# CameronDiao/MolCLR

Hardware: AMD Instinct MI355X
Metric: contrastive pre-train molecules/sec at batch 512, 1/2/4/8 MI355X; HBM GB/s on scatter_add (higher is better)
Workload: dtype f32; 1 GPU; c2: GIN 5x300 feat 512, batch 512/GPU, 10-50 atom graphs; model=gin 5x300 feat 512, global_batch=512, per_gpu_batch=512, mean_nodes_per_view=15278, mean_edges_per_view=25094, parallelism=dp1, views=one paired encoder pass, per-view BatchNorm statistics, augment=host: pre-built resident batch pairs

## Files before the change

### include/molclr.h

```cpp
#ifndef MOLCLR_H_
#define MOLCLR_H_

#include <stddef.h>
#include <stdint.h>

#ifdef __cplusplus
extern "C" {
#endif

typedef void* molclr_stream_t;

enum {
  MOLCLR_OK = 0,
  MOLCLR_ERR_ARG = -1,
  MOLCLR_ERR_WORKSPACE = -2,
  MOLCLR_ERR_UNSUPPORTED = -3
};

#define MOLCLR_NUM_ATOM_TYPE 119
#define MOLCLR_NUM_CHIRALITY 3
#define MOLCLR_NUM_BOND_TYPE 5
#define MOLCLR_NUM_BOND_DIR 3
#define MOLCLR_SELF_LOOP_BOND_TYPE 4
#define MOLCLR_ECOUNT_STRIDE 8
// ... 148 lines not shown
                         int64_t K, int64_t lda, int64_t ldb, int64_t ldc, int a_kmajor,
                         int b_kmajor, int epilogue_flags, const float* bias, const float* aux,
                         int64_t ldaux, void* workspace, size_t workspace_bytes,
                         molclr_stream_t stream, int impl);

size_t molclr_bplanes_bytes(int64_t N, int64_t K);
int molclr_bplanes_make(const float* B, int64_t N, int64_t K, int64_t ldb, int b_kmajor,
                        uint16_t* planes, molclr_stream_t stream);
int molclr_bplanes_make_batch(int count, const float* const* B, const int64_t* N,
                              const int64_t* K, const int64_t* ldb, const int* b_kmajor,
                              uint16_t* const* planes, molclr_stream_t stream);
int molclr_gemm_f32_bplanes(const float* A, const uint16_t* planes, float* C, int64_t M,
                            int64_t N, int64_t K, int64_t lda, int64_t ldc, int a_kmajor,
                            int epilogue_flags, const float* bias, const float* aux,
                            int64_t ldaux, void* workspace, size_t workspace_bytes,
                            molclr_stream_t stream);
int molclr_gemm_f32_bplanes_tile(const float* A, const uint16_t* planes, float* C, int64_t M,
                                 int64_t N, int64_t K, int64_t lda, int64_t ldc, int a_kmajor,
                                 int epilogue_flags, const float* bias, const float* aux,
                                 int64_t ldaux, void* workspace, size_t workspace_bytes,
                                 molclr_stream_t stream, int tile);

size_t molclr_linear_wgrad_workspace_bytes(int64_t rows, int64_t n_out, int64_t n_in);
int molclr_linear_wgrad(const float* dy, const float* x, float* dW, float* db, int64_t rows,
                        int64_t n_out, int64_t n_in, int64_t ld_dy, int64_t ld_x, int accumulate,
                        void* workspace, size_t workspace_bytes, molclr_stream_t stream);
int molclr_linear_wgrad_groups(const float* dy, const float* x, float* dW, float* db,
                               int64_t rows, int64_t n_out, int64_t n_in, int64_t ld_dy,
                               int64_t ld_x, int accumulate, void* workspace,
                               size_t workspace_bytes, molclr_stream_t stream, int groups);

int molclr_absmax_f32(const float* x, int64_t rows, int64_t cols, int64_t ld, float* slot,
                      int accumulate, molclr_stream_t stream);
size_t molclr_hplanes_bytes(int64_t N, int64_t K);
int molclr_hplanes_make_batch(int count, const float* const* B, const int64_t* N,
                              const int64_t* K, const int64_t* ldb, const int* b_kmajor,
                              uint16_t* const* planes, molclr_stream_t stream);
int64_t molclr_gemm_row_parts(int64_t N);
int molclr_gemm_f32_bplanes_max(const float* A, const uint16_t* planes, float* C, int64_t M,
                                int64_t N, int64_t K, int64_t lda, int64_t ldc,
                                int epilogue_flags, const float* bias, const float* aux,
                                int64_t ldaux, float* amax_out, float* cmax, float* crow,
                                uint32_t* relu_bits, void* workspace, size_t workspace_bytes,
                                molclr_stream_t stream);
int molclr_absmax_rows_f32(const float* x, int64_t rows, int64_t cols, int64_t ld,
                           float* rowmax, float* slot, int accumulate, molclr_stream_t stream);
int molclr_gemm_f32_h3(const float* A, const float* amax, int a_row_parts, const uint16_t* hplanes,
                       float* C, int64_t M, int64_t N, int64_t K, int64_t lda, int64_t ldc,
                       int epilogue_flags, const float* bias, const float* aux, int64_t ldaux,
                       const uint32_t* mask_bits, float* cmax, float* crow, float* amax_out,
                       molclr_stream_t stream);
int molclr_gemm_f32_h3_impl(const float* A, const float* amax, int a_row_parts,
                            const uint16_t* hplanes, float* C, int64_t M, int64_t N, int64_t K,
                            int64_t lda, int64_t ldc, int epilogue_flags, const float* bias,
                            const float* aux, int64_t ldaux, const uint32_t* mask_bits, float* cmax,
                            float* crow, float* amax_out, uint32_t* relu_bits,
                            molclr_stream_t stream, int impl);
int molclr_gemm_f32_h3_bits(const float* A, const float* amax, int a_row_parts,
                            const uint16_t* hplanes, float* C, int64_t M, int64_t N, int64_t K,
                            int64_t lda, int64_t ldc, int epilogue_flags, const float* bias,
                            const float* aux, int64_t ldaux, const uint32_t* mask_bits,
                            float* cmax, float* crow, float* amax_out, uint32_t* relu_bits,
                            molclr_stream_t stream);
int molclr_linear_wgrad_h3_groups(const float* dy, const float* dymax, const float* x,
                                  const float* xmax, float* dW, float* db, int64_t rows,
                                  int64_t n_out, int64_t n_in, int64_t ld_dy, int64_t ld_x,
                                  int accumulate, void* workspace, size_t workspace_bytes,
                                  molclr_stream_t stream, int groups);
int molclr_linear_wgrad_h3(const float* dy, const float* dymax, const float* x,
                           const float* xmax, float* dW, float* db, int64_t rows, int64_t n_out,
                           int64_t n_in, int64_t ld_dy, int64_t ld_x, int accumulate,
                           void* workspace, size_t workspace_bytes, molclr_stream_t stream);
size_t molclr_linear_wgrad_h3_pair_workspace_bytes(int64_t rows, int64_t n_out_a, int64_t n_in_a,
                                                   int64_t n_out_b, int64_t n_in_b);
int molclr_linear_wgrad_h3_pair(const float* dy_a, const float* dymax_a, const float* x_a,
                                const float* xmax_a, float* dW_a, float* db_a, int64_t n_out_a,
                                int64_t n_in_a, int64_t ld_dy_a, int64_t ld_x_a,
                                const float* dy_b, const float* dymax_b, const float* x_b,
                                const float* xmax_b, float* dW_b, float* db_b, int64_t n_out_b,
                                int64_t n_in_b, int64_t ld_dy_b, int64_t ld_x_b, int64_t rows,
                                int accumulate, void* workspace, size_t workspace_bytes,
                                molclr_stream_t stream);

size_t molclr_colsum_f32_workspace_bytes(int64_t rows, int64_t cols);
int molclr_colsum_f32(const float* X, float* out, int64_t rows, int64_t cols, int64_t ld,
                      int accumulate, void* workspace, size_t workspace_bytes,
                      molclr_stream_t stream);

size_t molclr_batchnorm_workspace_bytes(int64_t rows, int64_t dim);
int molclr_batchnorm_fwd(const float* z, const float* gamma, const float* beta,
                         float* running_mean, float* running_var,
                         int64_t* num_batches_tracked, float* y,
                         float* save_mean, float* save_invstd, int64_t rows, int64_t dim,
                         double momentum, double eps, int training, int relu,
                         void* workspace, size_t workspace_bytes, molclr_stream_t stream);
int molclr_batchnorm_bwd(const float* dy, const float* z, const float* gamma,
                         const float* beta, const float* save_mean,
                         const float* save_invstd, float* dz, float* dgamma, float* dbeta,
                         int64_t rows, int64_t dim, int relu, int accumulate, void* workspace,
                         size_t workspace_bytes, molclr_stream_t stream);

enum { MOLCLR_DTYPE_F32 = 0, MOLCLR_DTYPE_BF16 = 1 };
size_t molclr_batchnorm_seg_workspace_bytes(int nseg, const int64_t* seg_rows, int64_t dim);
int molclr_batchnorm_seg_fwd(const void* z, const float* gamma, const float* beta,
                             float* running_mean, float* running_var,
                             int64_t* num_batches_tracked, void* y, float* save_mean,
                             float* save_invstd, int nseg, const int64_t* seg_rows, int64_t dim,
                             int dtype, double momentum, double eps, int training, int relu,
                             void* workspace, size_t workspace_bytes, molclr_stream_t stream);
int molclr_batchnorm_seg_bwd(const void* dy, const void* z, const float* gamma,
                             const float* beta, const float* save_mean, const float* save_invstd,
                             void* dz, float* dgamma, float* dbeta, int nseg,
                             const int64_t* seg_rows, int64_t dim, int dtype, int relu,
                             int accumulate, void* workspace, size_t workspace_bytes,
                             molclr_stream_t stream);

int molclr_bn_row_parts(int64_t dim);
size_t molclr_batchnorm_seg_dev_workspace_bytes(int nseg, int64_t rows_cap, int64_t dim);
int molclr_batchnorm_seg_fwd_dev(const void* z, const float* gamma, const float* beta,
                                 float* running_mean, float* running_var,
                                 int64_t* num_batches_tracked, void* y, float* save_mean,
                                 float* save_invstd, int nseg, const int64_t* seg_rows_dev,
                                 int64_t rows_cap, int64_t dim, int dtype, double momentum,
                                 double eps, int training, int relu, void* workspace,
                                 size_t workspace_bytes, molclr_stream_t stream);
int molclr_batchnorm_seg_coeffs(const void* z, const float* gamma, const float* beta,
                                float* running_mean, float* running_var,
                                int64_t* num_batches_tracked, float* save_mean,
                                float* save_invstd, float* coeffs, int nseg,
                                const int64_t* seg_rows, int64_t dim, int dtype, double momentum,
                                double eps, int training, void* workspace, size_t workspace_bytes,
                                molclr_stream_t stream);
int molclr_batchnorm_seg_coeffs_dev(const void* z, const float* gamma, const float* beta,
                                    float* running_mean, float* running_var,
                                    int64_t* num_batches_tracked, float* save_mean,
                                    float* save_invstd, float* coeffs, int nseg,
                                    const int64_t* seg_rows_dev, int64_t rows_cap, int64_t dim,
                                    int dtype, double momentum, double eps, int training,
                                    void* workspace, size_t workspace_bytes,
                                    molclr_stream_t stream);
int molclr_batchnorm_seg_bwd_dev(const void* dy, const void* z, const float* gamma,
                                 const float* beta, const float* save_mean,
                                 const float* save_invstd, void* dz, float* dgamma, float* dbeta,
                                 int nseg, const int64_t* seg_rows_dev, int64_t rows_cap,
                                 int64_t dim, int dtype, int relu, int accumulate, float* rowmax,
                                 float* slot, void* workspace, size_t workspace_bytes,
                                 molclr_stream_t stream);
int molclr_batchnorm_seg_bwd_max(const float* dy, const float* z, const float* gamma,
                                 const float* beta, const float* save_mean,
                                 const float* save_invstd, float* dz, float* dgamma, float* dbeta,
                                 int nseg, const int64_t* seg_rows, int64_t dim, int relu,
                                 int accumulate, float* rowmax, float* slot, void* workspace,
                                 size_t workspace_bytes, molclr_stream_t stream);

int molclr_segment_pool_fwd(const float* h, const int32_t* graph_ptr, float* out,
                            int64_t num_graphs, int64_t dim, int mode,
                            molclr_stream_t stream);
int molclr_segment_pool_bwd(const float* dout, const int32_t* graph_ptr, float* dh,
                            int64_t num_nodes, int64_t num_graphs, int64_t dim, int mode,
                            molclr_stream_t stream);
int molclr_segment_max_fwd(const void* h, const int32_t* graph_ptr, float* out, int32_t* argmax,
                           int64_t num_graphs, int64_t dim, int dtype, molclr_stream_t stream);
int molclr_segment_max_bwd(const float* dout, const int32_t* argmax, void* dh, int64_t num_nodes,
                           int64_t num_graphs, int64_t dim, int dtype, molclr_stream_t stream);

int molclr_l2norm_fwd(const float* z, float* y, float* norm, int64_t rows, int64_t dim,
                      double eps, molclr_stream_t stream);
int molclr_l2norm_bwd(const float* dy, const float* y, const float* norm, float* dz,
                      int64_t rows, int64_t dim, double eps, molclr_stream_t stream);

int molclr_ntxent_prep(const float* r, float* rhat, float* norm, int64_t n, int64_t C,
                       int cosine, molclr_stream_t stream);
int molclr_ntxent_prep_bwd(const float* drhat, const float* rhat, const float* norm,
                           float* dr, int64_t n, int64_t C, int cosine,
                           molclr_stream_t stream);
int molclr_ntxent_prep_pair(const float* z, float* y, float* rhat, float* n1, float* n2,
                            int64_t batch_local, int64_t C, double eps, int cosine,
                            molclr_stream_t stream);
int molclr_ntxent_prep_pair_bwd(const float* drhat, const float* rhat, const float* n2,
                                const float* y, const float* n1, float* dz, int64_t batch_local,
                                int64_t C, double eps, int cosine, molclr_stream_t stream);
size_t molclr_ntxent_workspace_bytes(int64_t nrows, int64_t ncols, int64_t C);
int molclr_ntxent_fwd(const float* rhat_rows, const int32_t* row_gidx, const float* rhat_cols,
                      int64_t nrows, int64_t ncols, int64_t C, int64_t batch_size,
                      double temperature, float* lse_rows, float* loss_rows,
                      void* workspace, size_t workspace_bytes, molclr_stream_t stream);
int molclr_ntxent_bwd(const float* rhat_rows, const int32_t* row_gidx, const float* rhat_cols,
                      const float* lse_cols, const float* grad_loss, int64_t nrows,
                      int64_t ncols, int64_t C, int64_t batch_size, double temperature,
                      float* drhat_rows, void* workspace, size_t workspace_bytes,
                      molclr_stream_t stream);
size_t molclr_ntxent_sim_bytes(int64_t nrows, int64_t ncols, int64_t C, int impl);
int molclr_ntxent_fwd_impl(const float* rhat_rows, const int32_t* row_gidx,
                           const float* rhat_cols, int64_t nrows, int64_t ncols, int64_t C,
                           int64_t batch_size, double temperature, float* lse_rows,
                           float* loss_rows, float* sim, void* workspace, size_t workspace_bytes,
                           molclr_stream_t stream, int impl);
int molclr_ntxent_bwd_impl(const float* rhat_rows, const int32_t* row_gidx,
                           const float* rhat_cols, const float* lse_cols, const float* grad_loss,
                           int64_t nrows, int64_t ncols, int64_t C, int64_t batch_size,
                           double temperature, const float* sim, float* drhat_rows,
                           void* workspace, size_t workspace_bytes, molclr_stream_t stream,
                           int impl);
int molclr_sum_f32(const float* x, float* out, int64_t n, molclr_stream_t stream);

int molclr_adam_step(float* param, const float* grad, float* exp_avg, float* exp_avg_sq,
                     int64_t n, const float* lr, int32_t* step, double beta1, double beta2,
                     double eps, double weight_decay, molclr_stream_t stream);
int molclr_adam_step_ex(float* param, const float* grad, float* exp_avg, float* exp_avg_sq,
                        int64_t n, const float* lr, int32_t* step, double beta1, double beta2,
                        double eps, double weight_decay, int tick, molclr_stream_t stream);
int molclr_step_tail(int32_t* step, const float* loss_src, float* loss_dst,
                     const int32_t* status_src, int32_t* status_acc, molclr_stream_t stream);

typedef struct molclr_gin_encoder {
  int32_t num_layer;
  int32_t training;
  int64_t dim;
  int64_t n_atom;
  int64_t n_chiral;
  double momentum, eps;
  const float* x_embedding1;
  const float* x_embedding2;
  const float* mlp0_weight[MOLCLR_MAX_LAYERS];
  const float* mlp0_bias[MOLCLR_MAX_LAYERS];
  const float* mlp2_weight[MOLCLR_MAX_LAYERS];
  const float* mlp2_bias[MOLCLR_MAX_LAYERS];
  const float* edge_embedding1[MOLCLR_MAX_LAYERS];
  const float* edge_embedding2[MOLCLR_MAX_LAYERS];
  const float* bn_weight[MOLCLR_MAX_LAYERS];
  const float* bn_bias[MOLCLR_MAX_LAYERS];
  float* bn_running_mean[MOLCLR_MAX_LAYERS];
  float* bn_running_var[MOLCLR_MAX_LAYERS];
  int64_t* bn_num_batches_tracked[MOLCLR_MAX_LAYERS];
  const uint16_t* mlp0_planes[MOLCLR_MAX_LAYERS];
  const uint16_t* mlp0_planes_t[MOLCLR_MAX_LAYERS];
  const uint16_t* mlp2_planes[MOLCLR_MAX_LAYERS];
  const uint16_t* mlp2_planes_t[MOLCLR_MAX_LAYERS];
  int32_t dtype;
  int32_t fp32_gemm;
  int32_t* status;
} molclr_gin_encoder;

typedef struct molclr_gin_encoder_grads {
  float* x_embedding1;
  float* x_embedding2;
  float* mlp0_weight[MOLCLR_MAX_LAYERS];
  float* mlp0_bias[MOLCLR_MAX_LAYERS];
  float* mlp2_weight[MOLCLR_MAX_LAYERS];
  float* mlp2_bias[MOLCLR_MAX_LAYERS];
  float* edge_embedding1[MOLCLR_MAX_LAYERS];
  float* edge_embedding2[MOLCLR_MAX_LAYERS];
  float* bn_weight[MOLCLR_MAX_LAYERS];
  float* bn_bias[MOLCLR_MAX_LAYERS];
  void* layer_done[MOLCLR_MAX_LAYERS];
  void* embed_done;
} molclr_gin_encoder_grads;

typedef struct molclr_device_graph {
  int64_t num_nodes, num_edges, num_graphs;
  const int32_t *rowptr, *col, *rowptr_t, *col_t, *ecount, *graph_ptr;
  const uint8_t* ecode;
  const uint32_t *nbr, *nbr_t;
  int32_t num_segments;
  int64_t segment_nodes[MOLCLR_MAX_SEGMENTS];
  const int64_t* segment_nodes_dev;
} molclr_device_graph;

size_t molclr_gin_encoder_arena_bytes(int num_layer, int64_t num_nodes, int64_t dim, int dtype);
size_t molclr_gin_encoder_workspace_bytes(int num_layer, int64_t num_nodes, int64_t dim,
                                          int dtype);
int molclr_gin_encoder_fwd(const molclr_gin_encoder* enc, const int64_t* x,
                           const molclr_device_graph* graph, void* h_out, void* arena,
                           size_t arena_bytes, void* workspace, size_t workspace_bytes,
                           molclr_stream_t stream);
int molclr_gin_encoder_bwd(const molclr_gin_encoder* enc, const molclr_gin_encoder_grads* grads,
                           const int64_t* x, const molclr_device_graph* graph,
                           const void* dh_out, const void* arena, size_t arena_bytes,
                           void* workspace, size_t workspace_bytes, molclr_stream_t stream);

typedef struct molclr_gcn_encoder {
  int32_t num_layer;
  int32_t training;
  int64_t dim;
  int64_t n_atom;
  int64_t n_chiral;
  double momentum, eps;
  const float* x_embedding1;
  const float* x_embedding2;
  const float* weight[MOLCLR_MAX_LAYERS];
  const float* bias[MOLCLR_MAX_LAYERS];
  const float* edge_embedding1[MOLCLR_MAX_LAYERS];
  const float* edge_embedding2[MOLCLR_MAX_LAYERS];
  const float* bn_weight[MOLCLR_MAX_LAYERS];
  const float* bn_bias[MOLCLR_MAX_LAYERS];
  float* bn_running_mean[MOLCLR_MAX_LAYERS];
  float* bn_running_var[MOLCLR_MAX_LAYERS];
  int64_t* bn_num_batches_tracked[MOLCLR_MAX_LAYERS];
  const uint16_t* weight_planes[MOLCLR_MAX_LAYERS];
  const uint16_t* weight_planes_t[MOLCLR_MAX_LAYERS];
  int32_t fp32_gemm;
  int32_t* status;
} molclr_gcn_encoder;

typedef struct molclr_gcn_encoder_grads {
  float* x_embedding1;
// ... 130 lines not shown
```

### molclr_amd/_lib.py

```python
from __future__ import annotations

import ctypes
import os
from ctypes import POINTER, c_char_p, c_double, c_int, c_int64, c_size_t, c_uint64, c_void_p
from pathlib import Path

import torch

LIB_PATH = Path(os.environ.get("MOLCLR_LIB", Path(__file__).resolve().parent / "libmolclr_hip.so"))

_P = c_void_p
_I64 = c_int64

SIGNATURES = {
    "molclr_version": (c_char_p, []),
    "molclr_last_error": (c_char_p, []),
    "molclr_graph_build_workspace_bytes": (c_size_t, [_I64, _I64]),
    "molclr_graph_build": (c_int, [_P, _P, _P, _I64, _I64, _I64, _P, _P, _P, _P, _P, _P, _P, _P,
                                   _P, _P, _P, c_size_t, _P]),
    "molclr_graph_build_multi": (c_int, [c_int, _P, _P, _P, _P, _P, _P, _P, _P, _P, _P, _P, _P,
                                         c_size_t, _P]),
    "molclr_stage_segments": (c_int, [c_int, _P, _P, _P, _I64, _I64, _P, _P]),
    "molclr_graph_build_dev": (c_int, [c_int, _P, _P, _I64, _I64, _P, _P, _P, _P, _P, _P, _P, _P,
                                       _P, _P, _P, c_size_t, _P]),
    "molclr_mask_views_workspace_bytes": (c_size_t, [_I64]),
    "molclr_mask_views": (c_int, [_P, _P, _P, _P, _P, _I64, _I64, _P, _I64, c_uint64, c_int, _P, _P,
                                  _P, _P, _P, _I64, _I64, _P, _P, c_size_t, _P]),
    "molclr_atom_embed_fwd": (c_int, [_P, _P, _P, _P, _I64, _I64, _I64, _I64, _P, _P]),
    "molclr_atom_embed_bwd_workspace_bytes": (c_size_t, [_I64, _I64, _I64, _I64]),
    "molclr_atom_embed_bwd": (c_int, [_P, _P, _P, _P, _I64, _I64, _I64, _I64, c_int, _P, c_size_t,
                                      _P]),
    "molclr_edge_tables_combine": (c_int, [c_int, _P, _P, _P, _I64, _P]),
    "molclr_gine_aggregate_fwd": (c_int, [_P, _P, _P, _P, _P, _P, _P, _I64, _I64, _P]),
    "molclr_rowmax_layout": (_I64, [_I64]),
    "molclr_rowmax_bytes": (c_size_t, [_I64, _I64]),
    "molclr_gine_aggregate_fwd_rowmax": (c_int, [_P, _P, _P, _P, _P, _P, _P, _I64, _I64, _P, _P,
                                                 _P]),
    "molclr_gine_aggregate_bn_fwd": (c_int, [_P, _P, c_int, c_int, _P, _P, _P, _P, _P, _P, _P, _P,
                                             _I64, _I64, _P, _P, _P]),
    "molclr_gine_aggregate_bn_fwd_bf16": (c_int, [_P, _P, c_int, c_int, _P, _P, _P, _P, _P, _P, _P,
                                                  _P, _I64, _I64, _P]),
    "molclr_batchnorm_seg_coeffs": (c_int, [_P, _P, _P, _P, _P, _P, _P, _P, _P, c_int, _P, _I64,
                                            c_int, c_double, c_double, c_int, _P, c_size_t, _P]),
    "molclr_batchnorm_seg_coeffs_dev": (c_int, [_P, _P, _P, _P, _P, _P, _P, _P, _P, c_int, _P, _I64,
                                                _I64, c_int, c_double, c_double, c_int, _P,
                                                c_size_t, _P]),
    "molclr_gine_aggregate_bwd_workspace_bytes": (c_size_t, [_I64, _I64]),
    "molclr_gine_aggregate_bwd": (c_int, [_P, _P, _P, _P, _P, _P, _P, _P, _I64, _I64, c_int, _P,
                                          c_size_t, _P]),
    "molclr_gcn_aggregate_fwd": (c_int, [_P, _P, _P, _P, _P, _P, _P, _P, _P, _I64, _I64, _P]),
    "molclr_gcn_aggregate_bwd_workspace_bytes": (c_size_t, [_I64, _I64]),
    "molclr_gcn_aggregate_bwd": (c_int, [_P, _P, _P, _P, _P, _P, _P, _P, _P, _I64, _I64, c_int,
                                         _P, c_size_t, _P]),
    "molclr_gemm_f32_workspace_bytes": (c_size_t, [_I64, _I64, _I64]),
    "molclr_gemm_f32": (c_int, [_P, _P, _P, _I64, _I64, _I64, _I64, _I64, _I64, c_int, c_int, c_int,
                                _P, _P, _I64, _P, c_size_t, _P]),
    "molclr_gemm_f32_impl": (c_int, [_P, _P, _P, _I64, _I64, _I64, _I64, _I64, _I64, c_int, c_int,
                                     c_int, _P, _P, _I64, _P, c_size_t, _P, c_int]),
    "molclr_bplanes_bytes": (c_size_t, [_I64, _I64]),
    "molclr_bplanes_make": (c_int, [_P, _I64, _I64, _I64, c_int, _P, _P]),
    "molclr_bplanes_make_batch": (c_int, [c_int, _P, _P, _P, _P, _P, _P, _P]),
    "molclr_gemm_f32_bplanes": (c_int, [_P, _P, _P, _I64, _I64, _I64, _I64, _I64, c_int, c_int, _P,
                                        _P, _I64, _P, c_size_t, _P]),
    "molclr_gemm_f32_bplanes_tile": (c_int, [_P, _P, _P, _I64, _I64, _I64, _I64, _I64, c_int,
                                             c_int, _P, _P, _I64, _P, c_size_t, _P, c_int]),
    "molclr_linear_wgrad_workspace_bytes": (c_size_t, [_I64, _I64, _I64]),
    "molclr_linear_wgrad": (c_int, [_P, _P, _P, _P, _I64, _I64, _I64, _I64, _I64, c_int, _P, c_size_t,
                                    _P]),
    "molclr_linear_wgrad_groups": (c_int, [_P, _P, _P, _P, _I64, _I64, _I64, _I64, _I64, c_int, _P,
                                           c_size_t, _P, c_int]),
    "molclr_absmax_f32": (c_int, [_P, _I64, _I64, _I64, _P, c_int, _P]),
    "molclr_hplanes_bytes": (c_size_t, [_I64, _I64]),
    "molclr_hplanes_make_batch": (c_int, [c_int, _P, _P, _P, _P, _P, _P, _P]),
    "molclr_absmax_rows_f32": (c_int, [_P, _I64, _I64, _I64, _P, _P, c_int, _P]),
    "molclr_bn_row_parts": (c_int, [_I64]),
    "molclr_batchnorm_seg_bwd_max": (c_int, [_P, _P, _P, _P, _P, _P, _P, _P, _P, c_int, _P, _I64,
                                             c_int, c_int, _P, _P, _P, c_size_t, _P]),
    "molclr_gemm_row_parts": (_I64, [_I64]),
    "molclr_gemm_f32_bplanes_max": (c_int, [_P, _P, _P, _I64, _I64, _I64, _I64, _I64, c_int, _P,
                                            _P, _I64, _P, _P, _P, _P, _P, c_size_t, _P]),
    "molclr_gemm_f32_h3": (c_int, [_P, _P, c_int, _P, _P, _I64, _I64, _I64, _I64, _I64, c_int, _P,
                                   _P, _I64, _P, _P, _P, _P, _P]),
    "molclr_gemm_f32_h3_bits": (c_int, [_P, _P, c_int, _P, _P, _I64, _I64, _I64, _I64, _I64, c_int,
                                        _P, _P, _I64, _P, _P, _P, _P, _P, _P]),
    "molclr_gemm_f32_h3_impl": (c_int, [_P, _P, c_int, _P, _P, _I64, _I64, _I64, _I64, _I64, c_int,
                                        _P, _P, _I64, _P, _P, _P, _P, _P, _P, c_int]),
    "molclr_linear_wgrad_h3_groups": (c_int, [_P, _P, _P, _P, _P, _P, _I64, _I64, _I64, _I64, _I64,
                                              c_int, _P, c_size_t, _P, c_int]),
    "molclr_linear_wgrad_h3": (c_int, [_P, _P, _P, _P, _P, _P, _I64, _I64, _I64, _I64, _I64, c_int,
                                       _P, c_size_t, _P]),
    "molclr_colsum_f32_workspace_bytes": (c_size_t, [_I64, _I64]),
    "molclr_colsum_f32": (c_int, [_P, _P, _I64, _I64, _I64, c_int, _P, c_size_t, _P]),
    "molclr_batchnorm_workspace_bytes": (c_size_t, [_I64, _I64]),
    "molclr_batchnorm_fwd": (c_int, [_P, _P, _P, _P, _P, _P, _P, _P, _P, _I64, _I64, c_double,
                                     c_double, c_int, c_int, _P, c_size_t, _P]),
    "molclr_batchnorm_bwd": (c_int, [_P, _P, _P, _P, _P, _P, _P, _P, _P, _I64, _I64, c_int, c_int,
                                     _P, c_size_t, _P]),
    "molclr_batchnorm_seg_workspace_bytes": (c_size_t, [c_int, _P, _I64]),
    "molclr_batchnorm_seg_fwd": (c_int, [_P, _P, _P, _P, _P, _P, _P, _P, _P, c_int, _P, _I64, c_int,
                                         c_double, c_double, c_int, c_int, _P, c_size_t, _P]),
    "molclr_batchnorm_seg_bwd": (c_int, [_P, _P, _P, _P, _P, _P, _P, _P, _P, c_int, _P, _I64, c_int,
                                         c_int, c_int, _P, c_size_t, _P]),
    "molclr_batchnorm_seg_dev_workspace_bytes": (c_size_t, [c_int, _I64, _I64]),
    "molclr_batchnorm_seg_fwd_dev": (c_int, [_P, _P, _P, _P, _P, _P, _P, _P, _P, c_int, _P, _I64,
                                             _I64, c_int, c_double, c_double, c_int, c_int, _P,
                                             c_size_t, _P]),
    "molclr_batchnorm_seg_bwd_dev": (c_int, [_P, _P, _P, _P, _P, _P, _P, _P, _P, c_int, _P, _I64,
                                             _I64, c_int, c_int, c_int, _P, _P, _P, c_size_t, _P]),
    "molclr_segment_pool_fwd": (c_int, [_P, _P, _P, _I64, _I64, c_int, _P]),
    "molclr_segment_pool_bwd": (c_int, [_P, _P, _P, _I64, _I64, _I64, c_int, _P]),
    "molclr_l2norm_fwd": (c_int, [_P, _P, _P, _I64, _I64, c_double, _P]),
    "molclr_l2norm_bwd": (c_int, [_P, _P, _P, _P, _I64, _I64, c_double, _P]),
    "molclr_ntxent_prep": (c_int, [_P, _P, _P, _I64, _I64, c_int, _P]),
    "molclr_ntxent_prep_bwd": (c_int, [_P, _P, _P, _P, _I64, _I64, c_int, _P]),
    "molclr_ntxent_prep_pair": (c_int, [_P, _P, _P, _P, _P, _I64, _I64, c_double, c_int, _P]),
    "molclr_ntxent_prep_pair_bwd": (c_int, [_P, _P, _P, _P, _P, _P, _I64, _I64, c_double, c_int,
                                            _P]),
    "molclr_ntxent_workspace_bytes": (c_size_t, [_I64, _I64, _I64]),
    "molclr_ntxent_fwd": (c_int, [_P, _P, _P, _I64, _I64, _I64, _I64, c_double, _P, _P, _P,
                                  c_size_t, _P]),
    "molclr_ntxent_bwd": (c_int, [_P, _P, _P, _P, _P, _I64, _I64, _I64, _I64, c_double, _P, _P,
                                  c_size_t, _P]),
    "molclr_ntxent_sim_bytes": (c_size_t, [_I64, _I64, _I64, c_int]),
    "molclr_ntxent_fwd_impl": (c_int, [_P, _P, _P, _I64, _I64, _I64, _I64, c_double, _P, _P,
                                       _P, _P, c_size_t, _P, c_int]),
    "molclr_ntxent_bwd_impl": (c_int, [_P, _P, _P, _P, _P, _I64, _I64, _I64, _I64, c_double, _P,
                                       _P, _P, c_size_t, _P, c_int]),
    "molclr_sum_f32": (c_int, [_P, _P, _I64, _P]),
    "molclr_linear_wgrad_h3_pair_workspace_bytes": (c_size_t, [_I64, _I64, _I64, _I64, _I64]),
    "molclr_linear_wgrad_h3_pair": (c_int, [_P, _P, _P, _P, _P, _P, _I64, _I64, _I64, _I64,
                                            _P, _P, _P, _P, _P, _P, _I64, _I64, _I64, _I64,
                                            _I64, c_int, _P, c_size_t, _P]),
    "molclr_adam_step": (c_int, [_P, _P, _P, _P, _I64, _P, _P, c_double, c_double, c_double,
                                 c_double, _P]),
    "molclr_adam_step_ex": (c_int, [_P, _P, _P, _P, _I64, _P, _P, c_double, c_double, c_double,
                                    c_double, c_int, _P]),
    "molclr_step_tail": (c_int, [_P, _P, _P, _P, _P, _P]),
    "molclr_gin_encoder_arena_bytes": (c_size_t, [c_int, _I64, _I64, c_int]),
    "molclr_gin_encoder_workspace_bytes": (c_size_t, [c_int, _I64, _I64, c_int]),
    "molclr_gin_encoder_fwd": (c_int, [_P, _P, _P, _P, _P, c_size_t, _P, c_size_t, _P]),
    "molclr_gin_encoder_bwd": (c_int, [_P, _P, _P, _P, _P, _P, c_size_t, _P, c_size_t, _P]),
    "molclr_gcn_encoder_arena_bytes": (c_size_t, [c_int, _I64, _I64]),
    "molclr_gcn_encoder_workspace_bytes": (c_size_t, [c_int, _I64, _I64]),
    "molclr_gcn_encoder_fwd": (c_int, [_P, _P, _P, _P, _P, c_size_t, _P, c_size_t, _P]),
    "molclr_gcn_encoder_bwd": (c_int, [_P, _P, _P, _P, _P, _P, c_size_t, _P, c_size_t, _P]),
    "molclr_aug_views_workspace_bytes": (c_size_t, [_I64, _I64, _I64]),
    "molclr_aug_views_plan": (c_int, [_P, _P, _P, _I64, _I64, _P, _I64, ctypes.c_uint64, c_int,
                                      c_int, _I64, _I64, _P, _P, _P, _P, c_size_t, _P]),
    "molclr_aug_views_big_workspace_bytes": (c_size_t, [_I64, _I64, _I64]),
    "molclr_aug_views_plan_big": (c_int, [_P, _P, _P, _I64, _I64, _P, _I64, ctypes.c_uint64,
                                          c_int, c_int, _I64, _I64, _P, _P, _P, _P, c_size_t,
                                          _I64, _I64, _I64, _P, c_size_t, _P]),
    "molclr_aug_views_write": (c_int, [_P, _P, _P, _P, _P, _I64, _I64, _P, _I64, _P, _I64, _I64,
                                       _I64, _P, _P, _P, _P, _P, c_size_t, _P]),
    "molclr_atom_embed_fwd_bf16": (c_int, [_P, _P, _P, _P, _I64, _I64, _I64, _I64, _P, _P]),
    "molclr_atom_embed_bwd_bf16": (c_int, [_P, _P, _P, _P, _I64, _I64, _I64, _I64, c_int, _P,
                                           c_size_t, _P]),
    "molclr_gine_aggregate_fwd_bf16": (c_int, [_P, _P, _P, _P, _P, _P, _P, _I64, _I64, _P]),
    "molclr_gine_aggregate_bwd_bf16": (c_int, [_P, _P, _P, _P, _P, _P, _P, _P, _I64, _I64, c_int,
                                               _P, c_size_t, _P]),
    "molclr_segment_max_fwd": (c_int, [_P, _P, _P, _P, _I64, _I64, c_int, _P]),
    "molclr_segment_max_bwd": (c_int, [_P, _P, _P, _I64, _I64, _I64, c_int, _P]),
    "molclr_segment_pool_fwd_bf16": (c_int, [_P, _P, _P, _I64, _I64, c_int, _P]),
    "molclr_segment_pool_bwd_bf16": (c_int, [_P, _P, _P, _I64, _I64, _I64, c_int, _P]),
    "molclr_gemm_bf16": (c_int, [_P, _P, _P, _I64, _I64, _I64, _I64, _I64, c_int, _P, _P, _I64,
                                 _P]),
    "molclr_gemm_bf16_bits": (c_int, [_P, _P, _P, _I64, _I64, _I64, _I64, _I64, c_int, _P, _P, _P,
                                      _P]),
    "molclr_gemm_bf16_impl": (c_int, [_P, _P, _P, _I64, _I64, _I64, _I64, _I64, c_int, _P, _P,
                                      _I64, _P, c_int]),
    "molclr_linear_wgrad_bf16_workspace_bytes": (c_size_t, [_I64, _I64, _I64]),
    "molclr_linear_wgrad_bf16_impl": (c_int, [_P, _P, _P, _P, _I64, _I64, _I64, _I64, _I64, c_int,
                                              _P, c_size_t, _P, c_int]),
    "molclr_linear_wgrad_bf16": (c_int, [_P, _P, _P, _P, _I64, _I64, _I64, _I64, _I64, c_int, _P,
                                         c_size_t, _P]),
    "molclr_task_head_workspace_bytes": (c_size_t, [_P]),
    "molclr_task_head_fwd": (c_int, [_P, _P, c_size_t, _P]),
    "molclr_task_head_bwd": (c_int, [_P, _P, _P, c_size_t, _P]),
    "molclr_ktimer_start": (c_int, [c_int]),
    "molclr_ktimer_read": (c_int, [c_int, _P, _P]),
    "molclr_ktimer_stop": (c_int, []),
}

EPI_NONE, EPI_BIAS, EPI_BIAS_RELU, EPI_RELU_MASK = 0, 1, 2, 3
EPI_ACCUMULATE = 16
NUM_ECOMB = 15
MAX_LAYERS = 16
MAX_SEGMENTS = 8
DTYPE_F32, DTYPE_BF16 = 0, 1
STATUS_ATOM_RANGE = 8
STATUS_LABEL_RANGE = 16
TASK_HEAD_MAX_LAYERS = 10
TASK_HEAD_MAX_CLASSES = 16
TASK_HEAD_MAX_DIM = 2044
ACT_NONE, ACT_RELU, ACT_SOFTPLUS = 0, 1, 2
LOSS_NONE, LOSS_CROSS_ENTROPY, LOSS_MSE, LOSS_L1 = 0, 1, 2, 3
KTIMER_GINE_AGG = 1
KTIMER_GEMM = 2
KTIMER_NTXENT = 4
KTIMER_GCN_AGG = 8
AUG_SUBGRAPH, AUG_MIX = 0, 1


_L16 = c_void_p * 16


class GinEncoder(ctypes.Structure):
    _fields_ = [("num_layer", ctypes.c_int32), ("training", ctypes.c_int32), ("dim", c_int64),
                ("n_atom", c_int64), ("n_chiral", c_int64), ("momentum", c_double),
                ("eps", c_double), ("x_embedding1", c_void_p), ("x_embedding2", c_void_p)] + [
        (f, _L16) for f in ("mlp0_weight", "mlp0_bias", "mlp2_weight", "mlp2_bias",
                            "edge_embedding1", "edge_embedding2", "bn_weight", "bn_bias",
                            "bn_running_mean", "bn_running_var", "bn_num_batches_tracked",
                            "mlp0_planes", "mlp0_planes_t", "mlp2_planes", "mlp2_planes_t")] + [
        ("dtype", ctypes.c_int32), ("fp32_gemm", ctypes.c_int32), ("status", c_void_p)]


class GinEncoderGrads(ctypes.Structure):
    _fields_ = [("x_embedding1", c_void_p), ("x_embedding2", c_void_p)] + [
        (f, _L16) for f in ("mlp0_weight", "mlp0_bias", "mlp2_weight", "mlp2_bias",
                            "edge_embedding1", "edge_embedding2", "bn_weight", "bn_bias")] + [
        ("layer_done", _L16), ("embed_done", c_void_p)]


class GcnEncoder(ctypes.Structure):
    _fields_ = [("num_layer", ctypes.c_int32), ("training", ctypes.c_int32), ("dim", c_int64),
                ("n_atom", c_int64), ("n_chiral", c_int64), ("momentum", c_double),
                ("eps", c_double), ("x_embedding1", c_void_p), ("x_embedding2", c_void_p)] + [
        (f, _L16) for f in ("weight", "bias", "edge_embedding1", "edge_embedding2", "bn_weight",
                            "bn_bias", "bn_running_mean", "bn_running_var",
                            "bn_num_batches_tracked", "weight_planes", "weight_planes_t")] + [
        ("fp32_gemm", ctypes.c_int32), ("status", c_void_p)]


class GcnEncoderGrads(ctypes.Structure):
    _fields_ = [("x_embedding1", c_void_p), ("x_embedding2", c_void_p)] + [
        (f, _L16) for f in ("weight", "bias", "edge_embedding1", "edge_embedding2", "bn_weight",
                            "bn_bias")] + [("layer_done", _L16), ("embed_done", c_void_p)]


_L10 = c_void_p * 10


class TaskHeadC(ctypes.Structure):
    _fields_ = [("num_layers", ctypes.c_int32), ("loss", ctypes.c_int32), ("rows", c_int64),
                ("dims", c_int64 * 11), ("act", ctypes.c_int32 * 10), ("x", c_void_p),
                ("ldx", c_int64), ("weight", _L10), ("bias", _L10), ("a", _L10),
                ("target", c_void_p), ("loss_out", c_void_p), ("status", c_void_p),
                ("sync", c_void_p)]


class TaskHeadGradsC(ctypes.Structure):
    _fields_ = [("gloss", c_void_p), ("dh", c_void_p), ("dpred", c_void_p), ("dx", c_void_p),
                ("lddx", c_int64), ("dweight", _L10), ("dbias", _L10),
                ("accumulate", ctypes.c_int32 * 10)]


class DeviceGraphC(ctypes.Structure):
    _fields_ = [("num_nodes", c_int64), ("num_edges", c_int64), ("num_graphs", c_int64)] + [
        (f, c_void_p) for f in ("rowptr", "col", "rowptr_t", "col_t", "ecount", "graph_ptr",
                                "ecode", "nbr", "nbr_t")] + [
# ... 79 lines not shown
```

### molclr_amd/csrc/aggregate.hip

```cpp
#include "common.h"

#include <stdlib.h>

namespace {

constexpr int kT = 256;

template <typename St, int U = 1>
__global__ void k_atom_embed_fwd(const int64_t* __restrict__ x, const float4* __restrict__ X1,
                                 const float4* __restrict__ X2, typename St::T* __restrict__ h,
                                 int64_t N, int d4, int64_t n1, int64_t n2,
                                 int32_t* __restrict__ status) {
  int64_t t = (int64_t)blockIdx.x * blockDim.x + threadIdx.x;
  if (t >= N * d4 / U) return;
  const int64_t u0 = t * U;
  int64_t i = N * d4 < (1ll << 32) ? (int64_t)((uint32_t)u0 / (uint32_t)d4) : u0 / d4;
  int c = (int)(u0 - i * d4);
  const int64_t a = x[2 * i], b = x[2 * i + 1];
  float4 v[U];
  if (a < 0 || a >= n1 || b < 0 || b >= n2) {
    const float q = __builtin_nanf("");
#pragma unroll
    for (int j = 0; j < U; ++j) v[j] = make_float4(q, q, q, q);
    if (c == 0 && status != nullptr) atomicOr(status, MOLCLR_STATUS_ATOM_RANGE);
// ... 80 lines not shown
    kchunk0[k] = kc[k];
  }
  const int nch = kc[nk];
  for (int c = t; c < max_chunks; c += 1024) {
    if (c >= nch) break;
    int lo = 0, hi = nk - 1;
    while (lo < hi) {
      const int mid = (lo + hi + 1) >> 1;
      if (kc[mid] <= c) lo = mid;
      else hi = mid - 1;
    }
    const int32_t q = (c - kc[lo]) * kEmbChunk;
    cbeg[c] = ks[lo] + q;
    cend[c] = ks[lo] + (q + kEmbChunk < tot[lo] ? q + kEmbChunk : tot[lo]);
  }
}

__global__ __launch_bounds__(kEmbBlock) void k_emb_scatter(const int64_t* __restrict__ x,
                                                           int64_t N, int64_t n1, int64_t n2,
                                                           const int32_t* __restrict__ off,
                                                           const int32_t* __restrict__ kstart,
                                                           int32_t* __restrict__ perm) {
  __shared__ int32_t keys[kEmbBlock];
  const int nk = (int)(n1 + n2);
  const int64_t item = (int64_t)blockIdx.x * kEmbBlock + threadIdx.x;
  const bool live = item < 2 * N;
  const int k = live ? emb_key(x, item, N, n1, n2) : -1;
  keys[threadIdx.x] = k;
  __syncthreads();
  if (!live) return;
  int rank = 0;
  for (int j = 0; j < (int)threadIdx.x; ++j) rank += keys[j] == k;
  (void)nk;
  perm[kstart[k] + off[(int64_t)k * gridDim.x + blockIdx.x] + rank] =
      (int32_t)(item < N ? item : item - N);
}

template <typename St>
__global__ __launch_bounds__(64) void k_emb_chunk_sum(const typename St::T* __restrict__ dh,
                                                      const int32_t* __restrict__ perm,
                                                      const int32_t* __restrict__ cbeg,
                                                      const int32_t* __restrict__ cend,
                                                      const int32_t* __restrict__ nchunks,
                                                      int64_t d4, double* __restrict__ csum) {
  const int64_t ch = blockIdx.x;
  if (ch >= *nchunks) return;
  const int64_t c = (int64_t)blockIdx.y * 64 + threadIdx.x;
  if (c >= d4) return;
  const int32_t beg = cbeg[ch], end = cend[ch];
  float4 acc = f4zero();
  int32_t i = beg;
  for (; i + 16 <= end; i += 16) {
    float4 v[16];
#pragma unroll
    for (int u = 0; u < 16; ++u) v[u] = St::ld(dh, (int64_t)perm[i + u] * d4 + c);
#pragma unroll
    for (int u = 0; u < 16; ++u) acc = f4add(acc, v[u]);
  }
  for (; i + 4 <= end; i += 4) {
    float4 v[4];
#pragma unroll
    for (int u = 0; u < 4; ++u) v[u] = St::ld(dh, (int64_t)perm[i + u] * d4 + c);
#pragma unroll
    for (int u = 0; u < 4; ++u) acc = f4add(acc, v[u]);
  }
  for (; i < end; ++i) acc = f4add(acc, St::ld(dh, (int64_t)perm[i] * d4 + c));
  double* o = csum + ch * 4 * d4 + 4 * c;
  o[0] = acc.x;
  o[1] = acc.y;
  o[2] = acc.z;
  o[3] = acc.w;
}

constexpr int kEmbFinW = 8;
__global__ __launch_bounds__(64 * kEmbFinW) void k_emb_finish(
    const double* __restrict__ csum, const int32_t* __restrict__ kchunk0, int64_t n1, int64_t n2,
    int64_t D, float* __restrict__ dX1, float* __restrict__ dX2, int accumulate) {
  __shared__ double red[kEmbFinW][64];
  const int lane = threadIdx.x & 63, w = threadIdx.x >> 6;
  const int64_t k = blockIdx.x;
  const int64_t col = (int64_t)blockIdx.y * 64 + lane;
  double acc = 0.0;
  if (col < D) {
    int32_t ch = kchunk0[k] + w;
    const int32_t ce = kchunk0[k + 1];
    for (; ch + 7 * kEmbFinW < ce; ch += 8 * kEmbFinW) {
      double v[8];
#pragma unroll
      for (int u = 0; u < 8; ++u) v[u] = csum[(int64_t)(ch + u * kEmbFinW) * D + col];
#pragma unroll
      for (int u = 0; u < 8; ++u) acc += v[u];
    }
    for (; ch < ce; ch += kEmbFinW) acc += csum[(int64_t)ch * D + col];
  }
  red[w][lane] = acc;
  __syncthreads();
  if (w != 0 || col >= D) return;
  double t = red[0][lane];
#pragma unroll
  for (int q = 1; q < kEmbFinW; ++q) t += red[q][lane];
  float* o = k < n1 ? dX1 + k * D + col : dX2 + (k - n1) * D + col;
  *o = accumulate ? *o + (float)t : (float)t;
}

__global__ __launch_bounds__(1024) void k_reduce_partials_split(
    const double* __restrict__ partial, int64_t P, int64_t rows, int64_t D, int64_t split,
    float* __restrict__ outA, float* __restrict__ outB, int accumulate) {
  constexpr int EL = 16, LANES = 64;
  __shared__ double red[LANES][EL];
  const int cl = threadIdx.x % EL, rl = threadIdx.x / EL;
  const int64_t t = (int64_t)blockIdx.x * EL + cl;
  const int64_t n = rows * D;
  double a0 = 0.0, a1 = 0.0, a2 = 0.0, a3 = 0.0;
  if (t < n) {
    int64_t p = rl;
    for (; p + 3 * LANES < P; p += 4 * LANES) {
      a0 += partial[p * n + t];
      a1 += partial[(p + LANES) * n + t];
      a2 += partial[(p + 2 * LANES) * n + t];
      a3 += partial[(p + 3 * LANES) * n + t];
    }
    for (; p < P; p += LANES) a0 += partial[p * n + t];
  }
  double acc = (a0 + a1) + (a2 + a3);
  red[rl][cl] = acc;
  __syncthreads();
#pragma unroll
  for (int stride = LANES / 2; stride > 0; stride >>= 1) {
    if (rl < stride) red[rl][cl] = acc = acc + red[rl + stride][cl];
    __syncthreads();
  }
  if (rl != 0 || t >= n) return;
  int64_t r = t / D;
  float* o = r < split ? (outA ? outA + t : nullptr) : (outB ? outB + (t - split * D) : nullptr);
  if (o) *o = accumulate ? *o + (float)acc : (float)acc;
}

struct TablePtrs {
  const float* e1[MOLCLR_MAX_LAYERS];
  const float* e2[MOLCLR_MAX_LAYERS];
};
__global__ void k_edge_tables_combine(TablePtrs p, float* __restrict__ Ec, int layers, int64_t D,
                                      float* __restrict__ zero, int64_t n_zero) {
  const int64_t per = (int64_t)MOLCLR_NUM_ECOMB * D;
  int64_t t = (int64_t)blockIdx.x * blockDim.x + threadIdx.x;
  if (t < n_zero) zero[t] = 0.f;
  if (t >= layers * per) return;
  const int l = (int)(t / per);
  const int64_t rc = t - l * per;
  const int r = (int)(rc / D);
  const int64_t c = rc - (int64_t)r * D;
  Ec[t] = p.e1[l][(r / 3) * D + c] + p.e2[l][(r % 3) * D + c];
}

__device__ __forceinline__ uint32_t nbr_degree(uint32_t w0) { return w0 >> 29; }
__device__ __forceinline__ int32_t nbr_node(uint32_t w) { return (int32_t)(w & 0xFFFFFFu); }
__device__ __forceinline__ int nbr_ecomb(uint32_t w) { return (int)((w >> 24) & 15u); }

__device__ __forceinline__ float4 gine_msg(const float4* __restrict__ x, const float4* __restrict__ Ec,
                                           uint32_t w, int d4, int c) {
  return f4add(x[(int64_t)nbr_node(w) * d4 + c], Ec[nbr_ecomb(w) * d4 + c]);
}

struct NoSrcArgs {};
struct BnSrcArgs {
  const float4* scale;
  const float4* shift;
  int relu;
  Segs sg;
};

template <typename St>
__device__ __forceinline__ float4 bn_src_unit(float4 v, float4 sc, float4 sh, bool relu) {
  float4 o = make_float4(bn_apply1(v.x, sc.x, sh.x), bn_apply1(v.y, sc.y, sh.y),
                         bn_apply1(v.z, sc.z, sh.z), bn_apply1(v.w, sc.w, sh.w));
  if (relu) o = make_float4(fmaxf(o.x, 0.f), fmaxf(o.y, 0.f), fmaxf(o.z, 0.f), fmaxf(o.w, 0.f));
  if constexpr (St::kBytes == 2) {
    const uint32_t lo = f32x2_to_bf16x2(o.x, o.y), hi = f32x2_to_bf16x2(o.z, o.w);
    o = make_float4(bf16_to_f32(lo & 0xFFFFu), bf16_to_f32(lo >> 16), bf16_to_f32(hi & 0xFFFFu),
                    bf16_to_f32(hi >> 16));
  }
  return o;
}

template <typename St, typename SA>
struct AggSrc {
  __device__ __forceinline__ AggSrc(const SA&, int64_t, int, int) {}
  __device__ __forceinline__ float4 operator()(const typename St::T* __restrict__ x,
                                               int64_t unit) const {
    return St::ld(x, unit);
  }
};
template <typename St>
struct AggSrc<St, BnSrcArgs> {
  float4 sc, sh;
  bool relu, pad;
  __device__ __forceinline__ AggSrc(const BnSrcArgs& a, int64_t i, int c, int d4) {
    const int s = seg_of_row(a.sg, i);
    pad = s < 0;
    relu = a.relu != 0;
    sc = pad ? f4zero() : a.scale[s * d4 + c];
    sh = pad ? f4zero() : a.shift[s * d4 + c];
  }
  __device__ __forceinline__ float4 operator()(const typename St::T* __restrict__ x,
                                               int64_t unit) const {
    if (pad) return f4zero();
    return bn_src_unit<St>(St::ld(x, unit), sc, sh, relu);
  }
};

template <typename St, bool NT = false, typename SA = NoSrcArgs>
__device__ __forceinline__ float4 gine_agg_elem(
    const typename St::T* __restrict__ x, const int32_t* __restrict__ rowptr,
    const int32_t* __restrict__ col, const uint8_t* __restrict__ ecode,
    const uint4* __restrict__ nbr, const float4* __restrict__ Ec, typename St::T* __restrict__ out,
    int64_t t, int64_t i, int c, int d4, const SA& sa) {
  const AggSrc<St, SA> src(sa, i, c, d4);
  auto X = [&](int64_t idx) { return src(x, idx); };
  auto msg = [&](uint32_t w) {
    return f4add(X((int64_t)nbr_node(w) * d4 + c), Ec[nbr_ecomb(w) * d4 + c]);
  };
  const uint4 s = nbr[i];
  const float4 self = X(t);
  const float4 es = Ec[MOLCLR_SELF_LOOP_ECOMB * d4 + c];
  const uint32_t deg = nbr_degree(s.x);
  float4 acc = f4zero();
  if (deg <= MOLCLR_NBR_SLOTS) {
    const float4 m0 = deg > 0 ? msg(s.x) : acc;
    const float4 m1 = deg > 1 ? msg(s.y) : acc;
    const float4 m2 = deg > 2 ? msg(s.z) : acc;
    const float4 m3 = deg > 3 ? msg(s.w) : acc;
    if (deg > 0) acc = f4add(acc, m0);
    if (deg > 1) acc = f4add(acc, m1);
    if (deg > 2) acc = f4add(acc, m2);
    if (deg > 3) acc = f4add(acc, m3);
  } else {
    for (int32_t k = rowptr[i], e = rowptr[i + 1]; k < e; ++k)
      acc = f4add(acc, f4add(X((int64_t)col[k] * d4 + c), Ec[MOLCLR_ECOMB(ecode[k]) * d4 + c]));
  }
  acc = f4add(acc, f4add(self, es));
  if constexpr (NT) {
    typedef float f4v __attribute__((ext_vector_type(4)));
    __builtin_nontemporal_store(f4v{acc.x, acc.y, acc.z, acc.w}, reinterpret_cast<f4v*>(out) + t);
  } else {
    St::st(out, t, acc);
  }
  return acc;
}

template <typename St, bool ROWMAX, bool NT = false, typename SA = NoSrcArgs>
__global__ __launch_bounds__(kT) void k_gine_agg_fwd(
    const typename St::T* __restrict__ x, const int32_t* __restrict__ rowptr,
    const int32_t* __restrict__ col, const uint8_t* __restrict__ ecode,
    const uint4* __restrict__ nbr, const float4* __restrict__ Ec, typename St::T* __restrict__ out,
    int64_t N, int d4, float* __restrict__ rowparts, int nparts, float* __restrict__ slot, SA sa) {
  int64_t t = (int64_t)xcd_remap(blockIdx.x, gridDim.x) * blockDim.x + threadIdx.x;
  int64_t i;
  int c;
  if (N * d4 < (1ll << 32)) {
    const uint32_t q = (uint32_t)t / (uint32_t)d4;
    i = q;
    c = (int)((uint32_t)t - q * (uint32_t)d4);
  } else {
    i = t / d4;
    c = (int)(t - i * d4);
  }
  if constexpr (ROWMAX) {
    float m = 0.f;
    int row = -1;
    if (t < N * d4) {
      const float4 v = gine_agg_elem<St, NT>(x, rowptr, col, ecode, nbr, Ec, out, t, i, c, d4, sa);
      m = fmaxf(fmaxf(fabsf(v.x), fabsf(v.y)), fmaxf(fabsf(v.z), fabsf(v.w)));
      row = (int)i;
    }
    if (nparts < 0)
      row_max_waves(m, row, t, N, d4, reinterpret_cast<float2*>(rowparts));
    else
      row_max_parts(m, row, t, N, d4, rowparts, nparts);
    if (slot != nullptr) absmax_publish(m, slot);
    return;
  }
  if (t >= N * d4) return;
  gine_agg_elem<St, NT>(x, rowptr, col, ecode, nbr, Ec, out, t, i, c, d4, sa);
}

template <typename St = StF32>
__global__ __launch_bounds__(kT) void k_transpose_gather(const typename St::T* __restrict__ g,
                                                         const int32_t* __restrict__ rowptr_t,
                                                         const int32_t* __restrict__ col_t,
                                                         const uint4* __restrict__ nbr_t,
                                                         typename St::T* __restrict__ dx, int64_t N,
                                                         int d4) {
  int64_t t = (int64_t)xcd_remap(blockIdx.x, gridDim.x) * blockDim.x + threadIdx.x;
  if (t >= N * d4) return;
  int64_t j = N * d4 < (1ll << 32) ? (int64_t)((uint32_t)t / (uint32_t)d4) : t / d4;
  int c = (int)(t - j * d4);
  const uint4 s = nbr_t[j];
  const uint32_t deg = nbr_degree(s.x);
  float4 acc = f4zero();
  if (deg <= MOLCLR_NBR_SLOTS) {
    if (deg > 0) acc = f4add(acc, St::ld(g, (int64_t)nbr_node(s.x) * d4 + c));
    if (deg > 1) acc = f4add(acc, St::ld(g, (int64_t)nbr_node(s.y) * d4 + c));
    if (deg > 2) acc = f4add(acc, St::ld(g, (int64_t)nbr_node(s.z) * d4 + c));
    if (deg > 3) acc = f4add(acc, St::ld(g, (int64_t)nbr_node(s.w) * d4 + c));
  } else {
    for (int32_t k = rowptr_t[j], e = rowptr_t[j + 1]; k < e; ++k)
      acc = f4add(acc, St::ld(g, (int64_t)col_t[k] * d4 + c));
  }
  St::st(dx, t, f4add(acc, St::ld(g, t)));
}
// ... 751 lines not shown
```

### molclr_amd/csrc/common.h

```cpp
#pragma once

#include <hip/hip_ext.h>
#include <hip/hip_runtime.h>

#include <type_traits>
#include <stdint.h>
#include <stddef.h>

#include "../../include/molclr.h"

#define MOLCLR_API extern "C" __attribute__((visibility("default")))

namespace molclr {

void set_error(const char* fmt, ...) __attribute__((format(printf, 1, 2)));

inline hipStream_t as_stream(molclr_stream_t s) { return reinterpret_cast<hipStream_t>(s); }

int edge_tables_combine_zero(int layers, const float* const* E1s, const float* const* E2s,
                             float* Ec, int64_t D, float* zero, int64_t n_zero,
                             molclr_stream_t stream);

int hplanes_make_and_max(const float* B, int64_t N, int64_t K, uint16_t* planes, const float* x,
                         int64_t x_rows, int64_t x_cols, float* x_slot, hipStream_t stream);
// ... 104 lines not shown
}
}

inline hipError_t fill_async(void* p, int v, size_t bytes, hipStream_t s) {
  if (bytes == 0) return hipSuccess;
  hipLaunchKernelGGL(detail::k_fill_bytes, dim3(detail::fill_blocks(bytes)), dim3(256), 0, s,
                     static_cast<uint8_t*>(p), bytes, (uint8_t)v);
  return hipGetLastError();
}
inline hipError_t zero_async(void* p, size_t bytes, hipStream_t s) {
  return fill_async(p, 0, bytes, s);
}
inline hipError_t copy_async(void* dst, const void* src, size_t bytes, hipStream_t s) {
  if (bytes == 0) return hipSuccess;
  hipLaunchKernelGGL(detail::k_copy_bytes, dim3(detail::fill_blocks(bytes)), dim3(256), 0, s,
                     static_cast<uint8_t*>(dst), static_cast<const uint8_t*>(src), bytes);
  return hipGetLastError();
}

}

size_t molclr_batchnorm_ws_bound(int64_t rows, int64_t D);

#define MOLCLR_REQUIRE(cond, ...)        \
  do {                                   \
    if (!(cond)) {                       \
      molclr::set_error(__VA_ARGS__);    \
      return MOLCLR_ERR_ARG;             \
    }                                    \
  } while (0)

#define MOLCLR_REQUIRE_WS(ws, need)                                                   \
  do {                                                                                \
    if ((ws) < (need)) {                                                              \
      molclr::set_error("%s: workspace %zu bytes < required %zu", __func__,           \
                        (size_t)(ws), (size_t)(need));                                \
      return MOLCLR_ERR_WORKSPACE;                                                    \
    }                                                                                 \
  } while (0)

#define MOLCLR_TRY_RC(expr)   \
  do {                        \
    int rc_ = (expr);         \
    if (rc_) return rc_;      \
  } while (0)

#define MOLCLR_LAUNCHED()                                                             \
  do {                                                                                \
    hipError_t e_ = hipGetLastError();                                                \
    if (e_ != hipSuccess) {                                                           \
      molclr::set_error("%s: launch failed: %s", __func__, hipGetErrorString(e_));    \
      return (int)e_;                                                                 \
    }                                                                                 \
  } while (0)

__device__ __forceinline__ float4 f4add(float4 a, float4 b) {
  return make_float4(a.x + b.x, a.y + b.y, a.z + b.z, a.w + b.w);
}
__device__ __forceinline__ int xcd_remap(int bid, int nwg) {
  int q = nwg / 8, r = nwg % 8;
  int x = bid % 8, pos = bid / 8;
  int base = x < r ? x * (q + 1) : r * (q + 1) + (x - r) * q;
  return base + pos;
}

__device__ __forceinline__ float4 f4zero() { return make_float4(0.f, 0.f, 0.f, 0.f); }

__device__ __forceinline__ void wave_lds_sync() {
  __builtin_amdgcn_fence(__ATOMIC_RELEASE, "wavefront");
  __builtin_amdgcn_wave_barrier();
  __builtin_amdgcn_fence(__ATOMIC_ACQUIRE, "wavefront");
}

struct StF32 {
  typedef float T;
  static constexpr int kBytes = 4;
  __device__ __forceinline__ static float4 ld(const T* __restrict__ p, int64_t unit) {
    return reinterpret_cast<const float4*>(p)[unit];
  }
  __device__ __forceinline__ static void st(T* __restrict__ p, int64_t unit, float4 v) {
    reinterpret_cast<float4*>(p)[unit] = v;
  }
  __device__ __forceinline__ static void ld2(const T* __restrict__ p, int64_t u2, float4& a,
                                             float4& b) {
    a = reinterpret_cast<const float4*>(p)[2 * u2];
    b = reinterpret_cast<const float4*>(p)[2 * u2 + 1];
  }
  __device__ __forceinline__ static void st2(T* __restrict__ p, int64_t u2, float4 a, float4 b) {
    reinterpret_cast<float4*>(p)[2 * u2] = a;
    reinterpret_cast<float4*>(p)[2 * u2 + 1] = b;
  }
  __device__ __forceinline__ static float ld1(const T* __restrict__ p, int64_t i) { return p[i]; }
  __device__ __forceinline__ static void st1(T* __restrict__ p, int64_t i, float v) { p[i] = v; }
};

__device__ __forceinline__ float bf16_to_f32(uint32_t bits16) {
  return __uint_as_float(bits16 << 16);
}
__device__ __forceinline__ uint32_t f32x2_to_bf16x2(float a, float b) {
  typedef __bf16 bf2 __attribute__((ext_vector_type(2)));
  const bf2 v = {(__bf16)a, (__bf16)b};
  return __builtin_bit_cast(uint32_t, v);
}

struct StBF16 {
  typedef uint16_t T;
  static constexpr int kBytes = 2;
  __device__ __forceinline__ static float4 ld(const T* __restrict__ p, int64_t unit) {
    const uint2 u = reinterpret_cast<const uint2*>(p)[unit];
    return make_float4(bf16_to_f32(u.x & 0xFFFFu), bf16_to_f32(u.x >> 16),
                       bf16_to_f32(u.y & 0xFFFFu), bf16_to_f32(u.y >> 16));
  }
  __device__ __forceinline__ static void st(T* __restrict__ p, int64_t unit, float4 v) {
    reinterpret_cast<uint2*>(p)[unit] = make_uint2(f32x2_to_bf16x2(v.x, v.y), f32x2_to_bf16x2(v.z, v.w));
  }
  __device__ __forceinline__ static void ld2(const T* __restrict__ p, int64_t u2, float4& a,
                                             float4& b) {
    const uint4 q = reinterpret_cast<const uint4*>(p)[u2];
    a = make_float4(bf16_to_f32(q.x & 0xFFFFu), bf16_to_f32(q.x >> 16), bf16_to_f32(q.y & 0xFFFFu),
                    bf16_to_f32(q.y >> 16));
    b = make_float4(bf16_to_f32(q.z & 0xFFFFu), bf16_to_f32(q.z >> 16), bf16_to_f32(q.w & 0xFFFFu),
                    bf16_to_f32(q.w >> 16));
  }
  __device__ __forceinline__ static void st2(T* __restrict__ p, int64_t u2, float4 a, float4 b) {
    reinterpret_cast<uint4*>(p)[u2] = make_uint4(f32x2_to_bf16x2(a.x, a.y), f32x2_to_bf16x2(a.z, a.w),
                                                 f32x2_to_bf16x2(b.x, b.y), f32x2_to_bf16x2(b.z, b.w));
  }
  __device__ __forceinline__ static float ld1(const T* __restrict__ p, int64_t i) {
    return bf16_to_f32(p[i]);
  }
  __device__ __forceinline__ static void st1(T* __restrict__ p, int64_t i, float v) {
    p[i] = (uint16_t)(f32x2_to_bf16x2(v, 0.f) & 0xFFFFu);
  }
};

struct Segs {
  int n;
  int band;
  int64_t rows[MOLCLR_MAX_SEGMENTS];
  const int64_t* drows;
};

__device__ __forceinline__ int64_t seg_n(const Segs& sg, int s) {
  return sg.drows ? sg.drows[s] : sg.rows[s];
}
__device__ __forceinline__ int seg_of_row(const Segs& sg, int64_t i) {
  int64_t r = 0;
  for (int s = 0; s < sg.n; ++s) {
    r += seg_n(sg, s);
    if (i < r) return s;
  }
  return -1;
}

__device__ __forceinline__ float bn_apply1(float z, float sc, float sh) { return __fmaf_rn(z, sc, sh); }

__device__ __forceinline__ float wave_sum(float v) {
#pragma unroll
  for (int o = 32; o > 0; o >>= 1) v += __shfl_xor(v, o, 64);
  return v;
}
__device__ __forceinline__ float wave_max_dpp(float v) {
  auto dpp = [](float x, auto ctrl) {
    return __int_as_float(__builtin_amdgcn_update_dpp(0, __float_as_int(x), decltype(ctrl)::value,
                                                      0xF, 0xF, false));
  };
  v = fmaxf(v, dpp(v, std::integral_constant<int, 0xB1>{}));
  v = fmaxf(v, dpp(v, std::integral_constant<int, 0x4E>{}));
  v = fmaxf(v, dpp(v, std::integral_constant<int, 0x141>{}));
  v = fmaxf(v, dpp(v, std::integral_constant<int, 0x140>{}));
  const float a = __int_as_float(__builtin_amdgcn_readlane(__float_as_int(v), 0));
  const float b = __int_as_float(__builtin_amdgcn_readlane(__float_as_int(v), 16));
  const float c = __int_as_float(__builtin_amdgcn_readlane(__float_as_int(v), 32));
  const float d = __int_as_float(__builtin_amdgcn_readlane(__float_as_int(v), 48));
  return fmaxf(fmaxf(a, b), fmaxf(c, d));
}
__device__ __forceinline__ float wave_max(float v) {
#pragma unroll
  for (int o = 32; o > 0; o >>= 1) v = fmaxf(v, __shfl_xor(v, o, 64));
  return v;
}

__device__ __forceinline__ void row_max_parts(float m, int row, int64_t t, int64_t rows, int d4,
                                              float* __restrict__ rowparts, int nparts) {
  const int lane = threadIdx.x & 63;
  if (d4 >= 64) {
    const int64_t t0 = t - lane;
    const int64_t r0 = rows * d4 < (1ll << 32) ? (int64_t)((uint32_t)t0 / (uint32_t)d4) : t0 / d4;
    const bool second = row >= 0 && row != r0;
    const float m0 = wave_max_dpp(second ? 0.f : m), m1 = wave_max_dpp(second ? m : 0.f);
    if (lane == 0 && r0 < rows) {
      const int64_t rs = r0 * d4;
      const int part = (int)((t0 >> 6) - (rs >> 6));
      rowparts[part * rows + r0] = m0;
      if (part == 0)
        for (int q = (int)(((rs + d4 - 1) >> 6) - (rs >> 6)) + 1; q < nparts; ++q)
          rowparts[q * rows + r0] = 0.f;
    }
    const int64_t r1 = r0 + 1, rs1 = r1 * d4;
    if (lane == 1 && r1 < rows && rs1 < t0 + 64) {
      rowparts[r1] = m1;
      for (int q = (int)(((rs1 + d4 - 1) >> 6) - (rs1 >> 6)) + 1; q < nparts; ++q)
        rowparts[q * rows + r1] = 0.f;
    }
    return;
  }
#pragma unroll
  for (int off = 1; off < 64; off <<= 1) {
    const float mv = __shfl_down(m, off, 64);
    const int rv = __shfl_down(row, off, 64);
    if (lane + off < 64 && rv == row) m = fmaxf(m, mv);
  }
  const int rp = __shfl_up(row, 1, 64);
  if (row >= 0 && (lane == 0 || rp != row)) {
    const int64_t rs = (int64_t)row * d4;
    const int part = (int)((t >> 6) - (rs >> 6));
    rowparts[part * rows + row] = m;
    if (part == 0)
      for (int q = (int)(((rs + d4 - 1) >> 6) - (rs >> 6)) + 1; q < nparts; ++q)
        rowparts[q * rows + row] = 0.f;
  }
}

__device__ __forceinline__ void row_max_waves(float m, int row, int64_t t, int64_t rows, int d4,
                                              float2* __restrict__ wm) {
  const int lane = threadIdx.x & 63;
  const int64_t t0 = t - lane;
  const int64_t r0 = rows * d4 < (1ll << 32) ? (int64_t)((uint32_t)t0 / (uint32_t)d4) : t0 / d4;
  const bool second = row >= 0 && row != r0;
  const float m0 = wave_max_dpp(second ? 0.f : m), m1 = wave_max_dpp(second ? m : 0.f);
  if (lane == 0 && t0 < rows * d4) wm[t0 >> 6] = make_float2(m0, m1);
}
__device__ __forceinline__ float row_max_of_waves(const float2* __restrict__ wm, int64_t row,
                                                  int d4) {
  const int64_t s = row * d4, e = s + d4 - 1;
  float m = 0.f;
  for (int64_t w = s >> 6; w <= (e >> 6); ++w) {
    const float2 v = wm[w];
    m = fmaxf(m, (w << 6) >= s ? v.x : v.y);
  }
  return m;
}

constexpr int kMaxSlotParts = 64;
constexpr int kMaxSlotStride = 32;
constexpr int kMaxSlotFloats = kMaxSlotParts * kMaxSlotStride;

__device__ __forceinline__ float absmax4_range(const float4* __restrict__ x, int64_t t, int64_t n4,
                                               int64_t stride) {
  auto amax4 = [](float4 v) {
    return fmaxf(fmaxf(fabsf(v.x), fabsf(v.y)), fmaxf(fabsf(v.z), fabsf(v.w)));
  };
  float m = 0.f;
  for (; t + 7 * stride < n4; t += 8 * stride) {
    float4 v[8];
#pragma unroll
    for (int j = 0; j < 8; ++j) v[j] = x[t + j * stride];
#pragma unroll
    for (int j = 0; j < 8; ++j) m = fmaxf(m, amax4(v[j]));
  }
  for (; t < n4; t += stride) m = fmaxf(m, amax4(x[t]));
  return m;
}

__device__ __forceinline__ float block_max(float v) {
  __shared__ float red_b[16];
  v = wave_max(v);
  if ((threadIdx.x & 63) == 0) red_b[threadIdx.x >> 6] = v;
  __syncthreads();
  if (threadIdx.x == 0)
    for (int w = 1; w < (int)(blockDim.x >> 6); ++w) v = fmaxf(v, red_b[w]);
  return v;
}

__device__ __forceinline__ void absmax_publish(float v, float* slot) {
  __shared__ float red_[16];
  v = wave_max(v);
  if ((threadIdx.x & 63) == 0) red_[threadIdx.x >> 6] = v;
  __syncthreads();
  if (threadIdx.x == 0) {
    for (int w = 1; w < (int)((blockDim.x + 63) >> 6); ++w) v = fmaxf(v, red_[w]);
    atomicMax(reinterpret_cast<unsigned int*>(slot + (blockIdx.x % kMaxSlotParts) * kMaxSlotStride),
              __float_as_uint(v));
  }
  __syncthreads();
}
```

### molclr_amd/csrc/encoder.hip

```cpp
#include "common.h"

#include <stdlib.h>

namespace {

bool agg_bn() {
  static const bool on = [] {
    const char* e = getenv("MOLCLR_AGG_BN");
    return !(e != nullptr && e[0] == '0');
  }();
  return on;
}

struct ArenaLayout {
  size_t agg[MOLCLR_MAX_LAYERS], a1[MOLCLR_MAX_LAYERS], z[MOLCLR_MAX_LAYERS],
      h[MOLCLR_MAX_LAYERS], mean[MOLCLR_MAX_LAYERS], invstd[MOLCLR_MAX_LAYERS],
      coef[MOLCLR_MAX_LAYERS];
  size_t bits[MOLCLR_MAX_LAYERS];
  size_t h0, ec, smax, bmax, total;
  ArenaLayout(int L, int64_t N, int64_t D, size_t es) {
    size_t used = 0;
    auto off = [&](size_t bytes) {
      const size_t o = used;
      used += (bytes + 255) / 256 * 256;
      return o;
    };
    for (int l = 0; l < L; ++l) {
      agg[l] = off(N * D * es);
      a1[l] = off(N * 2 * D * es);
      z[l] = off(N * D * es);
      h[l] = agg_bn() ? 0 : off(N * D * es);
      mean[l] = off(MOLCLR_MAX_SEGMENTS * D * sizeof(float));
      invstd[l] = off(MOLCLR_MAX_SEGMENTS * D * sizeof(float));
      coef[l] = off(2 * MOLCLR_MAX_SEGMENTS * D * sizeof(float));
      bits[l] = off((size_t)N * ((2 * D + 31) / 32) * sizeof(uint32_t));
    }
    h0 = off(N * D * es);
    ec = off((size_t)L * MOLCLR_NUM_ECOMB * D * sizeof(float));
    smax = off((size_t)MOLCLR_MAX_LAYERS * 2 * kMaxSlotFloats * sizeof(float));
    bmax = off((size_t)MOLCLR_MAX_LAYERS * 2 * kMaxSlotFloats * sizeof(float));
    total = used;
  }
};

size_t elem_bytes(int dtype) { return dtype == MOLCLR_DTYPE_BF16 ? 2 : 4; }

size_t kernels_ws(int64_t N, int64_t D) {
  size_t m = 0;
  auto mx = [&](size_t v) { m = v > m ? v : m; };
  mx(molclr_gemm_f32_workspace_bytes(2 * D, D, N));
  mx(molclr_gemm_f32_workspace_bytes(D, 2 * D, N));
  mx(molclr_gemm_f32_workspace_bytes(N, 2 * D, D));
  mx(molclr_gemm_f32_workspace_bytes(N, D, 2 * D));
  mx(molclr_colsum_f32_workspace_bytes(N, 2 * D));
  mx(molclr_linear_wgrad_workspace_bytes(N, D, 2 * D));
  mx(molclr_linear_wgrad_workspace_bytes(N, 2 * D, D));
  if (N >= 1024 && D % 4 == 0) mx(molclr_linear_wgrad_h3_pair_workspace_bytes(N, D, 2 * D, 2 * D, D));
  mx(molclr_linear_wgrad_bf16_workspace_bytes(N, D, 2 * D));
  mx(molclr_linear_wgrad_bf16_workspace_bytes(N, 2 * D, D));
  mx(molclr_batchnorm_ws_bound(N, D));
  mx(molclr_gine_aggregate_bwd_workspace_bytes(N, D));
  mx(molclr_atom_embed_bwd_workspace_bytes(N, D, MOLCLR_NUM_ATOM_TYPE, MOLCLR_NUM_CHIRALITY));
  return m;
}

size_t scratch_bytes(int64_t N, int64_t D, size_t es) { return ((size_t)N * D * 3 + (size_t)N * 2 * D) * es; }

int check_encoder(const molclr_gin_encoder* e, const molclr_device_graph* g) {
  MOLCLR_REQUIRE(e && g, "gin_encoder: null encoder / graph");
  MOLCLR_REQUIRE(e->num_layer >= 1 && e->num_layer <= MOLCLR_MAX_LAYERS,
                 "gin_encoder: num_layer %d", e->num_layer);
  MOLCLR_REQUIRE(e->dim > 0 && e->dim % 4 == 0, "gin_encoder: dim %lld", (long long)e->dim);
  MOLCLR_REQUIRE(e->dtype == MOLCLR_DTYPE_F32 || (e->dtype == MOLCLR_DTYPE_BF16 && e->dim % 8 == 0),
                 "gin_encoder: dtype %d (bf16 needs dim %% 8 == 0)", e->dtype);
  MOLCLR_REQUIRE(e->n_atom == MOLCLR_NUM_ATOM_TYPE && e->n_chiral == MOLCLR_NUM_CHIRALITY,
                 "gin_encoder: embedding tables must be [%d,D] and [%d,D]",
                 MOLCLR_NUM_ATOM_TYPE, MOLCLR_NUM_CHIRALITY);
  for (int l = 0; l < e->num_layer; ++l)
    MOLCLR_REQUIRE(e->mlp0_planes[l] && e->mlp0_planes_t[l] && e->mlp2_planes[l] &&
                       e->mlp2_planes_t[l] && e->bn_weight[l] && e->bn_bias[l],
                   "gin_encoder: layer %d: missing planes or BatchNorm affine", l);
  return MOLCLR_OK;
}

struct SegRows {
  int n;
  const int64_t* rows;
  const int64_t* dev;
  int64_t cap;
};
int graph_segments(const molclr_device_graph* g, const int64_t* N, SegRows& out) {
  if (g->segment_nodes_dev) {
    MOLCLR_REQUIRE(g->num_segments >= 1 && g->num_segments <= MOLCLR_MAX_SEGMENTS,
                   "encoder: %d graph segments", g->num_segments);
    out = {g->num_segments, nullptr, g->segment_nodes_dev, *N};
    return MOLCLR_OK;
  }
  if (g->num_segments <= 1) {
    out = {1, N, nullptr, *N};
    return MOLCLR_OK;
  }
  MOLCLR_REQUIRE(g->num_segments <= MOLCLR_MAX_SEGMENTS, "encoder: %d graph segments",
                 g->num_segments);
  int64_t tot = 0;
  for (int s = 0; s < g->num_segments; ++s) tot += g->segment_nodes[s];
  MOLCLR_REQUIRE(tot == *N, "encoder: segment nodes sum to %lld, graph has %lld", (long long)tot,
                 (long long)*N);
  out = {g->num_segments, g->segment_nodes, nullptr, *N};
  return MOLCLR_OK;
}

int seg_bn_fwd(const SegRows& sg, const void* z, const float* gamma, const float* beta,
               float* rmean, float* rvar, int64_t* nbt, void* y, float* mean, float* invstd,
               int64_t D, int dtype, double momentum, double eps, int training, int relu,
               void* ws, size_t ws_bytes, molclr_stream_t stream) {
  if (sg.dev)
    return molclr_batchnorm_seg_fwd_dev(z, gamma, beta, rmean, rvar, nbt, y, mean, invstd, sg.n,
                                        sg.dev, sg.cap, D, dtype, momentum, eps, training, relu,
                                        ws, ws_bytes, stream);
  return molclr_batchnorm_seg_fwd(z, gamma, beta, rmean, rvar, nbt, y, mean, invstd, sg.n,
                                  sg.rows, D, dtype, momentum, eps, training, relu, ws, ws_bytes,
                                  stream);
}
int seg_bn_coeffs(const SegRows& sg, const void* z, const float* gamma, const float* beta,
                  float* rmean, float* rvar, int64_t* nbt, float* mean, float* invstd, float* coef,
                  int64_t D, int dtype, double momentum, double eps, int training, void* ws,
                  size_t ws_bytes, molclr_stream_t stream) {
  if (sg.dev)
    return molclr_batchnorm_seg_coeffs_dev(z, gamma, beta, rmean, rvar, nbt, mean, invstd, coef,
                                           sg.n, sg.dev, sg.cap, D, dtype, momentum, eps, training,
                                           ws, ws_bytes, stream);
  return molclr_batchnorm_seg_coeffs(z, gamma, beta, rmean, rvar, nbt, mean, invstd, coef, sg.n,
                                     sg.rows, D, dtype, momentum, eps, training, ws, ws_bytes,
                                     stream);
}
int seg_bn_bwd(const SegRows& sg, const void* dy, const void* z, const float* gamma,
               const float* beta, const float* mean, const float* invstd, void* dz, float* dgamma,
               float* dbeta, int64_t D, int dtype, int relu, int accumulate, float* rowmax,
               float* slot, void* ws, size_t ws_bytes, molclr_stream_t stream) {
  if (sg.dev)
    return molclr_batchnorm_seg_bwd_dev(dy, z, gamma, beta, mean, invstd, dz, dgamma, dbeta, sg.n,
                                        sg.dev, sg.cap, D, dtype, relu, accumulate, rowmax, slot,
                                        ws, ws_bytes, stream);
  if (rowmax)
    return molclr_batchnorm_seg_bwd_max((const float*)dy, (const float*)z, gamma, beta, mean,
                                        invstd, (float*)dz, dgamma, dbeta, sg.n, sg.rows, D, relu,
                                        accumulate, rowmax, slot, ws, ws_bytes, stream);
  return molclr_batchnorm_seg_bwd(dy, z, gamma, beta, mean, invstd, dz, dgamma, dbeta, sg.n,
                                  sg.rows, D, dtype, relu, accumulate, ws, ws_bytes, stream);
}

#define MOLCLR_TRY(expr)      \
  do {                        \
    int rc_ = (expr);         \
    if (rc_) return rc_;      \
  } while (0)

int record_done(void* ev, molclr_stream_t stream) {
  if (ev && hipEventRecord(static_cast<hipEvent_t>(ev), molclr::as_stream(stream)) != hipSuccess) {
    molclr::set_error("encoder_bwd: hipEventRecord failed");
    return MOLCLR_ERR_ARG;
  }
  return MOLCLR_OK;
}

}

MOLCLR_API size_t molclr_gin_encoder_arena_bytes(int L, int64_t N, int64_t D, int dtype) {
  if (L < 1 || L > MOLCLR_MAX_LAYERS) return 0;
  return ArenaLayout(L, N, D, elem_bytes(dtype)).total;
}

constexpr size_t kSlotBytes = MOLCLR_MAX_LAYERS * 2 * kMaxSlotFloats * sizeof(float);
size_t rowmax_first_bytes(int64_t N, int64_t D) {
  const size_t dz = (size_t)molclr_bn_row_parts(D) * N * sizeof(float);
  const size_t agg = molclr_rowmax_bytes(N, D);
  return molclr::align_up(dz > agg ? dz : agg, 256);
}
size_t rowmax_bytes(int64_t N, int64_t D) {
  return molclr::align_up(
      rowmax_first_bytes(N, D) + (size_t)molclr_gemm_row_parts(2 * D) * N * sizeof(float), 256);
}

MOLCLR_API size_t molclr_gin_encoder_workspace_bytes(int L, int64_t N, int64_t D, int dtype) {
  (void)L;
  return molclr::align_up(scratch_bytes(N, D, elem_bytes(dtype)), 256) + kSlotBytes +
         rowmax_bytes(N, D) + kernels_ws(N, D) + 256;
}

MOLCLR_API int molclr_gin_encoder_fwd(const molclr_gin_encoder* e, const int64_t* x,
                                      const molclr_device_graph* g, void* h_out, void* arena,
                                      size_t arena_bytes, void* workspace, size_t workspace_bytes,
                                      molclr_stream_t stream) {
  MOLCLR_TRY(check_encoder(e, g));
  const int L = e->num_layer;
  const int64_t N = g->num_nodes, D = e->dim;
  if (N == 0) return MOLCLR_OK;
  SegRows seg;
  MOLCLR_TRY(graph_segments(g, &g->num_nodes, seg));
  MOLCLR_REQUIRE(x && h_out && arena, "gin_encoder_fwd: null pointer");
  const bool bf = e->dtype == MOLCLR_DTYPE_BF16;
  const size_t es = elem_bytes(e->dtype);
  const ArenaLayout lay(L, N, D, es);
  MOLCLR_REQUIRE_WS(arena_bytes, lay.total);
  MOLCLR_REQUIRE_WS(workspace_bytes, molclr_gin_encoder_workspace_bytes(L, N, D, e->dtype));
  char* A = (char*)arena;
  auto F = [&](size_t off) { return (float*)(A + off); };
  auto H = [&](size_t off) { return (uint16_t*)(A + off); };
  float* ragg = (float*)((char*)workspace + molclr::align_up(scratch_bytes(N, D, es), 256) +
                         kSlotBytes);
  float* ra1 = (float*)((char*)ragg + rowmax_first_bytes(N, D));
  void* kws = (char*)ragg + rowmax_bytes(N, D);
  const size_t kws_bytes = kernels_ws(N, D);
  const bool h3 = !bf && e->fp32_gemm != 0;
  const bool h3f = h3 && (e->fp32_gemm & 2);
  float* fmax = F(lay.smax);

  const bool fused = agg_bn();
  void* h = A + lay.h0;
  if (bf)
    MOLCLR_TRY(molclr_atom_embed_fwd_bf16(x, e->x_embedding1, e->x_embedding2, (uint16_t*)h, N, D,
                                          e->n_atom, e->n_chiral, e->status, stream));
  else
    MOLCLR_TRY(molclr_atom_embed_fwd(x, e->x_embedding1, e->x_embedding2, (float*)h, N, D,
                                     e->n_atom, e->n_chiral, e->status, stream));
  float* Ec = F(lay.ec);
  const int64_t nz = h3 ? (int64_t)(lay.bmax - lay.smax) / 4 + (int64_t)L * 2 * kMaxSlotFloats : 0;
  MOLCLR_TRY(molclr::edge_tables_combine_zero(L, e->edge_embedding1, e->edge_embedding2, Ec, D,
                                              h3 ? fmax : nullptr, nz, stream));
  for (int l = 0; l < L; ++l) {
    const bool last = l == L - 1;
    const bool bn_src = fused && l > 0;
    const bool bn_next = fused && !last;
    void* y = last ? h_out : bn_next ? nullptr : A + lay.h[l];
    const float* Ecl = Ec + (size_t)l * MOLCLR_NUM_ECOMB * D;
    const void* zp = bn_src ? A + lay.z[l - 1] : nullptr;
    const float* cp = bn_src ? F(lay.coef[l - 1]) : nullptr;
    if (bf) {
      uint16_t *agg = H(lay.agg[l]), *a1 = H(lay.a1[l]), *z = H(lay.z[l]);
      if (bn_src)
        MOLCLR_TRY(molclr_gine_aggregate_bn_fwd_bf16((const uint16_t*)zp, cp, 1, seg.n, seg.rows,
                                                     seg.dev, g->rowptr, g->col, g->ecode, g->nbr,
                                                     Ecl, agg, N, D, stream));
      else
        MOLCLR_TRY(molclr_gine_aggregate_fwd_bf16((const uint16_t*)h, g->rowptr, g->col, g->ecode,
                                                  g->nbr, Ecl, agg, N, D, stream));
      if (D % 64 == 0)
        MOLCLR_TRY(molclr_gemm_bf16_bits(agg, e->mlp0_planes[l], a1, N, 2 * D, D, D, 2 * D,
                                         MOLCLR_EPI_BIAS_RELU, e->mlp0_bias[l],
                                         (uint32_t*)(A + lay.bits[l]), nullptr, stream));
      else
        MOLCLR_TRY(molclr_gemm_bf16(agg, e->mlp0_planes[l], a1, N, 2 * D, D, D, 2 * D,
                                    MOLCLR_EPI_BIAS_RELU, e->mlp0_bias[l], nullptr, 0, stream));
      MOLCLR_TRY(molclr_gemm_bf16(a1, e->mlp2_planes[l], z, N, D, 2 * D, 2 * D, D,
                                  MOLCLR_EPI_BIAS, e->mlp2_bias[l], nullptr, 0, stream));
      if (bn_next)
        MOLCLR_TRY(seg_bn_coeffs(seg, z, e->bn_weight[l], e->bn_bias[l], e->bn_running_mean[l],
                                 e->bn_running_var[l], e->bn_num_batches_tracked[l],
                                 F(lay.mean[l]), F(lay.invstd[l]), F(lay.coef[l]), D,
                                 MOLCLR_DTYPE_BF16, e->momentum, e->eps, e->training, kws,
                                 kws_bytes, stream));
      else
        MOLCLR_TRY(seg_bn_fwd(seg, z, e->bn_weight[l], e->bn_bias[l], e->bn_running_mean[l],
                              e->bn_running_var[l], e->bn_num_batches_tracked[l], y,
                              F(lay.mean[l]), F(lay.invstd[l]), D, MOLCLR_DTYPE_BF16, e->momentum,
                              e->eps, e->training, last ? 0 : 1, kws, kws_bytes, stream));
    } else {
      float *agg = F(lay.agg[l]), *a1 = F(lay.a1[l]), *z = F(lay.z[l]);
      float* sl = fmax + 2 * l * kMaxSlotFloats;
      if (bn_src)
        MOLCLR_TRY(molclr_gine_aggregate_bn_fwd((const float*)zp, cp, 1, seg.n, seg.rows, seg.dev,
                                                g->rowptr, g->col, g->ecode, g->nbr, Ecl, agg, N,
                                                D, h3f ? ragg : nullptr, nullptr, stream));
      else if (h3f)
        MOLCLR_TRY(molclr_gine_aggregate_fwd_rowmax((const float*)h, g->rowptr, g->col, g->ecode,
                                                    g->nbr, Ecl, agg, N, D, ragg, nullptr,
                                                    stream));
      else
        MOLCLR_TRY(molclr_gine_aggregate_fwd((const float*)h, g->rowptr, g->col, g->ecode, g->nbr,
                                             Ecl, agg, N, D, stream));
      if (h3f) {
        const uint16_t* p0 = e->mlp0_planes[l];
        const uint16_t* p2 = e->mlp2_planes[l];
        MOLCLR_TRY(molclr_gemm_f32_h3_bits(agg, ragg, (int)molclr_rowmax_layout(D), p0, a1, N,
                                           2 * D, D, D, 2 * D, MOLCLR_EPI_BIAS_RELU,
                                           e->mlp0_bias[l], nullptr, 0, nullptr,
                                           sl + kMaxSlotFloats, ra1, sl,
                                           (uint32_t*)(A + lay.bits[l]), stream));
        MOLCLR_TRY(molclr_gemm_f32_h3(a1, ra1, (int)molclr_gemm_row_parts(2 * D), p2, z, N, D,
                                      2 * D, 2 * D, D, MOLCLR_EPI_BIAS, e->mlp2_bias[l], nullptr, 0,
                                      nullptr,
                                      nullptr, nullptr, nullptr, stream));
      } else {
        if (h3)
          MOLCLR_TRY(molclr_gemm_f32_bplanes_max(agg, e->mlp0_planes[l], a1, N, 2 * D, D, D, 2 * D,
                                                 MOLCLR_EPI_BIAS_RELU, e->mlp0_bias[l], nullptr, 0,
                                                 fmax + 2 * l * kMaxSlotFloats,
                                                 fmax + (2 * l + 1) * kMaxSlotFloats, nullptr,
                                                 (uint32_t*)(A + lay.bits[l]), kws, kws_bytes,
                                                 stream));
        else
          MOLCLR_TRY(molclr_gemm_f32_bplanes(agg, e->mlp0_planes[l], a1, N, 2 * D, D, D, 2 * D, 0,
                                             MOLCLR_EPI_BIAS_RELU, e->mlp0_bias[l], nullptr, 0, kws,
                                             kws_bytes, stream));
        MOLCLR_TRY(molclr_gemm_f32_bplanes(a1, e->mlp2_planes[l], z, N, D, 2 * D, 2 * D, D, 0,
                                           MOLCLR_EPI_BIAS, e->mlp2_bias[l], nullptr, 0, kws,
                                           kws_bytes, stream));
      }
      if (bn_next)
        MOLCLR_TRY(seg_bn_coeffs(seg, z, e->bn_weight[l], e->bn_bias[l], e->bn_running_mean[l],
                                 e->bn_running_var[l], e->bn_num_batches_tracked[l],
                                 F(lay.mean[l]), F(lay.invstd[l]), F(lay.coef[l]), D,
                                 MOLCLR_DTYPE_F32, e->momentum, e->eps, e->training, kws, kws_bytes,
                                 stream));
      else
        MOLCLR_TRY(seg_bn_fwd(seg, z, e->bn_weight[l], e->bn_bias[l], e->bn_running_mean[l],
                              e->bn_running_var[l], e->bn_num_batches_tracked[l], y,
                              F(lay.mean[l]), F(lay.invstd[l]), D, MOLCLR_DTYPE_F32, e->momentum,
                              e->eps, e->training, last ? 0 : 1, kws, kws_bytes, stream));
    }
    h = y;
  }
  return MOLCLR_OK;
}

MOLCLR_API int molclr_gin_encoder_bwd(const molclr_gin_encoder* e,
                                      const molclr_gin_encoder_grads* gr, const int64_t* x,
                                      const molclr_device_graph* g, const void* dh_out,
                                      const void* arena, size_t arena_bytes, void* workspace,
                                      size_t workspace_bytes, molclr_stream_t stream) {
  MOLCLR_TRY(check_encoder(e, g));
  MOLCLR_REQUIRE(gr, "gin_encoder_bwd: null grads");
  MOLCLR_REQUIRE(e->training, "gin_encoder_bwd: backward through eval-mode BatchNorm");
  const int L = e->num_layer;
  const int64_t N = g->num_nodes, D = e->dim;
  if (N == 0) return MOLCLR_OK;
  SegRows seg;
  MOLCLR_TRY(graph_segments(g, &g->num_nodes, seg));
  MOLCLR_REQUIRE(x && dh_out && arena, "gin_encoder_bwd: null pointer");
  const bool bf = e->dtype == MOLCLR_DTYPE_BF16;
  const size_t es = elem_bytes(e->dtype);
  const ArenaLayout lay(L, N, D, es);
  MOLCLR_REQUIRE_WS(arena_bytes, lay.total);
  MOLCLR_REQUIRE_WS(workspace_bytes, molclr_gin_encoder_workspace_bytes(L, N, D, e->dtype));
  const char* A = (const char*)arena;
  auto F = [&](size_t off) { return (const float*)(A + off); };
  char* S = (char*)workspace;
  void* dh = S;
  void* dz = S + (size_t)N * D * es;
  void* dagg = S + 2 * (size_t)N * D * es;
  void* dz1 = S + 3 * (size_t)N * D * es;
  float* bmax = const_cast<float*>(F(lay.bmax));
  float* rdz = (float*)(S + molclr::align_up(scratch_bytes(N, D, es), 256)) +
               kSlotBytes / sizeof(float);
  float* rdz1 = (float*)((char*)rdz + rowmax_first_bytes(N, D));
  void* kws = (char*)rdz + rowmax_bytes(N, D);
  const size_t kws_bytes = kernels_ws(N, D);
  const int dt = bf ? MOLCLR_DTYPE_BF16 : MOLCLR_DTYPE_F32;
  const bool h3 = !bf && e->fp32_gemm != 0;
  const float* fmax = F(lay.smax);

  const void* dy = dh_out;
  for (int l = L - 1; l >= 0; --l) {
    const void* agg = A + lay.agg[l];
    const void* a1 = A + lay.a1[l];
    const void* z = A + lay.z[l];
    const bool last = l == L - 1;
    MOLCLR_REQUIRE(gr->bn_weight[l] && gr->bn_bias[l], "gin_encoder_bwd: BatchNorm grads needed");
    if (h3) {
      MOLCLR_TRY(seg_bn_bwd(seg, dy, z, e->bn_weight[l], e->bn_bias[l], F(lay.mean[l]),
                            F(lay.invstd[l]), dz, gr->bn_weight[l], gr->bn_bias[l], D,
                            MOLCLR_DTYPE_F32, last ? 0 : 1, 1, rdz, nullptr, kws, kws_bytes,
                            stream));
    } else {
      MOLCLR_TRY(seg_bn_bwd(seg, dy, z, e->bn_weight[l], e->bn_bias[l], F(lay.mean[l]),
                            F(lay.invstd[l]), dz, gr->bn_weight[l], gr->bn_bias[l], D, dt,
                            last ? 0 : 1, 1, nullptr, nullptr, kws, kws_bytes, stream));
    }
    if (bf) {
      const uint16_t *hz = (const uint16_t*)dz, *ha1 = (const uint16_t*)a1;
      if (gr->mlp2_weight[l] || gr->mlp2_bias[l]) {
        MOLCLR_REQUIRE(gr->mlp2_weight[l], "gin_encoder_bwd: bf16 needs the weight gradient");
        MOLCLR_TRY(molclr_linear_wgrad_bf16(hz, ha1, gr->mlp2_weight[l], gr->mlp2_bias[l], N, D,
                                            2 * D, D, 2 * D, 1, kws, kws_bytes, stream));
      }
      if (D % 64 == 0)
        MOLCLR_TRY(molclr_gemm_bf16_bits(hz, e->mlp2_planes_t[l], (uint16_t*)dz1, N, 2 * D, D, D,
                                         2 * D, MOLCLR_EPI_RELU_MASK, nullptr, nullptr,
                                         (const uint32_t*)(A + lay.bits[l]), stream));
      else
        MOLCLR_TRY(molclr_gemm_bf16(hz, e->mlp2_planes_t[l], (uint16_t*)dz1, N, 2 * D, D, D, 2 * D,
                                    MOLCLR_EPI_RELU_MASK, nullptr, ha1, 2 * D, stream));
      if (gr->mlp0_weight[l] || gr->mlp0_bias[l]) {
        MOLCLR_REQUIRE(gr->mlp0_weight[l], "gin_encoder_bwd: bf16 needs the weight gradient");
        MOLCLR_TRY(molclr_linear_wgrad_bf16((const uint16_t*)dz1, (const uint16_t*)agg,
                                            gr->mlp0_weight[l], gr->mlp0_bias[l], N, 2 * D, D,
                                            2 * D, D, 1, kws, kws_bytes, stream));
      }
      MOLCLR_TRY(molclr_gemm_bf16((const uint16_t*)dz1, e->mlp0_planes_t[l], (uint16_t*)dagg, N,
                                  D, 2 * D, 2 * D, D, MOLCLR_EPI_NONE, nullptr, nullptr, 0, stream));
      MOLCLR_TRY(molclr_gine_aggregate_bwd_bf16((const uint16_t*)dagg, g->rowptr_t, g->col_t,
                                                g->nbr_t, g->ecount, (uint16_t*)dh,
                                                gr->edge_embedding1[l], gr->edge_embedding2[l], N,
                                                D, 1, kws, kws_bytes, stream));
    } else if (h3) {
      const float *fz = (const float*)dz, *fa1 = (const float*)a1, *fagg = (const float*)agg;
      float* sl = bmax + 2 * l * kMaxSlotFloats;
      const float* fl = fmax + 2 * l * kMaxSlotFloats;
      MOLCLR_REQUIRE(gr->mlp2_weight[l] && gr->mlp2_bias[l] && gr->mlp0_weight[l] &&
                         gr->mlp0_bias[l],
                     "gin_encoder_bwd: h3 needs every MLP gradient");
      MOLCLR_TRY(molclr_gemm_f32_h3(fz, rdz, molclr_bn_row_parts(D), e->mlp2_planes_t[l],
                                    (float*)dz1, N, 2 * D, D, D, 2 * D, MOLCLR_EPI_RELU_MASK,
                                    nullptr, fa1, 2 * D, (const uint32_t*)(A + lay.bits[l]),
                                    sl + kMaxSlotFloats, rdz1, sl, stream));
      if (N >= 1024) {
        MOLCLR_TRY(molclr_linear_wgrad_h3_pair(
            fz, sl, fa1, fl + kMaxSlotFloats, gr->mlp2_weight[l], gr->mlp2_bias[l], D, 2 * D, D,
            2 * D, (const float*)dz1, sl + kMaxSlotFloats, fagg, fl, gr->mlp0_weight[l],
            gr->mlp0_bias[l], 2 * D, D, 2 * D, D, N, 1, kws, kws_bytes, stream));
      } else {
        MOLCLR_TRY(molclr_linear_wgrad_h3(fz, sl, fa1, fl + kMaxSlotFloats, gr->mlp2_weight[l],
                                          gr->mlp2_bias[l], N, D, 2 * D, D, 2 * D, 1, kws,
                                          kws_bytes, stream));
        MOLCLR_TRY(molclr_linear_wgrad_h3((const float*)dz1, sl + kMaxSlotFloats, fagg, fl,
                                          gr->mlp0_weight[l], gr->mlp0_bias[l], N, 2 * D, D, 2 * D,
                                          D, 1, kws, kws_bytes, stream));
      }
      MOLCLR_TRY(molclr_gemm_f32_h3((const float*)dz1, rdz1, (int)molclr_gemm_row_parts(2 * D),
                                    e->mlp0_planes_t[l], (float*)dagg, N, D, 2 * D, 2 * D, D,
                                    MOLCLR_EPI_NONE, nullptr, nullptr, 0, nullptr, nullptr,
                                    nullptr, nullptr, stream));
      MOLCLR_TRY(molclr_gine_aggregate_bwd((const float*)dagg, g->rowptr_t, g->col_t, g->nbr_t,
                                           g->ecount, (float*)dh, gr->edge_embedding1[l],
                                           gr->edge_embedding2[l], N, D, 1, kws, kws_bytes, stream));
    } else {
      const float *fz = (const float*)dz, *fa1 = (const float*)a1;
      if (gr->mlp2_weight[l])
        MOLCLR_TRY(molclr_linear_wgrad(fz, fa1, gr->mlp2_weight[l], gr->mlp2_bias[l], N, D, 2 * D,
                                       D, 2 * D, 1, kws, kws_bytes, stream));
      else if (gr->mlp2_bias[l])
        MOLCLR_TRY(molclr_colsum_f32(fz, gr->mlp2_bias[l], N, D, D, 1, kws, kws_bytes, stream));
      MOLCLR_TRY(molclr_gemm_f32_bplanes(fz, e->mlp2_planes_t[l], (float*)dz1, N, 2 * D, D, D,
                                         2 * D, 0, MOLCLR_EPI_RELU_MASK, nullptr, fa1, 2 * D, kws,
                                         kws_bytes, stream));
      if (gr->mlp0_weight[l])
        MOLCLR_TRY(molclr_linear_wgrad((const float*)dz1, (const float*)agg, gr->mlp0_weight[l],
                                       gr->mlp0_bias[l], N, 2 * D, D, 2 * D, D, 1, kws, kws_bytes,
                                       stream));
      else if (gr->mlp0_bias[l])
        MOLCLR_TRY(molclr_colsum_f32((const float*)dz1, gr->mlp0_bias[l], N, 2 * D, 2 * D, 1, kws,
                                     kws_bytes, stream));
      MOLCLR_TRY(molclr_gemm_f32_bplanes((const float*)dz1, e->mlp0_planes_t[l], (float*)dagg, N,
                                         D, 2 * D, 2 * D, D, 0, MOLCLR_EPI_NONE, nullptr, nullptr,
                                         0, kws, kws_bytes, stream));
      MOLCLR_TRY(molclr_gine_aggregate_bwd((const float*)dagg, g->rowptr_t, g->col_t, g->nbr_t,
                                           g->ecount, (float*)dh, gr->edge_embedding1[l],
                                           gr->edge_embedding2[l], N, D, 1, kws, kws_bytes, stream));
    }
    MOLCLR_TRY(record_done(gr->layer_done[l], stream));
    dy = dh;
  }
  if (gr->x_embedding1 || gr->x_embedding2) {
    MOLCLR_REQUIRE(gr->x_embedding1 && gr->x_embedding2,
                   "gin_encoder_bwd: both atom-embedding grads or neither");
    if (bf)
      MOLCLR_TRY(molclr_atom_embed_bwd_bf16(x, (const uint16_t*)dh, gr->x_embedding1,
                                            gr->x_embedding2, N, D, e->n_atom, e->n_chiral, 1, kws,
                                            kws_bytes, stream));
    else
      MOLCLR_TRY(molclr_atom_embed_bwd(x, (const float*)dh, gr->x_embedding1, gr->x_embedding2, N,
                                       D, e->n_atom, e->n_chiral, 1, kws, kws_bytes, stream));
  }
  MOLCLR_TRY(record_done(gr->embed_done, stream));
  return MOLCLR_OK;
}

namespace {

struct GcnArena {
  size_t z[MOLCLR_MAX_LAYERS], h[MOLCLR_MAX_LAYERS], mean[MOLCLR_MAX_LAYERS],
      invstd[MOLCLR_MAX_LAYERS];
  size_t hmax[MOLCLR_MAX_LAYERS];
  size_t h0, total;
  GcnArena(int L, int64_t N, int64_t D) {
    size_t used = 0;
    auto off = [&](size_t count) {
      const size_t o = used;
      used += (count + 63) / 64 * 64;
      return o;
    };
    for (int l = 0; l < L; ++l) {
      z[l] = off(N * D);
      h[l] = off(N * D);
      mean[l] = off(MOLCLR_MAX_SEGMENTS * D);
      invstd[l] = off(MOLCLR_MAX_SEGMENTS * D);
    }
    const size_t slots = off((size_t)L * kMaxSlotFloats);
    for (int l = 0; l < L; ++l) hmax[l] = slots + (size_t)l * kMaxSlotFloats;
    h0 = off(N * D);
    total = used * sizeof(float);
  }
};

size_t gcn_kernels_ws(int64_t N, int64_t D) {
  size_t m = 0;
  auto mx = [&](size_t v) { m = v > m ? v : m; };
  mx(molclr_gemm_f32_workspace_bytes(N, D, D));
  mx(molclr_gemm_f32_workspace_bytes(D, D, N));
  mx(molclr_linear_wgrad_workspace_bytes(N, D, D));
  mx(molclr_batchnorm_ws_bound(N, D));
  mx(molclr_gcn_aggregate_bwd_workspace_bytes(N, D));
  mx(molclr_atom_embed_bwd_workspace_bytes(N, D, MOLCLR_NUM_ATOM_TYPE, MOLCLR_NUM_CHIRALITY));
  return m;
}
size_t gcn_scratch_floats(int64_t N, int64_t D) { return (size_t)N * D * 3; }
size_t gcn_h3_bytes(int64_t N) {
  return molclr::align_up((size_t)N * sizeof(float), 256) + kMaxSlotFloats * sizeof(float);
}

int check_gcn(const molclr_gcn_encoder* e, const molclr_device_graph* g) {
  MOLCLR_REQUIRE(e && g, "gcn_encoder: null encoder / graph");
  MOLCLR_REQUIRE(e->num_layer >= 1 && e->num_layer <= MOLCLR_MAX_LAYERS,
                 "gcn_encoder: num_layer %d", e->num_layer);
  MOLCLR_REQUIRE(e->dim > 0 && e->dim % 4 == 0, "gcn_encoder: dim %lld", (long long)e->dim);
  MOLCLR_REQUIRE(e->n_atom == MOLCLR_NUM_ATOM_TYPE && e->n_chiral == MOLCLR_NUM_CHIRALITY,
                 "gcn_encoder: embedding tables must be [%d,D] and [%d,D]",
                 MOLCLR_NUM_ATOM_TYPE, MOLCLR_NUM_CHIRALITY);
  for (int l = 0; l < e->num_layer; ++l)
    MOLCLR_REQUIRE(e->weight_planes[l] && e->weight_planes_t[l] && e->bias[l] &&
                       e->edge_embedding1[l] && e->edge_embedding2[l] && e->bn_weight[l] &&
                       e->bn_bias[l],
                   "gcn_encoder: layer %d: missing planes, bias, edge tables or BatchNorm", l);
  return MOLCLR_OK;
}

}

MOLCLR_API size_t molclr_gcn_encoder_arena_bytes(int L, int64_t N, int64_t D) {
  if (L < 1 || L > MOLCLR_MAX_LAYERS) return 0;
  return GcnArena(L, N, D).total;
}

MOLCLR_API size_t molclr_gcn_encoder_workspace_bytes(int L, int64_t N, int64_t D) {
  (void)L;
  return gcn_scratch_floats(N, D) * sizeof(float) + 256 + gcn_h3_bytes(N) + gcn_kernels_ws(N, D) +
         256;
}

MOLCLR_API int molclr_gcn_encoder_fwd(const molclr_gcn_encoder* e, const int64_t* x,
                                      const molclr_device_graph* g, float* h_out, void* arena,
                                      size_t arena_bytes, void* workspace, size_t workspace_bytes,
                                      molclr_stream_t stream) {
  MOLCLR_TRY(check_gcn(e, g));
  const int L = e->num_layer;
  const int64_t N = g->num_nodes, D = e->dim;
  if (N == 0) return MOLCLR_OK;
  SegRows seg;
  MOLCLR_TRY(graph_segments(g, &g->num_nodes, seg));
  MOLCLR_REQUIRE(x && h_out && arena, "gcn_encoder_fwd: null pointer");
  const GcnArena lay(L, N, D);
  MOLCLR_REQUIRE_WS(arena_bytes, lay.total);
  MOLCLR_REQUIRE_WS(workspace_bytes, molclr_gcn_encoder_workspace_bytes(L, N, D));
  float* A = (float*)arena;
  float* xw = (float*)workspace;
  void* kws = (char*)workspace + molclr::align_up(gcn_scratch_floats(N, D) * sizeof(float), 256);
  const size_t kws_bytes = gcn_kernels_ws(N, D);

  const bool h3 = e->fp32_gemm == 1;
  if (h3 && molclr::zero_async(A + lay.hmax[0], (size_t)L * kMaxSlotFloats * sizeof(float),
                           molclr::as_stream(stream)) != hipSuccess) {
    molclr::set_error("gcn_encoder_fwd: zeroing the max slots failed");
    return MOLCLR_ERR_ARG;
  }
  float* h = A + lay.h0;
  MOLCLR_TRY(molclr_atom_embed_fwd(x, e->x_embedding1, e->x_embedding2, h, N, D, e->n_atom,
                                   e->n_chiral, e->status, stream));
  for (int l = 0; l < L; ++l) {
    float* z = A + lay.z[l];
    const bool last = l == L - 1;
    float* y = last ? h_out : A + lay.h[l];
    if (h3)
      MOLCLR_TRY(molclr_gemm_f32_bplanes_max(h, e->weight_planes[l], xw, N, D, D, D, D,
                                             MOLCLR_EPI_NONE, nullptr, nullptr, 0,
                                             (float*)(A + lay.hmax[l]), nullptr, nullptr, nullptr,
                                             kws, kws_bytes, stream));
    else
      MOLCLR_TRY(molclr_gemm_f32_bplanes(h, e->weight_planes[l], xw, N, D, D, D, D, 0,
                                       MOLCLR_EPI_NONE, nullptr, nullptr, 0, kws, kws_bytes,
                                       stream));
    MOLCLR_TRY(molclr_gcn_aggregate_fwd(xw, g->rowptr, g->col, g->ecode, g->nbr,
                                        e->edge_embedding1[l], e->edge_embedding2[l], e->bias[l],
                                        z, N, D, stream));
    MOLCLR_TRY(seg_bn_fwd(seg, z, e->bn_weight[l], e->bn_bias[l], e->bn_running_mean[l],
                          e->bn_running_var[l], e->bn_num_batches_tracked[l], y, A + lay.mean[l],
                          A + lay.invstd[l], D, MOLCLR_DTYPE_F32, e->momentum, e->eps,
                          e->training, last ? 0 : 1, kws, kws_bytes, stream));
    h = y;
  }
  return MOLCLR_OK;
}

MOLCLR_API int molclr_gcn_encoder_bwd(const molclr_gcn_encoder* e,
                                      const molclr_gcn_encoder_grads* gr, const int64_t* x,
                                      const molclr_device_graph* g, const float* dh_out,
                                      const void* arena, size_t arena_bytes, void* workspace,
                                      size_t workspace_bytes, molclr_stream_t stream) {
  MOLCLR_TRY(check_gcn(e, g));
  MOLCLR_REQUIRE(gr, "gcn_encoder_bwd: null grads");
  MOLCLR_REQUIRE(e->training, "gcn_encoder_bwd: backward through eval-mode BatchNorm");
  const int L = e->num_layer;
  const int64_t N = g->num_nodes, D = e->dim;
  if (N == 0) return MOLCLR_OK;
// ... 61 lines not shown
```

### molclr_amd/csrc/norm.hip

```cpp
#include "common.h"

#include <math.h>

namespace {

constexpr int kT = 256;

__host__ __device__ __forceinline__ int64_t band_parts(int64_t rows, int band) {
  const int64_t unit = (int64_t)band * 16;
  int64_t P = (rows + unit - 1) / unit;
  if (P > 1024) P = 1024;
  if (P < 1) P = 1;
  return P;
}

int64_t band_parts_bound(int64_t rows, int band, int nseg) {
  const int64_t unit = (int64_t)band * 16;
  int64_t P = (rows + unit - 1) / unit + nseg;
  if (P > (int64_t)nseg * 1024) P = (int64_t)nseg * 1024;
  return P;
}

__global__ void k_colsum_partial(const float4* __restrict__ X, int64_t rows, int d4, int64_t ld4,
                                 int band, int64_t rows_per_part, float4* __restrict__ partial) {
// ... 160 lines not shown
}

__device__ __forceinline__ void chan1(float& n, float& mean, float& m2, float nb, float mb, float qb) {
  if (nb == 0.f) return;
  if (n == 0.f) {
    n = nb;
    mean = mb;
    m2 = qb;
    return;
  }
  float nn = n + nb;
  float d = mb - mean;
  mean = mean + d * (nb / nn);
  m2 = m2 + qb + d * d * (n * nb / nn);
  n = nn;
}

constexpr int kSegLanes = kRedLanes / 2;

__global__ __launch_bounds__(kRedCols* kRedLanes) void k_bn_stats_final(
    const float* __restrict__ pmean, const float* __restrict__ pm2, const float* __restrict__ pn,
    Segs sg, int64_t D, const float* __restrict__ gamma, const float* __restrict__ beta,
    float* __restrict__ running_mean, float* __restrict__ running_var,
    float* __restrict__ save_mean, float* __restrict__ save_invstd, float* __restrict__ scale,
    float* __restrict__ shift, float momentum, float eps, int64_t* __restrict__ nbt) {
  __shared__ float rn[kRedLanes][kRedCols], rm[kRedLanes][kRedCols], rq[kRedLanes][kRedCols];
  if (nbt && blockIdx.x == 0 && threadIdx.x == 0) *nbt += sg.n;
  const int cl = threadIdx.x % kRedCols, rl = threadIdx.x / kRedCols;
  const int half = rl / kSegLanes, sl = rl % kSegLanes;
  const int64_t c = (int64_t)blockIdx.x * kRedCols + cl;
  for (int s0 = 0; s0 < sg.n; s0 += 2) {
    const int s = s0 + half;
    float n = 0.f, mean = 0.f, m2 = 0.f;
    if (s < sg.n && c < D) {
      const SegAt at = seg_info(sg, s);
      const int64_t P = at.P;
      const float* sm = pmean + at.part0 * D;
      const float* sq = pm2 + at.part0 * D;
      const float* sn = pn + at.part0;
      for (int64_t p = sl; p < P; p += 4 * kSegLanes) {
        float bn[4], bm[4], bq[4];
#pragma unroll
        for (int u = 0; u < 4; ++u) {
          const int64_t q = p + u * kSegLanes;
          const bool in = q < P;
          bn[u] = in ? sn[q] : 0.f;
          bm[u] = in ? sm[q * D + c] : 0.f;
          bq[u] = in ? sq[q * D + c] : 0.f;
        }
#pragma unroll
        for (int u = 0; u < 4; ++u) chan1(n, mean, m2, bn[u], bm[u], bq[u]);
      }
    }
    __syncthreads();
    rn[rl][cl] = n;
    rm[rl][cl] = mean;
    rq[rl][cl] = m2;
    __syncthreads();
#pragma unroll
    for (int stride = kSegLanes / 2; stride > 0; stride >>= 1) {
      if (sl < stride) {
        chan1(n, mean, m2, rn[rl + stride][cl], rm[rl + stride][cl], rq[rl + stride][cl]);
        rn[rl][cl] = n;
        rm[rl][cl] = mean;
        rq[rl][cl] = m2;
      }
      __syncthreads();
    }
    if (rl == 0 && c < D) {
      for (int h = 0; h < 2 && s0 + h < sg.n; ++h) {
        const int ss = s0 + h;
        const float nn = rn[h * kSegLanes][cl], mu = rm[h * kSegLanes][cl];
        const float q2 = rq[h * kSegLanes][cl];
        const float var = q2 / nn;
        const float invstd = 1.0f / sqrtf(var + eps);
        save_mean[ss * D + c] = mu;
        save_invstd[ss * D + c] = invstd;
        if (running_mean) running_mean[c] = (1.f - momentum) * running_mean[c] + momentum * mu;
        if (running_var) {
          const float unbiased = nn > 1.f ? q2 / (nn - 1.f) : var;
          running_var[c] = (1.f - momentum) * running_var[c] + momentum * unbiased;
        }
        float sc, sh;
        bn_coeffs(gamma ? gamma[c] : 1.f, beta ? beta[c] : 0.f, mu, invstd, sc, sh);
        scale[ss * D + c] = sc;
        shift[ss * D + c] = sh;
      }
    }
  }
}

__global__ void k_bn_eval_coeffs(const float* __restrict__ gamma, const float* __restrict__ beta,
                                 const float* __restrict__ running_mean,
                                 const float* __restrict__ running_var, int64_t D, int nseg,
                                 float eps, float* __restrict__ save_mean,
                                 float* __restrict__ save_invstd, float* __restrict__ scale,
                                 float* __restrict__ shift) {
  int64_t c = (int64_t)blockIdx.x * blockDim.x + threadIdx.x;
  if (c >= D) return;
  float mean = running_mean[c];
  float invstd = 1.0f / sqrtf(running_var[c] + eps);
  float sc, sh;
  bn_coeffs(gamma ? gamma[c] : 1.f, beta ? beta[c] : 0.f, mean, invstd, sc, sh);
  for (int s = 0; s < nseg; ++s) {
    if (save_mean) save_mean[s * D + c] = mean;
    if (save_invstd) save_invstd[s * D + c] = invstd;
    scale[s * D + c] = sc;
    shift[s * D + c] = sh;
  }
}

template <typename St, int U = 1>
__global__ __launch_bounds__(kT) void k_bn_apply(const typename St::T* __restrict__ z,
                                                 const float4* __restrict__ scale,
                                                 const float4* __restrict__ shift,
                                                 typename St::T* __restrict__ y, int64_t total4,
                                                 int d4, int relu, Segs sg) {
  int64_t t = (int64_t)blockIdx.x * blockDim.x + threadIdx.x;
  if (t >= total4 / U) return;
  const int64_t u0 = t * U;
  const int64_t i = row_of(u0, d4, total4);
  const int c = (int)(u0 - i * d4);
  const int s = seg_of_row(sg, i);
  float4 v[U];
  if (s < 0) {
    if constexpr (U == 2) St::st2(y, t, f4zero(), f4zero());
    else St::st(y, t, f4zero());
    return;
  }
  if constexpr (U == 2) St::ld2(z, t, v[0], v[1]);
  else v[0] = St::ld(z, t);
#pragma unroll
  for (int j = 0; j < U; ++j) {
    const float4 sc = scale[s * d4 + c + j], sh = shift[s * d4 + c + j];
    float4 o = make_float4(bn_apply1(v[j].x, sc.x, sh.x), bn_apply1(v[j].y, sc.y, sh.y),
                           bn_apply1(v[j].z, sc.z, sh.z), bn_apply1(v[j].w, sc.w, sh.w));
    if (relu) o = make_float4(fmaxf(o.x, 0.f), fmaxf(o.y, 0.f), fmaxf(o.z, 0.f), fmaxf(o.w, 0.f));
    v[j] = o;
  }
  if constexpr (U == 2) St::st2(y, t, v[0], v[1]);
  else St::st(y, t, v[0]);
}

__device__ __forceinline__ void bn_coeffs4(const float* gamma, const float* beta, float4 mu,
                                           float4 is, int c, float4& sc, float4& sh) {
  float4 g = gamma ? reinterpret_cast<const float4*>(gamma)[c] : make_float4(1.f, 1.f, 1.f, 1.f);
  float4 b = beta ? reinterpret_cast<const float4*>(beta)[c] : f4zero();
  bn_coeffs(g.x, b.x, mu.x, is.x, sc.x, sh.x);
  bn_coeffs(g.y, b.y, mu.y, is.y, sc.y, sh.y);
  bn_coeffs(g.z, b.z, mu.z, is.z, sc.z, sh.z);
  bn_coeffs(g.w, b.w, mu.w, is.w, sc.w, sh.w);
}

template <typename St>
__global__ void k_bn_bwd_partial(const typename St::T* __restrict__ dy,
                                 const typename St::T* __restrict__ z,
                                 const float4* __restrict__ mean, const float4* __restrict__ invstd,
                                 const float* __restrict__ gamma, const float* __restrict__ beta,
                                 int d4, int band, Segs sg, int relu, float4* __restrict__ p1,
                                 float4* __restrict__ p2) {
  extern __shared__ __attribute__((aligned(16))) float4 red[];
  const int tid = threadIdx.x;
  const bool live = tid < band * d4;
  const int r = live ? tid / d4 : 0, c = live ? tid - r * d4 : 0;
  const SegAt at = seg_of_part(sg, blockIdx.x);
  if (at.s < 0) return;
  const int s = at.s;
  const int64_t beg = at.row0 + (blockIdx.x - at.part0) * at.rpp;
  int64_t end = beg + at.rpp;
  if (end > at.row1) end = at.row1;
  float4 s1 = f4zero(), s2 = f4zero();
  if (live) {
    float4 mu = mean[s * d4 + c], is = invstd[s * d4 + c], sc, sh;
    bn_coeffs4(gamma, beta, mu, is, c, sc, sh);
    constexpr int U = 8;
    for (int64_t i0 = beg + r; i0 < end; i0 += U * (int64_t)band) {
      float4 gv[U], xv[U];
#pragma unroll
      for (int u = 0; u < U; ++u) {
        const int64_t i = i0 + (int64_t)u * band;
        const int64_t ii = i < end ? i : i0;
        gv[u] = St::ld(dy, ii * d4 + c);
        xv[u] = St::ld(z, ii * d4 + c);
      }
#pragma unroll
      for (int u = 0; u < U; ++u) {
        if (i0 + (int64_t)u * band >= end) break;
        float4 g = gv[u];
        const float4 x = xv[u];
        if (relu) {
          g.x = bn_apply1(x.x, sc.x, sh.x) > 0.f ? g.x : 0.f;
          g.y = bn_apply1(x.y, sc.y, sh.y) > 0.f ? g.y : 0.f;
          g.z = bn_apply1(x.z, sc.z, sh.z) > 0.f ? g.z : 0.f;
          g.w = bn_apply1(x.w, sc.w, sh.w) > 0.f ? g.w : 0.f;
        }
        s1 = f4add(s1, g);
        s2.x += g.x * ((x.x - mu.x) * is.x);
        s2.y += g.y * ((x.y - mu.y) * is.y);
        s2.z += g.z * ((x.z - mu.z) * is.z);
        s2.w += g.w * ((x.w - mu.w) * is.w);
      }
    }
    red[r * d4 + c] = s1;
    red[(band + r) * d4 + c] = s2;
  }
  __syncthreads();
  if (live && r == 0) {
    float4 a = red[c], b = red[band * d4 + c];
    for (int q = 1; q < band; ++q) {
      a = f4add(a, red[q * d4 + c]);
      b = f4add(b, red[(band + q) * d4 + c]);
    }
    p1[(int64_t)blockIdx.x * d4 + c] = a;
    p2[(int64_t)blockIdx.x * d4 + c] = b;
  }
}

__global__ __launch_bounds__(kRedCols* kRedLanes) void k_bn_bwd_final(
    const float* __restrict__ p1, const float* __restrict__ p2, Segs sg, int64_t D,
    float* __restrict__ dgamma, float* __restrict__ dbeta, float* __restrict__ k1,
    float* __restrict__ k2, int accumulate) {
  __shared__ float ra[kRedLanes][kRedCols], rb[kRedLanes][kRedCols];
  const int cl = threadIdx.x % kRedCols, rl = threadIdx.x / kRedCols;
  const int half = rl / kSegLanes, sl = rl % kSegLanes;
  const int64_t c = (int64_t)blockIdx.x * kRedCols + cl;
  for (int s0 = 0; s0 < sg.n; s0 += 2) {
    const int s = s0 + half;
    float a0 = 0.f, a1 = 0.f, a2 = 0.f, a3 = 0.f, b0 = 0.f, b1 = 0.f, b2 = 0.f, b3 = 0.f;
    if (s < sg.n && c < D) {
      const SegAt at = seg_info(sg, s);
      const int64_t P = at.P;
      const float* q1 = p1 + at.part0 * D;
      const float* q2 = p2 + at.part0 * D;
      for (int64_t p = sl; p < P; p += 4 * kSegLanes) {
        float x1[4], x2[4];
#pragma unroll
        for (int u = 0; u < 4; ++u) {
          const int64_t q = p + u * kSegLanes;
          x1[u] = q < P ? q1[q * D + c] : 0.f;
          x2[u] = q < P ? q2[q * D + c] : 0.f;
        }
        a0 += x1[0];
        a1 += x1[1];
        a2 += x1[2];
        a3 += x1[3];
        b0 += x2[0];
        b1 += x2[1];
        b2 += x2[2];
        b3 += x2[3];
      }
    }
    float a = (a0 + a1) + (a2 + a3), b = (b0 + b1) + (b2 + b3);
    __syncthreads();
    ra[rl][cl] = a;
    rb[rl][cl] = b;
    __syncthreads();
#pragma unroll
    for (int stride = kSegLanes / 2; stride > 0; stride >>= 1) {
      if (sl < stride) {
        ra[rl][cl] = a = a + ra[rl + stride][cl];
        rb[rl][cl] = b = b + rb[rl + stride][cl];
      }
      __syncthreads();
    }
    if (rl == 0 && c < D) {
      for (int h = 0; h < 2 && s0 + h < sg.n; ++h) {
        const int ss = s0 + h;
        const float sa = ra[h * kSegLanes][cl], sb = rb[h * kSegLanes][cl];
        const float inv_rows = 1.0f / (float)seg_n(sg, ss);
        const bool add = accumulate || ss > 0;
        if (dbeta) dbeta[c] = add ? dbeta[c] + sa : sa;
        if (dgamma) dgamma[c] = add ? dgamma[c] + sb : sb;
        k1[ss * D + c] = sa * inv_rows;
        k2[ss * D + c] = sb * inv_rows;
      }
    }
  }
}

__device__ __forceinline__ float4 bn_bwd_math(float4 g, float4 x, const float4* __restrict__ mean,
                                              const float4* __restrict__ invstd,
                                              const float* __restrict__ gamma,
                                              const float* __restrict__ beta,
                                              const float4* __restrict__ k1,
                                              const float4* __restrict__ k2, int s, int c, int d4,
                                              int relu) {
  float4 mu = mean[s * d4 + c], is = invstd[s * d4 + c], sc, sh;
  bn_coeffs4(gamma, beta, mu, is, c, sc, sh);
  float4 a = k1[s * d4 + c], b = k2[s * d4 + c];
  if (relu) {
    g.x = bn_apply1(x.x, sc.x, sh.x) > 0.f ? g.x : 0.f;
    g.y = bn_apply1(x.y, sc.y, sh.y) > 0.f ? g.y : 0.f;
    g.z = bn_apply1(x.z, sc.z, sh.z) > 0.f ? g.z : 0.f;
    g.w = bn_apply1(x.w, sc.w, sh.w) > 0.f ? g.w : 0.f;
  }
  float4 o;
  o.x = (g.x - a.x - ((x.x - mu.x) * is.x) * b.x) * sc.x;
  o.y = (g.y - a.y - ((x.y - mu.y) * is.y) * b.y) * sc.y;
  o.z = (g.z - a.z - ((x.z - mu.z) * is.z) * b.z) * sc.z;
  o.w = (g.w - a.w - ((x.w - mu.w) * is.w) * b.w) * sc.w;
  return o;
}

template <typename St>
__device__ __forceinline__ float4 bn_bwd_elem(
    const typename St::T* __restrict__ dy, const typename St::T* __restrict__ z,
    const float4* __restrict__ mean, const float4* __restrict__ invstd,
    const float* __restrict__ gamma, const float* __restrict__ beta, const float4* __restrict__ k1,
    const float4* __restrict__ k2, typename St::T* __restrict__ dz, int64_t t, int d4, int relu,
    Segs sg, int64_t total4) {
  const int64_t i = row_of(t, d4, total4);
  const int c = (int)(t - i * d4);
  const int s = seg_of_row(sg, i);
  if (s < 0) {
    St::st(dz, t, f4zero());
    return f4zero();
  }
  const float4 o = bn_bwd_math(St::ld(dy, t), St::ld(z, t), mean, invstd, gamma, beta, k1, k2, s,
                               c, d4, relu);
  St::st(dz, t, o);
  return o;
}

template <typename St>
__global__ __launch_bounds__(kT) void k_bn_bwd_apply2(
    const typename St::T* __restrict__ dy, const typename St::T* __restrict__ z,
    const float4* __restrict__ mean, const float4* __restrict__ invstd,
    const float* __restrict__ gamma, const float* __restrict__ beta, const float4* __restrict__ k1,
    const float4* __restrict__ k2, typename St::T* __restrict__ dz, int64_t total4, int d4,
    int relu, Segs sg) {
  const int64_t t = (int64_t)blockIdx.x * blockDim.x + threadIdx.x;
  if (t >= total4 / 2) return;
  const int64_t u0 = 2 * t;
  const int64_t i = row_of(u0, d4, total4);
  const int c = (int)(u0 - i * d4);
  const int s = seg_of_row(sg, i);
  if (s < 0) {
    St::st2(dz, t, f4zero(), f4zero());
    return;
  }
  float4 g0, g1, x0, x1;
  St::ld2(dy, t, g0, g1);
  St::ld2(z, t, x0, x1);
  St::st2(dz, t, bn_bwd_math(g0, x0, mean, invstd, gamma, beta, k1, k2, s, c, d4, relu),
          bn_bwd_math(g1, x1, mean, invstd, gamma, beta, k1, k2, s, c + 1, d4, relu));
}

template <typename St>
__global__ __launch_bounds__(kT) void k_bn_bwd_apply(
    const typename St::T* __restrict__ dy, const typename St::T* __restrict__ z,
    const float4* __restrict__ mean, const float4* __restrict__ invstd,
    const float* __restrict__ gamma, const float* __restrict__ beta, const float4* __restrict__ k1,
    const float4* __restrict__ k2, typename St::T* __restrict__ dz, int64_t total4, int d4,
    int relu, Segs sg, float* __restrict__ rowparts, int nparts, float* __restrict__ slot) {
  int64_t t = (int64_t)blockIdx.x * blockDim.x + threadIdx.x;
  if (rowparts != nullptr) {
    const int64_t rows = total4 / d4;
    float m = 0.f;
    int row = -1;
    if (t < total4) {
      const float4 o = bn_bwd_elem<St>(dy, z, mean, invstd, gamma, beta, k1, k2, dz, t, d4, relu,
                                       sg, total4);
      m = fmaxf(fmaxf(fabsf(o.x), fabsf(o.y)), fmaxf(fabsf(o.z), fabsf(o.w)));
      row = (int)row_of(t, d4, total4);
    }
    row_max_parts(m, row, t, rows, d4, rowparts, nparts);
    if (slot != nullptr) absmax_publish(m, slot);
    return;
  }
  if (t >= total4) return;
  bn_bwd_elem<St>(dy, z, mean, invstd, gamma, beta, k1, k2, dz, t, d4, relu, sg, total4);
}


template <typename St = StF32>
__global__ void k_pool_fwd(const typename St::T* __restrict__ h, const int32_t* __restrict__ ptr,
                           float4* __restrict__ out, int64_t G, int d4, int mode) {
  int64_t t = (int64_t)blockIdx.x * blockDim.x + threadIdx.x;
  if (t >= G * d4) return;
  int64_t g = t / d4;
  int c = (int)(t - g * d4);
  int32_t beg = ptr[g], end = ptr[g + 1];
  float4 acc = f4zero();
  int32_t i = beg;
  for (; i + 8 <= end; i += 8) {
    float4 v[8];
#pragma unroll
    for (int u = 0; u < 8; ++u) v[u] = St::ld(h, (int64_t)(i + u) * d4 + c);
#pragma unroll
    for (int u = 0; u < 8; ++u) acc = f4add(acc, v[u]);
  }
  for (; i < end; ++i) acc = f4add(acc, St::ld(h, (int64_t)i * d4 + c));
  if (mode == 0) {
    float cnt = (float)(end - beg > 1 ? end - beg : 1);
    acc = make_float4(acc.x / cnt, acc.y / cnt, acc.z / cnt, acc.w / cnt);
  }
  out[t] = acc;
}

template <typename St = StF32>
__global__ void k_pool_bwd(const float4* __restrict__ dout, const int32_t* __restrict__ ptr,
                           typename St::T* __restrict__ dh, int64_t G, int d4, int mode, int64_t N) {
  int64_t t = (int64_t)blockIdx.x * blockDim.x + threadIdx.x;
  {
    const int64_t stride = (int64_t)gridDim.x * blockDim.x;
    const int64_t lo = (int64_t)ptr[0] * d4, hi0 = (int64_t)ptr[G] * d4, n4 = N * d4;
    const float4 z = make_float4(0.f, 0.f, 0.f, 0.f);
    for (int64_t q = t; q < lo; q += stride) St::st(dh, q, z);
    for (int64_t q = hi0 + t; q < n4; q += stride) St::st(dh, q, z);
  }
  if (t >= G * d4) return;
  int64_t g = t / d4;
  int c = (int)(t - g * d4);
  int32_t beg = ptr[g], end = ptr[g + 1];
  float4 v = dout[t];
  if (mode == 0) {
    float cnt = (float)(end - beg > 1 ? end - beg : 1);
    v = make_float4(v.x / cnt, v.y / cnt, v.z / cnt, v.w / cnt);
  }
  for (int32_t i = beg; i < end; ++i) St::st(dh, (int64_t)i * d4 + c, v);
}

template <typename St = StF32>
__global__ void k_pool_max_fwd(const typename St::T* __restrict__ h, const int32_t* __restrict__ ptr,
                               float4* __restrict__ out, int4* __restrict__ arg, int64_t G, int d4) {
  int64_t t = (int64_t)blockIdx.x * blockDim.x + threadIdx.x;
  if (t >= G * d4) return;
  int64_t g = t / d4;
  int c = (int)(t - g * d4);
  int32_t beg = ptr[g], end = ptr[g + 1];
  float m[4] = {-INFINITY, -INFINITY, -INFINITY, -INFINITY};
  int a[4] = {-1, -1, -1, -1};
  for (int32_t i = beg; i < end; ++i) {
    const float4 v = St::ld(h, (int64_t)i * d4 + c);
    const float e[4] = {v.x, v.y, v.z, v.w};
#pragma unroll
    for (int j = 0; j < 4; ++j)
      if (a[j] < 0 || e[j] > m[j]) {
        m[j] = e[j];
        a[j] = i;
      }
  }
#pragma unroll
  for (int j = 0; j < 4; ++j)
    if (a[j] < 0) m[j] = 0.f;
  out[t] = make_float4(m[0], m[1], m[2], m[3]);
  arg[t] = make_int4(a[0], a[1], a[2], a[3]);
}

template <typename St = StF32>
__global__ void k_pool_max_bwd(const float4* __restrict__ dout, const int4* __restrict__ arg,
                               typename St::T* __restrict__ dh, int64_t G, int d4) {
  int64_t t = (int64_t)blockIdx.x * blockDim.x + threadIdx.x;
  if (t >= G * d4) return;
  const int c = (int)(t % d4);
  const float4 v = dout[t];
  const int4 a = arg[t];
  const float e[4] = {v.x, v.y, v.z, v.w};
  const int ai[4] = {a.x, a.y, a.z, a.w};
#pragma unroll
  for (int j = 0; j < 4; ++j)
    if (ai[j] >= 0) St::st1(dh, (int64_t)ai[j] * (4 * d4) + 4 * c + j, e[j]);
}

__global__ __launch_bounds__(256) void k_l2norm_fwd(const float* __restrict__ z,
                                                    float* __restrict__ y,
                                                    float* __restrict__ norm, int64_t rows,
                                                    int64_t D, float eps) {
  const int lane = threadIdx.x & 63;
  const int64_t r = ((int64_t)blockIdx.x * blockDim.x + threadIdx.x) >> 6;
  if (r >= rows) return;
  const float* zr = z + r * D;
  float ss = 0.f;
  for (int64_t c = lane; c < D; c += 64) ss += zr[c] * zr[c];
  ss = wave_sum(ss);
  float nrm = sqrtf(ss);
  float den = fmaxf(nrm, eps);
  if (lane == 0) norm[r] = nrm;
  for (int64_t c = lane; c < D; c += 64) y[r * D + c] = zr[c] / den;
}

__global__ __launch_bounds__(256) void k_l2norm_bwd(const float* __restrict__ dy,
                                                    const float* __restrict__ y,
                                                    const float* __restrict__ norm,
                                                    float* __restrict__ dz, int64_t rows,
                                                    int64_t D, float eps) {
  const int lane = threadIdx.x & 63;
  const int64_t r = ((int64_t)blockIdx.x * blockDim.x + threadIdx.x) >> 6;
  if (r >= rows) return;
  float nrm = norm[r];
  if (nrm > eps) {
    float dot = 0.f;
    for (int64_t c = lane; c < D; c += 64) dot += dy[r * D + c] * y[r * D + c];
    dot = wave_sum(dot);
    for (int64_t c = lane; c < D; c += 64)
      dz[r * D + c] = (dy[r * D + c] - dot * y[r * D + c]) / nrm;
  } else {
    for (int64_t c = lane; c < D; c += 64) dz[r * D + c] = dy[r * D + c] / eps;
  }
}

__global__ __launch_bounds__(1024) void k_sum(const float* __restrict__ x, float* __restrict__ out,
                                              int64_t n) {
  __shared__ float ws[16];
  float acc = 0.f;
  for (int64_t i = threadIdx.x; i < n; i += blockDim.x) acc += x[i];
  acc = wave_sum(acc);
  if ((threadIdx.x & 63) == 0) ws[threadIdx.x >> 6] = acc;
  __syncthreads();
  if (threadIdx.x == 0) {
    float s = 0.f;
    for (int w = 0; w < (int)(blockDim.x >> 6); ++w) s += ws[w];
    *out = s;
  }
}

}

size_t molclr_colsum_ws(int64_t rows, int64_t cols) {
  molclr::Band b = molclr::make_band(cols);
  return (size_t)band_parts(rows, b.band) * cols * sizeof(float) + 256;
}

int molclr_colsum_impl(const float* X, float* out, int64_t rows, int64_t cols, int64_t ld,
// ... 3 lines not shown
  int64_t P = band_parts(rows, b.band);
  float* partial = w.take<float>(P * cols);
  if (!w.ok()) {
    molclr::set_error("colsum: workspace too small");
    return MOLCLR_ERR_WORKSPACE;
  }
  int64_t rpp = molclr::ceil_div(rows > 0 ? rows : 1, P);
  size_t lds = (size_t)b.band * b.d4 * sizeof(float4);
  hipLaunchKernelGGL(k_colsum_partial, dim3(P), dim3(b.threads), lds, s, (const float4*)X, rows,
                     b.d4, ld / 4, b.band, rpp, (float4*)partial);
  hipLaunchKernelGGL(k_colsum_final, dim3(molclr::ceil_div(cols, kRedCols)), dim3(kRedCols * kRedLanes), 0, s, partial, P,
                     cols, out, accumulate);
  MOLCLR_LAUNCHED();
  return MOLCLR_OK;
}

MOLCLR_API size_t molclr_colsum_f32_workspace_bytes(int64_t rows, int64_t cols) {
  return molclr_colsum_ws(rows, cols);
}

MOLCLR_API int molclr_colsum_f32(const float* X, float* out, int64_t rows, int64_t cols,
                                 int64_t ld, int accumulate, void* workspace,
                                 size_t workspace_bytes, molclr_stream_t stream) {
  MOLCLR_REQUIRE_WS(workspace_bytes, molclr_colsum_ws(rows, cols));
  molclr::Workspace w(workspace, workspace_bytes);
  return molclr_colsum_impl(X, out, rows, cols, ld, accumulate, w, molclr::as_stream(stream));
}

namespace {

int make_segs(int nseg, const int64_t* seg_rows, const int64_t* drows, int64_t cap, int64_t D,
              Segs& sg, int64_t& P, int64_t& rows) {
  MOLCLR_REQUIRE(nseg >= 1 && nseg <= MOLCLR_MAX_SEGMENTS && (seg_rows || drows),
                 "batchnorm: %d segments (1..%d)", nseg, MOLCLR_MAX_SEGMENTS);
  const molclr::Band b = molclr::make_band(D);
  sg.n = nseg;
  sg.band = b.band;
  sg.drows = drows;
  P = 0;
  rows = 0;
  for (int s = 0; s < MOLCLR_MAX_SEGMENTS; ++s) sg.rows[s] = 0;
  if (drows) {
    MOLCLR_REQUIRE(cap >= 0, "batchnorm: negative row capacity");
    P = band_parts_bound(cap, b.band, nseg);
    rows = cap;
    return MOLCLR_OK;
  }
  for (int s = 0; s < nseg; ++s) {
    MOLCLR_REQUIRE(seg_rows[s] >= 0, "batchnorm: negative segment rows");
    sg.rows[s] = seg_rows[s];
    P += band_parts(seg_rows[s], b.band);
    rows += seg_rows[s];
  }
  return MOLCLR_OK;
}

size_t bn_ws_bytes(int64_t P, int64_t D, int nseg) {
  molclr::Workspace w(nullptr, 0);
  w.take<float>(P * D);
  w.take<float>(P * D);
  w.take<float>(P);
  w.take<float>(nseg * D);
  w.take<float>(nseg * D);
  w.take<float>(nseg * D);
  w.take<float>(nseg * D);
  return w.used + 256;
}

struct BnPlan {
  Segs sg;
  int64_t rows;
  const float *scale, *shift;
};
template <typename St>
int bn_fwd_coeffs(const void* zv, const float* gamma, const float* beta, float* running_mean,
                  float* running_var, int64_t* nbt, float* save_mean, float* save_invstd,
                  float* coeffs, int nseg, const int64_t* seg_rows, int64_t D, double momentum,
                  double eps, int training, void* workspace, size_t workspace_bytes, hipStream_t s,
                  const int64_t* drows, int64_t cap, BnPlan& plan) {
  Segs& sg = plan.sg;
  int64_t P = 0, rows = 0;
  if (int rc = make_segs(nseg, seg_rows, drows, cap, D, sg, P, rows)) return rc;
  MOLCLR_REQUIRE(D > 0 && D % 4 == 0, "batchnorm_fwd: dim must be a multiple of 4");
  for (int q = 0; q < nseg && !drows; ++q)
    MOLCLR_REQUIRE(!training || seg_rows[q] > 1,
                   "batchnorm_fwd: need more than 1 row per segment when training");
  MOLCLR_REQUIRE(training || (running_mean && running_var), "batchnorm_fwd: eval needs running stats");
  MOLCLR_REQUIRE(save_mean && save_invstd && (rows == 0 || zv), "batchnorm_fwd: null pointer");
  MOLCLR_REQUIRE_WS(workspace_bytes, bn_ws_bytes(P, D, nseg));
  const auto* z = static_cast<const typename St::T*>(zv);
  const molclr::Band b = molclr::make_band(D);
  molclr::Workspace w(workspace, workspace_bytes);
  float* pmean = w.take<float>(P * D);
  float* pm2 = w.take<float>(P * D);
  float* pn = w.take<float>(P);
  float* scale = w.take<float>(nseg * D);
  float* shift = w.take<float>(nseg * D);
  if (coeffs) {
    scale = coeffs;
    shift = coeffs + (size_t)nseg * D;
  }
  if (training) {
    const size_t lds = 2 * (size_t)b.band * b.d4 * sizeof(float4);
    hipLaunchKernelGGL(k_bn_stats_partial<St>, dim3((unsigned)P), dim3(b.threads), lds, s, z, b.d4,
                       b.band, sg, (float4*)pmean, (float4*)pm2, pn);
    hipLaunchKernelGGL(k_bn_stats_final, dim3(molclr::ceil_div(D, kRedCols)),
                       dim3(kRedCols * kRedLanes), 0, s, pmean, pm2, pn, sg, D, gamma, beta,
                       running_mean, running_var, save_mean, save_invstd, scale, shift,
                       (float)momentum, (float)eps, nbt);
  } else {
    hipLaunchKernelGGL(k_bn_eval_coeffs, dim3(molclr::ceil_div(D, kT)), dim3(kT), 0, s, gamma,
                       beta, running_mean, running_var, D, nseg, (float)eps, save_mean,
                       save_invstd, scale, shift);
  }
  plan.rows = rows;
  plan.scale = scale;
  plan.shift = shift;
  MOLCLR_LAUNCHED();
  return MOLCLR_OK;
}

template <typename St>
int bn_fwd(const void* zv, const float* gamma, const float* beta, float* running_mean,
           float* running_var, int64_t* nbt, void* yv, float* save_mean, float* save_invstd,
           int nseg, const int64_t* seg_rows, int64_t D, double momentum, double eps, int training,
           int relu, void* workspace, size_t workspace_bytes, hipStream_t s,
           const int64_t* drows = nullptr, int64_t cap = 0) {
  BnPlan plan;
  if (int rc = bn_fwd_coeffs<St>(zv, gamma, beta, running_mean, running_var, nbt, save_mean,
                                 save_invstd, nullptr, nseg, seg_rows, D, momentum, eps, training,
                                 workspace, workspace_bytes, s, drows, cap, plan))
    return rc;
  const auto* z = static_cast<const typename St::T*>(zv);
  auto* y = static_cast<typename St::T*>(yv);
  const Segs& sg = plan.sg;
  const float *scale = plan.scale, *shift = plan.shift;
  const int64_t total4 = plan.rows * (D / 4);
  if (total4 > 0 && y) {
    if (St::kBytes == 2 && D % 8 == 0)
      hipLaunchKernelGGL((k_bn_apply<St, 2>), dim3(molclr::ceil_div(total4 / 2, kT)), dim3(kT), 0,
                         s, z, (const float4*)scale, (const float4*)shift, y, total4, (int)(D / 4),
                         relu, sg);
    else
      hipLaunchKernelGGL((k_bn_apply<St, 1>), dim3(molclr::ceil_div(total4, kT)), dim3(kT), 0, s,
                         z, (const float4*)scale, (const float4*)shift, y, total4, (int)(D / 4),
                         relu, sg);
  }
  MOLCLR_LAUNCHED();
  return MOLCLR_OK;
}

int bn_row_parts(int64_t D) { return (int)((D / 4 + 62) / 64) + 1; }

template <typename St>
int bn_bwd(const void* dyv, const void* zv, const float* gamma, const float* beta,
           const float* save_mean, const float* save_invstd, void* dzv, float* dgamma,
           float* dbeta, int nseg, const int64_t* seg_rows, int64_t D, int relu, int accumulate,
           void* workspace, size_t workspace_bytes, hipStream_t s, float* rowparts = nullptr,
           float* slot = nullptr, const int64_t* drows = nullptr, int64_t cap = 0) {
  Segs sg;
  int64_t P = 0, rows = 0;
  if (int rc = make_segs(nseg, seg_rows, drows, cap, D, sg, P, rows)) return rc;
  MOLCLR_REQUIRE(D > 0 && D % 4 == 0, "batchnorm_bwd: dim must be a multiple of 4");
  MOLCLR_REQUIRE(rows > 0 && dyv && zv && save_mean && save_invstd && dzv, "batchnorm_bwd: bad args");
  for (int q = 0; q < nseg && !drows; ++q)
    MOLCLR_REQUIRE(seg_rows[q] > 0, "batchnorm_bwd: empty segment");
  MOLCLR_REQUIRE_WS(workspace_bytes, bn_ws_bytes(P, D, nseg));
  const auto* dy = static_cast<const typename St::T*>(dyv);
  const auto* z = static_cast<const typename St::T*>(zv);
  auto* dz = static_cast<typename St::T*>(dzv);
  const molclr::Band b = molclr::make_band(D);
  molclr::Workspace w(workspace, workspace_bytes);
  float* p1 = w.take<float>(P * D);
  float* p2 = w.take<float>(P * D);
  w.take<float>(P);
  w.take<float>(nseg * D);
  w.take<float>(nseg * D);
  float* k1 = w.take<float>(nseg * D);
  float* k2 = w.take<float>(nseg * D);
  const size_t lds = 2 * (size_t)b.band * b.d4 * sizeof(float4);
  hipLaunchKernelGGL(k_bn_bwd_partial<St>, dim3((unsigned)P), dim3(b.threads), lds, s, dy, z,
                     (const float4*)save_mean, (const float4*)save_invstd, gamma, beta, b.d4,
                     b.band, sg, relu, (float4*)p1, (float4*)p2);
  hipLaunchKernelGGL(k_bn_bwd_final, dim3(molclr::ceil_div(D, kRedCols)), dim3(kRedCols * kRedLanes),
                     0, s, p1, p2, sg, D, dgamma, dbeta, k1, k2, accumulate);
  const int64_t total4 = rows * (D / 4);
  static_assert(kT % 64 == 0, "row parts follow the waves");
  MOLCLR_REQUIRE(!rowparts || rows < (1ll << 31), "batchnorm_seg_bwd_max: too many rows");
  if (St::kBytes == 2 && D % 8 == 0 && !rowparts && !slot)
    hipLaunchKernelGGL(k_bn_bwd_apply2<St>, dim3(molclr::ceil_div(total4 / 2, kT)), dim3(kT), 0, s,
                       dy, z, (const float4*)save_mean, (const float4*)save_invstd, gamma, beta,
                       (const float4*)k1, (const float4*)k2, dz, total4, (int)(D / 4), relu, sg);
  else
    hipLaunchKernelGGL(k_bn_bwd_apply<St>, dim3(molclr::ceil_div(total4, kT)), dim3(kT), 0, s, dy,
                       z, (const float4*)save_mean, (const float4*)save_invstd, gamma, beta,
                       (const float4*)k1, (const float4*)k2, dz, total4, (int)(D / 4), relu, sg,
                       rowparts, bn_row_parts(D), slot);
  MOLCLR_LAUNCHED();
  return MOLCLR_OK;
}

}

size_t molclr_batchnorm_ws_bound(int64_t rows, int64_t D) {
  const molclr::Band b = molclr::make_band(D > 0 ? D : 4);
  return bn_ws_bytes(band_parts_bound(rows, b.band, MOLCLR_MAX_SEGMENTS), D, MOLCLR_MAX_SEGMENTS);
}

MOLCLR_API size_t molclr_batchnorm_seg_workspace_bytes(int nseg, const int64_t* seg_rows,
                                                       int64_t D) {
  Segs sg;
  int64_t P = 0, rows = 0;
  if (make_segs(nseg, seg_rows, nullptr, 0, D > 0 ? D : 4, sg, P, rows)) return 0;
  return bn_ws_bytes(P, D, nseg);
}

MOLCLR_API size_t molclr_batchnorm_workspace_bytes(int64_t rows, int64_t D) {
  return molclr_batchnorm_seg_workspace_bytes(1, &rows, D);
}

MOLCLR_API int molclr_batchnorm_seg_fwd(const void* z, const float* gamma, const float* beta,
                                        float* running_mean, float* running_var,
                                        int64_t* num_batches_tracked, void* y, float* save_mean,
                                        float* save_invstd, int nseg, const int64_t* seg_rows,
                                        int64_t D, int dtype, double momentum, double eps,
                                        int training, int relu, void* workspace,
                                        size_t workspace_bytes, molclr_stream_t stream) {
  hipStream_t s = molclr::as_stream(stream);
  if (dtype == MOLCLR_DTYPE_F32)
    return bn_fwd<StF32>(z, gamma, beta, running_mean, running_var, num_batches_tracked, y,
                         save_mean, save_invstd, nseg, seg_rows, D, momentum, eps, training, relu,
                         workspace, workspace_bytes, s);
  MOLCLR_REQUIRE(dtype == MOLCLR_DTYPE_BF16, "batchnorm_seg_fwd: dtype %d", dtype);
  return bn_fwd<StBF16>(z, gamma, beta, running_mean, running_var, num_batches_tracked, y,
                        save_mean, save_invstd, nseg, seg_rows, D, momentum, eps, training, relu,
                        workspace, workspace_bytes, s);
}

MOLCLR_API int molclr_batchnorm_seg_bwd(const void* dy, const void* z, const float* gamma,
                                        const float* beta, const float* save_mean,
                                        const float* save_invstd, void* dz, float* dgamma,
                                        float* dbeta, int nseg, const int64_t* seg_rows, int64_t D,
                                        int dtype, int relu, int accumulate, void* workspace,
                                        size_t workspace_bytes, molclr_stream_t stream) {
  hipStream_t s = molclr::as_stream(stream);
  if (dtype == MOLCLR_DTYPE_F32)
    return bn_bwd<StF32>(dy, z, gamma, beta, save_mean, save_invstd, dz, dgamma, dbeta, nseg,
                         seg_rows, D, relu, accumulate, workspace, workspace_bytes, s);
  MOLCLR_REQUIRE(dtype == MOLCLR_DTYPE_BF16, "batchnorm_seg_bwd: dtype %d", dtype);
  return bn_bwd<StBF16>(dy, z, gamma, beta, save_mean, save_invstd, dz, dgamma, dbeta, nseg,
                        seg_rows, D, relu, accumulate, workspace, workspace_bytes, s);
}

MOLCLR_API int molclr_bn_row_parts(int64_t dim) { return bn_row_parts(dim); }

MOLCLR_API int molclr_batchnorm_seg_bwd_max(const float* dy, const float* z, const float* gamma,
                                            const float* beta, const float* save_mean,
                                            const float* save_invstd, float* dz, float* dgamma,
                                            float* dbeta, int nseg, const int64_t* seg_rows,
                                            int64_t D, int relu, int accumulate, float* rowmax,
                                            float* slot, void* workspace, size_t workspace_bytes,
                                            molclr_stream_t stream) {
  MOLCLR_REQUIRE(rowmax, "batchnorm_seg_bwd_max: null rowmax");
  return bn_bwd<StF32>(dy, z, gamma, beta, save_mean, save_invstd, dz, dgamma, dbeta, nseg,
                       seg_rows, D, relu, accumulate, workspace, workspace_bytes,
                       molclr::as_stream(stream), rowmax, slot);
}

MOLCLR_API size_t molclr_batchnorm_seg_dev_workspace_bytes(int nseg, int64_t rows_cap, int64_t D) {
  if (nseg < 1 || nseg > MOLCLR_MAX_SEGMENTS) return 0;
  const molclr::Band b = molclr::make_band(D > 0 ? D : 4);
  return bn_ws_bytes(band_parts_bound(rows_cap, b.band, nseg), D, nseg);
}

MOLCLR_API int molclr_batchnorm_seg_fwd_dev(const void* z, const float* gamma, const float* beta,
                                            float* running_mean, float* running_var,
                                            int64_t* num_batches_tracked, void* y, float* save_mean,
                                            float* save_invstd, int nseg,
                                            const int64_t* seg_rows_dev, int64_t rows_cap,
                                            int64_t D, int dtype, double momentum, double eps,
                                            int training, int relu, void* workspace,
                                            size_t workspace_bytes, molclr_stream_t stream) {
  MOLCLR_REQUIRE(seg_rows_dev, "batchnorm_seg_fwd_dev: null seg_rows_dev");
  hipStream_t s = molclr::as_stream(stream);
  if (dtype == MOLCLR_DTYPE_F32)
    return bn_fwd<StF32>(z, gamma, beta, running_mean, running_var, num_batches_tracked, y,
                         save_mean, save_invstd, nseg, nullptr, D, momentum, eps, training, relu,
                         workspace, workspace_bytes, s, seg_rows_dev, rows_cap);
  MOLCLR_REQUIRE(dtype == MOLCLR_DTYPE_BF16, "batchnorm_seg_fwd_dev: dtype %d", dtype);
  return bn_fwd<StBF16>(z, gamma, beta, running_mean, running_var, num_batches_tracked, y,
                        save_mean, save_invstd, nseg, nullptr, D, momentum, eps, training, relu,
                        workspace, workspace_bytes, s, seg_rows_dev, rows_cap);
}

MOLCLR_API int molclr_batchnorm_seg_coeffs(const void* z, const float* gamma, const float* beta,
                                           float* running_mean, float* running_var,
                                           int64_t* num_batches_tracked, float* save_mean,
                                           float* save_invstd, float* coeffs, int nseg,
                                           const int64_t* seg_rows, int64_t D, int dtype,
                                           double momentum, double eps, int training,
                                           void* workspace, size_t workspace_bytes,
                                           molclr_stream_t stream) {
  MOLCLR_REQUIRE(coeffs, "batchnorm_seg_coeffs: null coeffs");
  hipStream_t s = molclr::as_stream(stream);
  BnPlan plan;
  if (dtype == MOLCLR_DTYPE_F32)
    return bn_fwd_coeffs<StF32>(z, gamma, beta, running_mean, running_var, num_batches_tracked,
                                save_mean, save_invstd, coeffs, nseg, seg_rows, D, momentum, eps,
                                training, workspace, workspace_bytes, s, nullptr, 0, plan);
  MOLCLR_REQUIRE(dtype == MOLCLR_DTYPE_BF16, "batchnorm_seg_coeffs: dtype %d", dtype);
  return bn_fwd_coeffs<StBF16>(z, gamma, beta, running_mean, running_var, num_batches_tracked,
                               save_mean, save_invstd, coeffs, nseg, seg_rows, D, momentum, eps,
                               training, workspace, workspace_bytes, s, nullptr, 0, plan);
}

MOLCLR_API int molclr_batchnorm_seg_coeffs_dev(const void* z, const float* gamma, const float* beta,
                                               float* running_mean, float* running_var,
                                               int64_t* num_batches_tracked, float* save_mean,
                                               float* save_invstd, float* coeffs, int nseg,
                                               const int64_t* seg_rows_dev, int64_t rows_cap,
                                               int64_t D, int dtype, double momentum, double eps,
                                               int training, void* workspace,
                                               size_t workspace_bytes, molclr_stream_t stream) {
  MOLCLR_REQUIRE(coeffs && seg_rows_dev, "batchnorm_seg_coeffs_dev: null coeffs / seg_rows_dev");
  hipStream_t s = molclr::as_stream(stream);
  BnPlan plan;
  if (dtype == MOLCLR_DTYPE_F32)
    return bn_fwd_coeffs<StF32>(z, gamma, beta, running_mean, running_var, num_batches_tracked,
                                save_mean, save_invstd, coeffs, nseg, nullptr, D, momentum, eps,
                                training, workspace, workspace_bytes, s, seg_rows_dev, rows_cap,
                                plan);
  MOLCLR_REQUIRE(dtype == MOLCLR_DTYPE_BF16, "batchnorm_seg_coeffs_dev: dtype %d", dtype);
  return bn_fwd_coeffs<StBF16>(z, gamma, beta, running_mean, running_var, num_batches_tracked,
                               save_mean, save_invstd, coeffs, nseg, nullptr, D, momentum, eps,
                               training, workspace, workspace_bytes, s, seg_rows_dev, rows_cap,
                               plan);
}

MOLCLR_API int molclr_batchnorm_seg_bwd_dev(const void* dy, const void* z, const float* gamma,
                                            const float* beta, const float* save_mean,
                                            const float* save_invstd, void* dz, float* dgamma,
                                            float* dbeta, int nseg, const int64_t* seg_rows_dev,
                                            int64_t rows_cap, int64_t D, int dtype, int relu,
                                            int accumulate, float* rowmax, float* slot,
                                            void* workspace, size_t workspace_bytes,
                                            molclr_stream_t stream) {
  MOLCLR_REQUIRE(seg_rows_dev, "batchnorm_seg_bwd_dev: null seg_rows_dev");
  MOLCLR_REQUIRE(!rowmax || dtype == MOLCLR_DTYPE_F32, "batchnorm_seg_bwd_dev: row maxima are fp32 only");
  hipStream_t s = molclr::as_stream(stream);
  if (dtype == MOLCLR_DTYPE_F32)
    return bn_bwd<StF32>(dy, z, gamma, beta, save_mean, save_invstd, dz, dgamma, dbeta, nseg,
                         nullptr, D, relu, accumulate, workspace, workspace_bytes, s, rowmax, slot,
                         seg_rows_dev, rows_cap);
  MOLCLR_REQUIRE(dtype == MOLCLR_DTYPE_BF16, "batchnorm_seg_bwd_dev: dtype %d", dtype);
  return bn_bwd<StBF16>(dy, z, gamma, beta, save_mean, save_invstd, dz, dgamma, dbeta, nseg,
                        nullptr, D, relu, accumulate, workspace, workspace_bytes, s, nullptr,
                        nullptr, seg_rows_dev, rows_cap);
}

MOLCLR_API int molclr_batchnorm_fwd(const float* z, const float* gamma, const float* beta,
                                    float* running_mean, float* running_var,
                                    int64_t* num_batches_tracked, float* y,
                                    float* save_mean, float* save_invstd, int64_t rows,
                                    int64_t D, double momentum, double eps, int training,
                                    int relu, void* workspace, size_t workspace_bytes,
                                    molclr_stream_t stream) {
  return molclr_batchnorm_seg_fwd(z, gamma, beta, running_mean, running_var, num_batches_tracked,
                                  y, save_mean, save_invstd, 1, &rows, D, MOLCLR_DTYPE_F32,
                                  momentum, eps, training, relu, workspace, workspace_bytes, stream);
}

MOLCLR_API int molclr_batchnorm_bwd(const float* dy, const float* z, const float* gamma,
                                    const float* beta, const float* save_mean,
                                    const float* save_invstd, float* dz, float* dgamma,
                                    float* dbeta, int64_t rows, int64_t D, int relu,
                                    int accumulate, void* workspace, size_t workspace_bytes,
                                    molclr_stream_t stream) {
  return molclr_batchnorm_seg_bwd(dy, z, gamma, beta, save_mean, save_invstd, dz, dgamma, dbeta,
                                  1, &rows, D, MOLCLR_DTYPE_F32, relu, accumulate, workspace,
                                  workspace_bytes, stream);
}

MOLCLR_API int molclr_segment_pool_fwd(const float* h, const int32_t* graph_ptr, float* out,
                                       int64_t G, int64_t D, int mode, molclr_stream_t stream) {
  MOLCLR_REQUIRE(D > 0 && D % 4 == 0, "segment_pool_fwd: dim must be a multiple of 4");
  if (mode != 0 && mode != 1) {
    molclr::set_error("segment_pool_fwd: mode %d unsupported (0 mean, 1 add)", mode);
    return MOLCLR_ERR_UNSUPPORTED;
  }
  if (G == 0) return MOLCLR_OK;
  int d4 = (int)(D / 4);
  hipLaunchKernelGGL(k_pool_fwd<StF32>, dim3(molclr::ceil_div(G * d4, kT)), dim3(kT), 0,
                     molclr::as_stream(stream), h, graph_ptr, (float4*)out, G, d4, mode);
  MOLCLR_LAUNCHED();
  return MOLCLR_OK;
}

MOLCLR_API int molclr_segment_pool_bwd(const float* dout, const int32_t* graph_ptr, float* dh,
                                       int64_t N, int64_t G, int64_t D, int mode,
                                       molclr_stream_t stream) {
  MOLCLR_REQUIRE(D > 0 && D % 4 == 0, "segment_pool_bwd: dim must be a multiple of 4");
  if (mode != 0 && mode != 1) {
    molclr::set_error("segment_pool_bwd: mode %d unsupported (0 mean, 1 add)", mode);
    return MOLCLR_ERR_UNSUPPORTED;
  }
  hipStream_t s = molclr::as_stream(stream);
  if (N == 0) return MOLCLR_OK;
  int d4 = (int)(D / 4);
  const int64_t work = G * d4 > 0 ? G * d4 : 1;
  hipLaunchKernelGGL(k_pool_bwd<StF32>, dim3(molclr::ceil_div(work, kT)), dim3(kT), 0, s,
                     (const float4*)dout, graph_ptr, dh, G, d4, mode, N);
  MOLCLR_LAUNCHED();
  return MOLCLR_OK;
}

MOLCLR_API int molclr_segment_pool_fwd_bf16(const uint16_t* h, const int32_t* graph_ptr,
                                            float* out, int64_t G, int64_t D, int mode,
                                            molclr_stream_t stream) {
  MOLCLR_REQUIRE(D > 0 && D % 4 == 0, "segment_pool_fwd_bf16: dim must be a multiple of 4");
  MOLCLR_REQUIRE(mode == 0 || mode == 1, "segment_pool_fwd_bf16: mode %d (0 mean, 1 add)", mode);
  if (G == 0) return MOLCLR_OK;
  const int d4 = (int)(D / 4);
  hipLaunchKernelGGL(k_pool_fwd<StBF16>, dim3(molclr::ceil_div(G * d4, kT)), dim3(kT), 0,
                     molclr::as_stream(stream), h, graph_ptr, (float4*)out, G, d4, mode);
  MOLCLR_LAUNCHED();
  return MOLCLR_OK;
}

MOLCLR_API int molclr_segment_pool_bwd_bf16(const float* dout, const int32_t* graph_ptr,
                                            uint16_t* dh, int64_t N, int64_t G, int64_t D, int mode,
                                            molclr_stream_t stream) {
  MOLCLR_REQUIRE(D > 0 && D % 4 == 0, "segment_pool_bwd_bf16: dim must be a multiple of 4");
  MOLCLR_REQUIRE(mode == 0 || mode == 1, "segment_pool_bwd_bf16: mode %d (0 mean, 1 add)", mode);
  hipStream_t s = molclr::as_stream(stream);
  if (N == 0) return MOLCLR_OK;
  const int d4 = (int)(D / 4);
  const int64_t work = G * d4 > 0 ? G * d4 : 1;
  hipLaunchKernelGGL(k_pool_bwd<StBF16>, dim3(molclr::ceil_div(work, kT)), dim3(kT), 0, s,
                     (const float4*)dout, graph_ptr, dh, G, d4, mode, N);
  MOLCLR_LAUNCHED();
  return MOLCLR_OK;
}

MOLCLR_API int molclr_segment_max_fwd(const void* h, const int32_t* graph_ptr, float* out,
                                      int32_t* argmax, int64_t G, int64_t D, int dtype,
                                      molclr_stream_t stream) {
  MOLCLR_REQUIRE(D > 0 && D % 4 == 0, "segment_max_fwd: dim must be a multiple of 4");
  MOLCLR_REQUIRE(dtype == MOLCLR_DTYPE_F32 || dtype == MOLCLR_DTYPE_BF16,
                 "segment_max_fwd: bad dtype %d", dtype);
  MOLCLR_REQUIRE(G >= 0, "segment_max_fwd: bad graph count");
  if (G == 0) return MOLCLR_OK;
  MOLCLR_REQUIRE(h && graph_ptr && out && argmax, "segment_max_fwd: null pointer");
  const int d4 = (int)(D / 4);
  const dim3 g(molclr::ceil_div(G * d4, kT)), b(kT);
  hipStream_t s = molclr::as_stream(stream);
  if (dtype == MOLCLR_DTYPE_BF16)
    hipLaunchKernelGGL(k_pool_max_fwd<StBF16>, g, b, 0, s, static_cast<const uint16_t*>(h),
                       graph_ptr, (float4*)out, (int4*)argmax, G, d4);
  else
    hipLaunchKernelGGL(k_pool_max_fwd<StF32>, g, b, 0, s, static_cast<const float*>(h), graph_ptr,
                       (float4*)out, (int4*)argmax, G, d4);
  MOLCLR_LAUNCHED();
  return MOLCLR_OK;
}

MOLCLR_API int molclr_segment_max_bwd(const float* dout, const int32_t* argmax, void* dh,
                                      int64_t N, int64_t G, int64_t D, int dtype,
                                      molclr_stream_t stream) {
  MOLCLR_REQUIRE(D > 0 && D % 4 == 0, "segment_max_bwd: dim must be a multiple of 4");
  MOLCLR_REQUIRE(dtype == MOLCLR_DTYPE_F32 || dtype == MOLCLR_DTYPE_BF16,
                 "segment_max_bwd: bad dtype %d", dtype);
  MOLCLR_REQUIRE(N >= 0 && G >= 0, "segment_max_bwd: bad sizes");
  hipStream_t s = molclr::as_stream(stream);
  const size_t esz = dtype == MOLCLR_DTYPE_BF16 ? sizeof(uint16_t) : sizeof(float);
  if (N > 0 && molclr::zero_async(dh, (size_t)N * D * esz, s) != hipSuccess) {
    molclr::set_error("segment_max_bwd: memset failed");
    return MOLCLR_ERR_ARG;
  }
  if (G == 0) return MOLCLR_OK;
  const int d4 = (int)(D / 4);
  const dim3 g(molclr::ceil_div(G * d4, kT)), b(kT);
  if (dtype == MOLCLR_DTYPE_BF16)
    hipLaunchKernelGGL(k_pool_max_bwd<StBF16>, g, b, 0, s, (const float4*)dout,
                       (const int4*)argmax, static_cast<uint16_t*>(dh), G, d4);
  else
    hipLaunchKernelGGL(k_pool_max_bwd<StF32>, g, b, 0, s, (const float4*)dout, (const int4*)argmax,
                       static_cast<float*>(dh), G, d4);
  MOLCLR_LAUNCHED();
  return MOLCLR_OK;
}

MOLCLR_API int molclr_l2norm_fwd(const float* z, float* y, float* norm, int64_t rows, int64_t D,
                                 double eps, molclr_stream_t stream) {
  MOLCLR_REQUIRE(D > 0, "l2norm_fwd: bad dim");
  if (rows == 0) return MOLCLR_OK;
  hipLaunchKernelGGL(k_l2norm_fwd, dim3(molclr::ceil_div(rows * 64, 256)), dim3(256), 0,
                     molclr::as_stream(stream), z, y, norm, rows, D, (float)eps);
  MOLCLR_LAUNCHED();
  return MOLCLR_OK;
}

MOLCLR_API int molclr_l2norm_bwd(const float* dy, const float* y, const float* norm, float* dz,
                                 int64_t rows, int64_t D, double eps, molclr_stream_t stream) {
  MOLCLR_REQUIRE(D > 0, "l2norm_bwd: bad dim");
  if (rows == 0) return MOLCLR_OK;
  hipLaunchKernelGGL(k_l2norm_bwd, dim3(molclr::ceil_div(rows * 64, 256)), dim3(256), 0,
                     molclr::as_stream(stream), dy, y, norm, dz, rows, D, (float)eps);
  MOLCLR_LAUNCHED();
  return MOLCLR_OK;
}

MOLCLR_API int molclr_sum_f32(const float* x, float* out, int64_t n, molclr_stream_t stream) {
// ... 6 lines not shown
```

Measured before the change: 186,800 molecules/s.

## Fuse GINE aggregate-backward node gather into next BatchNorm backward

For layers below the top, the aggregate backward no longer writes dh. The following BatchNorm backward gathers the upstream gradient on the fly from dagg, summing over in-neighbours plus the self row via the neighbour slot table or CSR, so the full dh write and re-read are avoided. The fold is on by default for fp32, and mode 2 also materialises the gathered dy once so the apply pass reads it instead of gathering again. In the default mode the gather runs twice, in the partial-sum kernel and again in the apply kernel, so random neighbour reads rise while the streaming dh traffic goes away.

```diff
diff --git a/include/molclr.h b/include/molclr.h
--- a/include/molclr.h
+++ b/include/molclr.h
@@ -324,6 +324,15 @@
                                  int nseg, const int64_t* seg_rows, int64_t dim, int relu,
                                  int accumulate, float* rowmax, float* slot, void* workspace,
                                  size_t workspace_bytes, molclr_stream_t stream);
+int molclr_batchnorm_seg_bwd_gather(const void* g, const int32_t* rowptr_t, const int32_t* col_t,
+                                    const uint32_t* nbr_t, const void* z, const float* gamma,
+                                    const float* beta, const float* save_mean,
+                                    const float* save_invstd, void* dz, float* dgamma,
+                                    float* dbeta, int nseg, const int64_t* seg_rows,
+                                    const int64_t* seg_rows_dev, int64_t rows_cap, int64_t dim,
+                                    int dtype, int relu, int accumulate, float* rowmax,
+                                    float* slot, void* dy_out, void* workspace,
+                                    size_t workspace_bytes, molclr_stream_t stream);
 
 int molclr_segment_pool_fwd(const float* h, const int32_t* graph_ptr, float* out,
                             int64_t num_graphs, int64_t dim, int mode,
diff --git a/molclr_amd/_lib.py b/molclr_amd/_lib.py
--- a/molclr_amd/_lib.py
+++ b/molclr_amd/_lib.py
@@ -107,6 +107,9 @@
                                              c_size_t, _P]),
     "molclr_batchnorm_seg_bwd_dev": (c_int, [_P, _P, _P, _P, _P, _P, _P, _P, _P, c_int, _P, _I64,
                                              _I64, c_int, c_int, c_int, _P, _P, _P, c_size_t, _P]),
+    "molclr_batchnorm_seg_bwd_gather": (c_int, [_P, _P, _P, _P, _P, _P, _P, _P, _P, _P, _P, _P, c_int,
+                                                _P, _P, _I64, _I64, c_int, c_int, c_int, _P, _P, _P,
+                                                _P, c_size_t, _P]),
     "molclr_segment_pool_fwd": (c_int, [_P, _P, _P, _I64, _I64, c_int, _P]),
     "molclr_segment_pool_bwd": (c_int, [_P, _P, _P, _I64, _I64, _I64, c_int, _P]),
     "molclr_l2norm_fwd": (c_int, [_P, _P, _P, _I64, _I64, c_double, _P]),
diff --git a/molclr_amd/csrc/aggregate.hip b/molclr_amd/csrc/aggregate.hip
--- a/molclr_amd/csrc/aggregate.hip
+++ b/molclr_amd/csrc/aggregate.hip
@@ -256,10 +256,6 @@
   const int64_t c = rc - (int64_t)r * D;
   Ec[t] = p.e1[l][(r / 3) * D + c] + p.e2[l][(r % 3) * D + c];
 }
-
-__device__ __forceinline__ uint32_t nbr_degree(uint32_t w0) { return w0 >> 29; }
-__device__ __forceinline__ int32_t nbr_node(uint32_t w) { return (int32_t)(w & 0xFFFFFFu); }
-__device__ __forceinline__ int nbr_ecomb(uint32_t w) { return (int)((w >> 24) & 15u); }
 
 __device__ __forceinline__ float4 gine_msg(const float4* __restrict__ x, const float4* __restrict__ Ec,
                                            uint32_t w, int d4, int c) {
diff --git a/molclr_amd/csrc/common.h b/molclr_amd/csrc/common.h
--- a/molclr_amd/csrc/common.h
+++ b/molclr_amd/csrc/common.h
@@ -280,6 +280,10 @@
   }
   return -1;
 }
+
+__device__ __forceinline__ uint32_t nbr_degree(uint32_t w0) { return w0 >> 29; }
+__device__ __forceinline__ int32_t nbr_node(uint32_t w) { return (int32_t)(w & 0xFFFFFFu); }
+__device__ __forceinline__ int nbr_ecomb(uint32_t w) { return (int)((w >> 24) & 15u); }
 
 __device__ __forceinline__ float bn_apply1(float z, float sc, float sh) { return __fmaf_rn(z, sc, sh); }
 
diff --git a/molclr_amd/csrc/encoder.hip b/molclr_amd/csrc/encoder.hip
--- a/molclr_amd/csrc/encoder.hip
+++ b/molclr_amd/csrc/encoder.hip
@@ -10,6 +10,12 @@
     return !(e != nullptr && e[0] == '0');
   }();
   return on;
+}
+
+int bnbwd_gather(bool bf) {
+  const char* e = getenv("MOLCLR_BNBWD_GATHER");
+  if (e == nullptr) return bf ? 0 : 1;
+  return e[0] == '0' ? 0 : e[0] == '2' ? 2 : 1;
 }
 
 struct ArenaLayout {
@@ -148,6 +154,17 @@
                                         accumulate, rowmax, slot, ws, ws_bytes, stream);
   return molclr_batchnorm_seg_bwd(dy, z, gamma, beta, mean, invstd, dz, dgamma, dbeta, sg.n,
                                   sg.rows, D, dtype, relu, accumulate, ws, ws_bytes, stream);
+}
+
+int seg_bn_bwd_gather(const SegRows& sg, const void* g, const molclr_device_graph* gph,
+                      const void* z, const float* gamma, const float* beta, const float* mean,
+                      const float* invstd, void* dz, float* dgamma, float* dbeta, int64_t D,
+                      int dtype, int relu, int accumulate, float* rowmax, float* slot,
+                      void* dy_out, void* ws, size_t ws_bytes, molclr_stream_t stream) {
+  return molclr_batchnorm_seg_bwd_gather(g, gph->rowptr_t, gph->col_t, gph->nbr_t, z, gamma, beta,
+                                         mean, invstd, dz, dgamma, dbeta, sg.n, sg.rows, sg.dev,
+                                         sg.cap, D, dtype, relu, accumulate, rowmax, slot, dy_out,
+                                         ws, ws_bytes, stream);
 }
 
 #define MOLCLR_TRY(expr)      \
@@ -360,6 +377,8 @@
   const bool h3 = !bf && e->fp32_gemm != 0;
   const float* fmax = F(lay.smax);
 
+  const int fold = bnbwd_gather(bf);
+  bool gathered = false;
   const void* dy = dh_out;
   for (int l = L - 1; l >= 0; --l) {
     const void* agg = A + lay.agg[l];
@@ -367,16 +386,17 @@
     const void* z = A + lay.z[l];
     const bool last = l == L - 1;
     MOLCLR_REQUIRE(gr->bn_weight[l] && gr->bn_bias[l], "gin_encoder_bwd: BatchNorm grads needed");
-    if (h3) {
-      MOLCLR_TRY(seg_bn_bwd(seg, dy, z, e->bn_weight[l], e->bn_bias[l], F(lay.mean[l]),
-                            F(lay.invstd[l]), dz, gr->bn_weight[l], gr->bn_bias[l], D,
-                            MOLCLR_DTYPE_F32, last ? 0 : 1, 1, rdz, nullptr, kws, kws_bytes,
-                            stream));
-    } else {
+    float* rmax = h3 ? rdz : nullptr;
+    if (gathered)
+      MOLCLR_TRY(seg_bn_bwd_gather(seg, dagg, g, z, e->bn_weight[l], e->bn_bias[l],
+                                   F(lay.mean[l]), F(lay.invstd[l]), dz, gr->bn_weight[l],
+                                   gr->bn_bias[l], D, dt, last ? 0 : 1, 1, rmax, nullptr,
+                                   fold == 2 ? dh : nullptr, kws, kws_bytes, stream));
+    else
       MOLCLR_TRY(seg_bn_bwd(seg, dy, z, e->bn_weight[l], e->bn_bias[l], F(lay.mean[l]),
                             F(lay.invstd[l]), dz, gr->bn_weight[l], gr->bn_bias[l], D, dt,
-                            last ? 0 : 1, 1, nullptr, nullptr, kws, kws_bytes, stream));
-    }
+                            last ? 0 : 1, 1, rmax, nullptr, kws, kws_bytes, stream));
+    void* dx = fold && l >= 1 ? nullptr : dh;
     if (bf) {
       const uint16_t *hz = (const uint16_t*)dz, *ha1 = (const uint16_t*)a1;
       if (gr->mlp2_weight[l] || gr->mlp2_bias[l]) {
@@ -400,7 +420,7 @@
       MOLCLR_TRY(molclr_gemm_bf16((const uint16_t*)dz1, e->mlp0_planes_t[l], (uint16_t*)dagg, N,
                                   D, 2 * D, 2 * D, D, MOLCLR_EPI_NONE, nullptr, nullptr, 0, stream));
       MOLCLR_TRY(molclr_gine_aggregate_bwd_bf16((const uint16_t*)dagg, g->rowptr_t, g->col_t,
-                                                g->nbr_t, g->ecount, (uint16_t*)dh,
+                                                g->nbr_t, g->ecount, (uint16_t*)dx,
                                                 gr->edge_embedding1[l], gr->edge_embedding2[l], N,
                                                 D, 1, kws, kws_bytes, stream));
     } else if (h3) {
@@ -432,7 +452,7 @@
                                     MOLCLR_EPI_NONE, nullptr, nullptr, 0, nullptr, nullptr,
                                     nullptr, nullptr, stream));
       MOLCLR_TRY(molclr_gine_aggregate_bwd((const float*)dagg, g->rowptr_t, g->col_t, g->nbr_t,
-                                           g->ecount, (float*)dh, gr->edge_embedding1[l],
+                                           g->ecount, (float*)dx, gr->edge_embedding1[l],
                                            gr->edge_embedding2[l], N, D, 1, kws, kws_bytes, stream));
     } else {
       const float *fz = (const float*)dz, *fa1 = (const float*)a1;
@@ -455,10 +475,11 @@
                                          D, 2 * D, 2 * D, D, 0, MOLCLR_EPI_NONE, nullptr, nullptr,
                                          0, kws, kws_bytes, stream));
       MOLCLR_TRY(molclr_gine_aggregate_bwd((const float*)dagg, g->rowptr_t, g->col_t, g->nbr_t,
-                                           g->ecount, (float*)dh, gr->edge_embedding1[l],
+                                           g->ecount, (float*)dx, gr->edge_embedding1[l],
                                            gr->edge_embedding2[l], N, D, 1, kws, kws_bytes, stream));
     }
     MOLCLR_TRY(record_done(gr->layer_done[l], stream));
+    gathered = dx == nullptr;
     dy = dh;
   }
   if (gr->x_embedding1 || gr->x_embedding2) {
diff --git a/molclr_amd/csrc/norm.hip b/molclr_amd/csrc/norm.hip
--- a/molclr_amd/csrc/norm.hip
+++ b/molclr_amd/csrc/norm.hip
@@ -336,53 +336,161 @@
   bn_coeffs(g.w, b.w, mu.w, is.w, sc.w, sh.w);
 }
 
+struct PlainDy {};
+struct GatherDy {
+  const int32_t* rowptr_t;
+  const int32_t* col_t;
+  const uint4* nbr_t;
+};
+
+template <typename St, int W>
+__device__ __forceinline__ void ld_units(const typename St::T* __restrict__ p, int64_t idx,
+                                         float4 (&o)[W]) {
+  if constexpr (W == 2) St::ld2(p, idx, o[0], o[1]);
+  else o[0] = St::ld(p, idx);
+}
 template <typename St>
-__global__ void k_bn_bwd_partial(const typename St::T* __restrict__ dy,
-                                 const typename St::T* __restrict__ z,
-                                 const float4* __restrict__ mean, const float4* __restrict__ invstd,
-                                 const float* __restrict__ gamma, const float* __restrict__ beta,
-                                 int d4, int band, Segs sg, int relu, float4* __restrict__ p1,
-                                 float4* __restrict__ p2) {
+__device__ __forceinline__ float4 st_round(float4 o) {
+  if constexpr (St::kBytes == 2) {
+    const uint32_t lo = f32x2_to_bf16x2(o.x, o.y), hi = f32x2_to_bf16x2(o.z, o.w);
+    o = make_float4(bf16_to_f32(lo & 0xFFFFu), bf16_to_f32(lo >> 16), bf16_to_f32(hi & 0xFFFFu),
+                    bf16_to_f32(hi >> 16));
+  }
+  return o;
+}
+template <typename St, int W>
+__device__ __forceinline__ void dy_gather(const typename St::T* __restrict__ g, const GatherDy& ga,
+                                          int64_t j, int c, int dw, float4 (&o)[W]) {
+  const uint4 s = ga.nbr_t[j];
+  const uint32_t deg = nbr_degree(s.x);
+  float4 acc[W];
+#pragma unroll
+  for (int w = 0; w < W; ++w) acc[w] = f4zero();
+  auto add = [&](int64_t row) {
+    float4 v[W];
+    ld_units<St, W>(g, row * dw + c, v);
+#pragma unroll
+    for (int w = 0; w < W; ++w) acc[w] = f4add(acc[w], v[w]);
+  };
+  if (deg <= MOLCLR_NBR_SLOTS) {
+    if (deg > 0) add(nbr_node(s.x));
+    if (deg > 1) add(nbr_node(s.y));
+    if (deg > 2) add(nbr_node(s.z));
+    if (deg > 3) add(nbr_node(s.w));
+  } else {
+    for (int32_t k = ga.rowptr_t[j], e = ga.rowptr_t[j + 1]; k < e; ++k) add(ga.col_t[k]);
+  }
+  add(j);
+#pragma unroll
+  for (int w = 0; w < W; ++w) o[w] = st_round<St>(acc[w]);
+}
+template <typename St, int W, typename SA>
+__device__ __forceinline__ void dy_units(const typename St::T* __restrict__ dy, const SA& sa,
+                                         int64_t t, int64_t i, int c, int dw, float4 (&o)[W]) {
+  if constexpr (std::is_same<SA, GatherDy>::value) dy_gather<St, W>(dy, sa, i, c, dw, o);
+  else ld_units<St, W>(dy, t, o);
+}
+template <typename SA>
+__device__ __forceinline__ int64_t dy_block() {
+  if constexpr (std::is_same<SA, GatherDy>::value) return xcd_remap(blockIdx.x, gridDim.x);
+  else return blockIdx.x;
+}
+
+__device__ __forceinline__ void bn_bwd_sums(float4 g, float4 x, float4 mu, float4 is, float4 sc,
+                                            float4 sh, int relu, float4& s1, float4& s2) {
+  if (relu) {
+    g.x = bn_apply1(x.x, sc.x, sh.x) > 0.f ? g.x : 0.f;
+    g.y = bn_apply1(x.y, sc.y, sh.y) > 0.f ? g.y : 0.f;
+    g.z = bn_apply1(x.z, sc.z, sh.z) > 0.f ? g.z : 0.f;
+    g.w = bn_apply1(x.w, sc.w, sh.w) > 0.f ? g.w : 0.f;
+  }
+  s1 = f4add(s1, g);
+  s2.x += g.x * ((x.x - mu.x) * is.x);
+  s2.y += g.y * ((x.y - mu.y) * is.y);
+  s2.z += g.z * ((x.z - mu.z) * is.z);
+  s2.w += g.w * ((x.w - mu.w) * is.w);
+}
+
+template <typename St, typename SA, int U, int LB>
+__global__ __launch_bounds__(LB) void k_bn_bwd_partial(
+    const typename St::T* __restrict__ dy, const typename St::T* __restrict__ z,
+    const float4* __restrict__ mean, const float4* __restrict__ invstd,
+    const float* __restrict__ gamma, const float* __restrict__ beta, int d4, int band, Segs sg,
+    int relu, float4* __restrict__ p1, float4* __restrict__ p2, SA sa,
+    typename St::T* __restrict__ dy_out) {
   extern __shared__ __attribute__((aligned(16))) float4 red[];
   const int tid = threadIdx.x;
   const bool live = tid < band * d4;
   const int r = live ? tid / d4 : 0, c = live ? tid - r * d4 : 0;
-  const SegAt at = seg_of_part(sg, blockIdx.x);
+  const int64_t blk = dy_block<SA>();
+  const SegAt at = seg_of_part(sg, blk);
   if (at.s < 0) return;
   const int s = at.s;
-  const int64_t beg = at.row0 + (blockIdx.x - at.part0) * at.rpp;
+  const int64_t beg = at.row0 + (blk - at.part0) * at.rpp;
   int64_t end = beg + at.rpp;
   if (end > at.row1) end = at.row1;
   float4 s1 = f4zero(), s2 = f4zero();
   if (live) {
     float4 mu = mean[s * d4 + c], is = invstd[s * d4 + c], sc, sh;
     bn_coeffs4(gamma, beta, mu, is, c, sc, sh);
-    constexpr int U = 8;
     for (int64_t i0 = beg + r; i0 < end; i0 += U * (int64_t)band) {
       float4 gv[U], xv[U];
-#pragma unroll
-      for (int u = 0; u < U; ++u) {
-        const int64_t i = i0 + (int64_t)u * band;
-        const int64_t ii = i < end ? i : i0;
-        gv[u] = St::ld(dy, ii * d4 + c);
-        xv[u] = St::ld(z, ii * d4 + c);
-      }
-#pragma unroll
-      for (int u = 0; u < U; ++u) {
-        if (i0 + (int64_t)u * band >= end) break;
-        float4 g = gv[u];
-        const float4 x = xv[u];
-        if (relu) {
-          g.x = bn_apply1(x.x, sc.x, sh.x) > 0.f ? g.x : 0.f;
-          g.y = bn_apply1(x.y, sc.y, sh.y) > 0.f ? g.y : 0.f;
-          g.z = bn_apply1(x.z, sc.z, sh.z) > 0.f ? g.z : 0.f;
-          g.w = bn_apply1(x.w, sc.w, sh.w) > 0.f ? g.w : 0.f;
+      if constexpr (std::is_same<SA, GatherDy>::value) {
+        uint4 sl[U];
+        float4 nv[U][MOLCLR_NBR_SLOTS];
+#pragma unroll
+        for (int u = 0; u < U; ++u) {
+          const int64_t i = i0 + (int64_t)u * band;
+          sl[u] = sa.nbr_t[i < end ? i : i0];
         }
-        s1 = f4add(s1, g);
-        s2.x += g.x * ((x.x - mu.x) * is.x);
-        s2.y += g.y * ((x.y - mu.y) * is.y);
-        s2.z += g.z * ((x.z - mu.z) * is.z);
-        s2.w += g.w * ((x.w - mu.w) * is.w);
+#pragma unroll
+        for (int u = 0; u < U; ++u) {
+          const int64_t i = i0 + (int64_t)u * band;
+          const int64_t ii = i < end ? i : i0;
+          const uint32_t deg = nbr_degree(sl[u].x);
+#pragma unroll
+          for (int q = 0; q < MOLCLR_NBR_SLOTS; ++q) nv[u][q] = f4zero();
+          if (deg <= MOLCLR_NBR_SLOTS) {
+            if (deg > 0) nv[u][0] = St::ld(dy, (int64_t)nbr_node(sl[u].x) * d4 + c);
+            if (deg > 1) nv[u][1] = St::ld(dy, (int64_t)nbr_node(sl[u].y) * d4 + c);
+            if (deg > 2) nv[u][2] = St::ld(dy, (int64_t)nbr_node(sl[u].z) * d4 + c);
+            if (deg > 3) nv[u][3] = St::ld(dy, (int64_t)nbr_node(sl[u].w) * d4 + c);
+          }
+          gv[u] = St::ld(dy, ii * d4 + c);
+          xv[u] = St::ld(z, ii * d4 + c);
+        }
+#pragma unroll
+        for (int u = 0; u < U; ++u) {
+          const int64_t i = i0 + (int64_t)u * band;
+          if (i >= end) break;
+          const uint32_t deg = nbr_degree(sl[u].x);
+          float4 acc = f4zero();
+          if (deg <= MOLCLR_NBR_SLOTS) {
+            if (deg > 0) acc = f4add(acc, nv[u][0]);
+            if (deg > 1) acc = f4add(acc, nv[u][1]);
+            if (deg > 2) acc = f4add(acc, nv[u][2]);
+            if (deg > 3) acc = f4add(acc, nv[u][3]);
+          } else {
+            for (int32_t k = sa.rowptr_t[i], e = sa.rowptr_t[i + 1]; k < e; ++k)
+              acc = f4add(acc, St::ld(dy, (int64_t)sa.col_t[k] * d4 + c));
+          }
+          const float4 g = st_round<St>(f4add(acc, gv[u]));
+          if (dy_out != nullptr) St::st(dy_out, i * d4 + c, g);
+          bn_bwd_sums(g, xv[u], mu, is, sc, sh, relu, s1, s2);
+        }
+      } else {
+#pragma unroll
+        for (int u = 0; u < U; ++u) {
+          const int64_t i = i0 + (int64_t)u * band;
+          const int64_t ii = i < end ? i : i0;
+          gv[u] = St::ld(dy, ii * d4 + c);
+          xv[u] = St::ld(z, ii * d4 + c);
+        }
+#pragma unroll
+        for (int u = 0; u < U; ++u) {
+          if (i0 + (int64_t)u * band >= end) break;
+          bn_bwd_sums(gv[u], xv[u], mu, is, sc, sh, relu, s1, s2);
+        }
       }
     }
     red[r * d4 + c] = s1;
@@ -395,8 +503,8 @@
       a = f4add(a, red[q * d4 + c]);
       b = f4add(b, red[(band + q) * d4 + c]);
     }
-    p1[(int64_t)blockIdx.x * d4 + c] = a;
-    p2[(int64_t)blockIdx.x * d4 + c] = b;
+    p1[blk * d4 + c] = a;
+    p2[blk * d4 + c] = b;
   }
 }
 
@@ -486,13 +594,13 @@
   return o;
 }
 
-template <typename St>
+template <typename St, typename SA>
 __device__ __forceinline__ float4 bn_bwd_elem(
     const typename St::T* __restrict__ dy, const typename St::T* __restrict__ z,
     const float4* __restrict__ mean, const float4* __restrict__ invstd,
     const float* __restrict__ gamma, const float* __restrict__ beta, const float4* __restrict__ k1,
     const float4* __restrict__ k2, typename St::T* __restrict__ dz, int64_t t, int d4, int relu,
-    Segs sg, int64_t total4) {
+    Segs sg, int64_t total4, const SA& sa) {
   const int64_t i = row_of(t, d4, total4);
   const int c = (int)(t - i * d4);
   const int s = seg_of_row(sg, i);
@@ -500,20 +608,22 @@
     St::st(dz, t, f4zero());
     return f4zero();
   }
-  const float4 o = bn_bwd_math(St::ld(dy, t), St::ld(z, t), mean, invstd, gamma, beta, k1, k2, s,
-                               c, d4, relu);
+  float4 g[1];
+  dy_units<St, 1>(dy, sa, t, i, c, d4, g);
+  const float4 o = bn_bwd_math(g[0], St::ld(z, t), mean, invstd, gamma, beta, k1, k2, s, c, d4,
+                               relu);
   St::st(dz, t, o);
   return o;
 }
 
-template <typename St>
+template <typename St, typename SA>
 __global__ __launch_bounds__(kT) void k_bn_bwd_apply2(
     const typename St::T* __restrict__ dy, const typename St::T* __restrict__ z,
     const float4* __restrict__ mean, const float4* __restrict__ invstd,
     const float* __restrict__ gamma, const float* __restrict__ beta, const float4* __restrict__ k1,
     const float4* __restrict__ k2, typename St::T* __restrict__ dz, int64_t total4, int d4,
-    int relu, Segs sg) {
-  const int64_t t = (int64_t)blockIdx.x * blockDim.x + threadIdx.x;
+    int relu, Segs sg, SA sa) {
+  const int64_t t = dy_block<SA>() * blockDim.x + threadIdx.x;
   if (t >= total4 / 2) return;
   const int64_t u0 = 2 * t;
   const int64_t i = row_of(u0, d4, total4);
@@ -523,28 +633,28 @@
     St::st2(dz, t, f4zero(), f4zero());
     return;
   }
-  float4 g0, g1, x0, x1;
-  St::ld2(dy, t, g0, g1);
+  float4 g[2], x0, x1;
+  dy_units<St, 2>(dy, sa, t, i, c / 2, d4 / 2, g);
   St::ld2(z, t, x0, x1);
-  St::st2(dz, t, bn_bwd_math(g0, x0, mean, invstd, gamma, beta, k1, k2, s, c, d4, relu),
-          bn_bwd_math(g1, x1, mean, invstd, gamma, beta, k1, k2, s, c + 1, d4, relu));
-}
-
-template <typename St>
+  St::st2(dz, t, bn_bwd_math(g[0], x0, mean, invstd, gamma, beta, k1, k2, s, c, d4, relu),
+          bn_bwd_math(g[1], x1, mean, invstd, gamma, beta, k1, k2, s, c + 1, d4, relu));
+}
+
+template <typename St, typename SA>
 __global__ __launch_bounds__(kT) void k_bn_bwd_apply(
     const typename St::T* __restrict__ dy, const typename St::T* __restrict__ z,
     const float4* __restrict__ mean, const float4* __restrict__ invstd,
     const float* __restrict__ gamma, const float* __restrict__ beta, const float4* __restrict__ k1,
     const float4* __restrict__ k2, typename St::T* __restrict__ dz, int64_t total4, int d4,
-    int relu, Segs sg, float* __restrict__ rowparts, int nparts, float* __restrict__ slot) {
-  int64_t t = (int64_t)blockIdx.x * blockDim.x + threadIdx.x;
+    int relu, Segs sg, float* __restrict__ rowparts, int nparts, float* __restrict__ slot, SA sa) {
+  int64_t t = dy_block<SA>() * blockDim.x + threadIdx.x;
   if (rowparts != nullptr) {
     const int64_t rows = total4 / d4;
     float m = 0.f;
     int row = -1;
     if (t < total4) {
       const float4 o = bn_bwd_elem<St>(dy, z, mean, invstd, gamma, beta, k1, k2, dz, t, d4, relu,
-                                       sg, total4);
+                                       sg, total4, sa);
       m = fmaxf(fmaxf(fabsf(o.x), fabsf(o.y)), fmaxf(fabsf(o.z), fabsf(o.w)));
       row = (int)row_of(t, d4, total4);
     }
@@ -553,7 +663,7 @@
     return;
   }
   if (t >= total4) return;
-  bn_bwd_elem<St>(dy, z, mean, invstd, gamma, beta, k1, k2, dz, t, d4, relu, sg, total4);
+  bn_bwd_elem<St>(dy, z, mean, invstd, gamma, beta, k1, k2, dz, t, d4, relu, sg, total4, sa);
 }
 
 
@@ -863,12 +973,14 @@
 
 int bn_row_parts(int64_t D) { return (int)((D / 4 + 62) / 64) + 1; }
 
-template <typename St>
+template <typename St, typename SA = PlainDy>
 int bn_bwd(const void* dyv, const void* zv, const float* gamma, const float* beta,
            const float* save_mean, const float* save_invstd, void* dzv, float* dgamma,
            float* dbeta, int nseg, const int64_t* seg_rows, int64_t D, int relu, int accumulate,
            void* workspace, size_t workspace_bytes, hipStream_t s, float* rowparts = nullptr,
-           float* slot = nullptr, const int64_t* drows = nullptr, int64_t cap = 0) {
+           float* slot = nullptr, const int64_t* drows = nullptr, int64_t cap = 0, SA sa = SA{},
+           void* dy_outv = nullptr) {
+  constexpr bool kGather = std::is_same<SA, GatherDy>::value;
   Segs sg;
   int64_t P = 0, rows = 0;
   if (int rc = make_segs(nseg, seg_rows, drows, cap, D, sg, P, rows)) return rc;
@@ -880,6 +992,7 @@
   const auto* dy = static_cast<const typename St::T*>(dyv);
   const auto* z = static_cast<const typename St::T*>(zv);
   auto* dz = static_cast<typename St::T*>(dzv);
+  auto* dy_out = static_cast<typename St::T*>(dy_outv);
   const molclr::Band b = molclr::make_band(D);
   molclr::Workspace w(workspace, workspace_bytes);
   float* p1 = w.take<float>(P * D);
@@ -890,23 +1003,40 @@
   float* k1 = w.take<float>(nseg * D);
   float* k2 = w.take<float>(nseg * D);
   const size_t lds = 2 * (size_t)b.band * b.d4 * sizeof(float4);
-  hipLaunchKernelGGL(k_bn_bwd_partial<St>, dim3((unsigned)P), dim3(b.threads), lds, s, dy, z,
-                     (const float4*)save_mean, (const float4*)save_invstd, gamma, beta, b.d4,
-                     b.band, sg, relu, (float4*)p1, (float4*)p2);
+  const auto* mu = (const float4*)save_mean;
+  const auto* is = (const float4*)save_invstd;
+  bool launched = false;
+  if constexpr (kGather) {
+    if (b.threads <= 256) {
+      hipLaunchKernelGGL((k_bn_bwd_partial<St, SA, 4, 256>), dim3((unsigned)P), dim3(b.threads),
+                         lds, s, dy, z, mu, is, gamma, beta, b.d4, b.band, sg, relu, (float4*)p1,
+                         (float4*)p2, sa, dy_out);
+      launched = true;
+    }
+  }
+  if (!launched)
+    hipLaunchKernelGGL((k_bn_bwd_partial<St, SA, (kGather ? 2 : 8), 1024>), dim3((unsigned)P),
+                       dim3(b.threads), lds, s, dy, z, mu, is, gamma, beta, b.d4, b.band, sg, relu,
+                       (float4*)p1, (float4*)p2, sa, dy_out);
   hipLaunchKernelGGL(k_bn_bwd_final, dim3(molclr::ceil_div(D, kRedCols)), dim3(kRedCols * kRedLanes),
                      0, s, p1, p2, sg, D, dgamma, dbeta, k1, k2, accumulate);
   const int64_t total4 = rows * (D / 4);
   static_assert(kT % 64 == 0, "row parts follow the waves");
   MOLCLR_REQUIRE(!rowparts || rows < (1ll << 31), "batchnorm_seg_bwd_max: too many rows");
-  if (St::kBytes == 2 && D % 8 == 0 && !rowparts && !slot)
-    hipLaunchKernelGGL(k_bn_bwd_apply2<St>, dim3(molclr::ceil_div(total4 / 2, kT)), dim3(kT), 0, s,
-                       dy, z, (const float4*)save_mean, (const float4*)save_invstd, gamma, beta,
-                       (const float4*)k1, (const float4*)k2, dz, total4, (int)(D / 4), relu, sg);
-  else
-    hipLaunchKernelGGL(k_bn_bwd_apply<St>, dim3(molclr::ceil_div(total4, kT)), dim3(kT), 0, s, dy,
-                       z, (const float4*)save_mean, (const float4*)save_invstd, gamma, beta,
-                       (const float4*)k1, (const float4*)k2, dz, total4, (int)(D / 4), relu, sg,
-                       rowparts, bn_row_parts(D), slot);
+  const bool two = St::kBytes == 2 && D % 8 == 0 && !rowparts && !slot;
+  auto apply = [&](const typename St::T* src, auto asa) {
+    typedef decltype(asa) AS;
+    if (two)
+      hipLaunchKernelGGL((k_bn_bwd_apply2<St, AS>), dim3(molclr::ceil_div(total4 / 2, kT)), dim3(kT),
+                         0, s, src, z, mu, is, gamma, beta, (const float4*)k1, (const float4*)k2, dz,
+                         total4, (int)(D / 4), relu, sg, asa);
+    else
+      hipLaunchKernelGGL((k_bn_bwd_apply<St, AS>), dim3(molclr::ceil_div(total4, kT)), dim3(kT), 0, s,
+                         src, z, mu, is, gamma, beta, (const float4*)k1, (const float4*)k2, dz,
+                         total4, (int)(D / 4), relu, sg, rowparts, bn_row_parts(D), slot, asa);
+  };
+  if (kGather && dy_out) apply(dy_out, PlainDy{});
+  else apply(dy, sa);
   MOLCLR_LAUNCHED();
   return MOLCLR_OK;
 }
@@ -1069,6 +1199,35 @@
                         nullptr, seg_rows_dev, rows_cap);
 }
 
+MOLCLR_API int molclr_batchnorm_seg_bwd_gather(
+    const void* g, const int32_t* rowptr_t, const int32_t* col_t, const uint32_t* nbr_t,
+    const void* z, const float* gamma, const float* beta, const float* save_mean,
+    const float* save_invstd, void* dz, float* dgamma, float* dbeta, int nseg,
+    const int64_t* seg_rows, const int64_t* seg_rows_dev, int64_t rows_cap, int64_t D, int dtype,
+    int relu, int accumulate, float* rowmax, float* slot, void* dy_out, void* workspace,
+    size_t workspace_bytes, molclr_stream_t stream) {
+  MOLCLR_REQUIRE(D > 0 && D % 4 == 0, "batchnorm_seg_bwd_gather: dim must be a multiple of 4");
+  MOLCLR_REQUIRE(dtype == MOLCLR_DTYPE_F32 || dtype == MOLCLR_DTYPE_BF16,
+                 "batchnorm_seg_bwd_gather: dtype %d", dtype);
+  MOLCLR_REQUIRE(rowptr_t && col_t && nbr_t, "batchnorm_seg_bwd_gather: null graph arrays");
+  MOLCLR_REQUIRE((seg_rows != nullptr) != (seg_rows_dev != nullptr),
+                 "batchnorm_seg_bwd_gather: seg_rows or seg_rows_dev, one of them");
+  MOLCLR_REQUIRE((!rowmax && !slot) || dtype == MOLCLR_DTYPE_F32,
+                 "batchnorm_seg_bwd_gather: row maxima are fp32 only");
+  MOLCLR_REQUIRE(rowmax || !slot, "batchnorm_seg_bwd_gather: a slot needs rowmax");
+  MOLCLR_REQUIRE(dy_out != g && dy_out != dz && dz != g,
+                 "batchnorm_seg_bwd_gather: g, dz and dy_out must not alias");
+  const GatherDy ga = {rowptr_t, col_t, reinterpret_cast<const uint4*>(nbr_t)};
+  hipStream_t s = molclr::as_stream(stream);
+  if (dtype == MOLCLR_DTYPE_F32)
+    return bn_bwd<StF32, GatherDy>(g, z, gamma, beta, save_mean, save_invstd, dz, dgamma, dbeta,
+                                   nseg, seg_rows, D, relu, accumulate, workspace, workspace_bytes,
+                                   s, rowmax, slot, seg_rows_dev, rows_cap, ga, dy_out);
+  return bn_bwd<StBF16, GatherDy>(g, z, gamma, beta, save_mean, save_invstd, dz, dgamma, dbeta,
+                                  nseg, seg_rows, D, relu, accumulate, workspace, workspace_bytes,
+                                  s, nullptr, nullptr, seg_rows_dev, rows_cap, ga, dy_out);
+}
+
 MOLCLR_API int molclr_batchnorm_fwd(const float* z, const float* gamma, const float* beta,
                                     float* running_mean, float* running_var,
                                     int64_t* num_batches_tracked, float* y,
```

Measured after the change: 187,700 molecules/s (median of 6 runs). About the same (+0.5%).
